# Entscheider/depthhead

Hardware: AMD Instinct MI355X
Metric: depth frames/sec (640x480, 10-tree forest) (higher is better)
Workload: dtype u32/f64

## Files before the change

depthhead_amd/_lib.py:

```python
from __future__ import annotations

import ctypes as C
import os

import numpy as np

_HERE = os.path.dirname(os.path.abspath(__file__))
LIB_PATH = os.path.join(_HERE, "libdepthhead_hip.so")

DH_OK = 0
ERRORS = {-1: "DH_EINVAL", -2: "DH_EFOREST", -3: "DH_EHIP", -4: "DH_ENOMEM", -5: "DH_ESIZE", -6: "DH_ESTATE"}

POSE_DTYPE = np.dtype([("mid_point", "<f4", (3,)), ("reserved", "<u4"), ("rotation", "<f8", (3,))], align=True)
assert POSE_DTYPE.itemsize == 40
SUPPORT_DTYPE = np.dtype([("x", "<u4"), ("y", "<u4"), ("width", "<u4"), ("height", "<u4"), ("windows", "<u4"), ("hits", "<u4"),
                          ("mass", "<u8"), ("total_mass", "<u8")], align=True)
assert SUPPORT_DTYPE.itemsize == 40
SUPPORT_RADIUS = 30
HEAD_DTYPE = np.dtype([("pose", POSE_DTYPE), ("support", SUPPORT_DTYPE)], align=True)
assert HEAD_DTYPE.itemsize == 80 and HEAD_DTYPE.fields["support"][1] == 40
MAX_HEADS = 4
HEADS_SUPPRESS = 2
TRACK_DTYPE = np.dtype([("id", "<u4"), ("age", "<u4"), ("hits", "<u4"), ("misses", "<u4"), ("head", HEAD_DTYPE)], align=True)
assert TRACK_DTYPE.itemsize == 96 and TRACK_DTYPE.fields["head"][1] == 16
# ... 92 lines not shown


class IdentParams(C.Structure):
    _fields_ = [("iterations", C.c_uint32), ("min_points", C.c_uint32), ("gate", C.c_double), ("lam", C.c_double), ("max_rms", C.c_double),
                ("min_ratio", C.c_double), ("reserved", C.c_uint64 * 3)]


VIEW_INSTANCE_DTYPE = np.dtype([("first_cam", "<u4"), ("model", "<u4"), ("views", "<u8"), ("R", "<f4", (9,)), ("t", "<f4", (3,)),
                                ("scale", "<f4"), ("flags", "<u4")], align=True)
assert VIEW_INSTANCE_DTYPE.itemsize == 72
VIEW_FIT_RECORD_DTYPE = np.dtype([("points", "<u4"), ("steps", "<u4"), ("status", "<u4"), ("reserved", "<u4"), ("sum_r2_fixed", "<i8"),
                                  ("views_used", "<u8")], align=True)
assert VIEW_FIT_RECORD_DTYPE.itemsize == 32
FIT_VIEW_TOLERANCE = 0.001


RIG_FIT_STATE_DTYPE = np.dtype([("id", "<u4"), ("R", "<f4", (9,)), ("t", "<f4", (3,)), ("t_prev", "<f4", (3,)), ("views_used", "<u8"),
                                ("tracked", "<u4"), ("have_prev", "<u4"), ("age", "<u4"), ("lost", "<u4")], align=True)
assert RIG_FIT_STATE_DTYPE.itemsize == 88 and RIG_FIT_STATE_DTYPE.fields["views_used"][1] == 64
RIG_FIT_RECORD_DTYPE = np.dtype([("instance", VIEW_INSTANCE_DTYPE), ("fit", VIEW_FIT_RECORD_DTYPE), ("id", "<u4"), ("status", "<u4"),
                                 ("age", "<u4"), ("lost", "<u4"), ("person", "<u4"), ("reserved", "<u4")], align=True)
assert RIG_FIT_RECORD_DTYPE.itemsize == 128 and RIG_FIT_RECORD_DTYPE.fields["fit"][1] == 72
RIG_FIT_NO_PERSON = 0xFFFFFFFF


class RigFitTrackParams(C.Structure):
    _fields_ = [("iterations_tracked", C.c_uint32), ("keep_points", C.c_uint32), ("rms_max", C.c_double), ("max_jump", C.c_double),
                ("max_coast", C.c_uint32), ("max_misses", C.c_uint32), ("reserved", C.c_uint64 * 2)]


class ShapeParams(C.Structure):
    _fields_ = [("gate", C.c_double), ("lam", C.c_double), ("min_points", C.c_uint32), ("reserved0", C.c_uint32),
                ("reserved", C.c_uint64 * 2)]


CALIB_RECORD_DTYPE = np.dtype([("V", "<f4", (9,)), ("u", "<f4", (3,)), ("points", "<u4"), ("pairs", "<u4"), ("status", "<u4"),
                               ("reserved", "<u4"), ("sum_r2_fixed", "<i8"), ("delta", "<f8", (6,))], align=True)
assert CALIB_RECORD_DTYPE.itemsize == 120
CALIB_SKIP = 0xFFFFFFFF
CALIB_ARM_UNIT = 64
CALIB_MAX_ARM = 2048


class CalibParams(C.Structure):
    _fields_ = [("gate", C.c_double), ("lam", C.c_double), ("pivot", C.c_double * 3), ("min_points", C.c_uint32),
                ("reserved0", C.c_uint32), ("reserved", C.c_uint64 * 2)]


class RigTrackParams(C.Structure):
    _fields_ = [("max_heads", C.c_int32), ("radius", C.c_uint32), ("fuse_gate", C.c_uint32), ("gate", C.c_uint32),
                ("max_misses", C.c_uint32)]


class MultiTrackParams(C.Structure):
    _fields_ = [("max_heads", C.c_int32), ("radius", C.c_uint32), ("gate", C.c_uint32), ("max_misses", C.c_uint32)]


class ForestDesc(C.Structure):
    _fields_ = [("n_trees", C.c_uint32), ("roots", C.c_void_p), ("n_nodes", C.c_uint32), ("nodes", C.c_void_p),
                ("n_leaves", C.c_uint32), ("leaf_prob", C.c_void_p), ("off_begin", C.c_void_p),
                ("rot_begin", C.c_void_p), ("offsets", C.c_void_p), ("rotations", C.c_void_p)]


class Params(C.Structure):
    _fields_ = [("stepwidth", C.c_uint32), ("subimage_width", C.c_uint32), ("subimage_height", C.c_uint32),
                ("gaussian_sigma", C.c_float), ("meanshift_iterations", C.c_uint32)]


class Timing(C.Structure):
    _fields_ = [("traverse_ms", C.c_float), ("vote_ms", C.c_float), ("cluster_ms", C.c_float),
                ("total_ms", C.c_float), ("n_frames", C.c_uint32), ("boxsum_ms", C.c_float),
                ("emit_ms", C.c_float), ("reserved", C.c_uint32)]


EXPORTS = [
    "dh_last_error", "dh_version", "dh_forest_create", "dh_forest_destroy", "dh_forest_info",
    "dh_predictor_create", "dh_predictor_destroy", "dh_predictor_update_sigma", "dh_predictor_sigma",
    "dh_predict_batch", "dh_predict_batch_device", "dh_predict_batch_rle", "dh_biwi_decode_depth_device", "dh_host_alloc", "dh_host_free", "dh_predictor_reserve", "dh_predictor_set_forking", "dh_patch_grid",
    "dh_predict_mask", "dh_predict_mask_device", "dh_hough_image", "dh_hough_image_device", "dh_build_hough_image", "dh_build_hough_image_device",
    "dh_predict_from2dhough", "dh_predict_from2dhough_device",
    "dh_biwi_decode_depth", "dh_biwi_parse_cal", "dh_biwi_parse_pose",
    "dh_graph_capture", "dh_graph_launch", "dh_graph_destroy",
    "dh_set_profiling", "dh_get_timing", "dh_debug_enable", "dh_debug_leaf_indices", "dh_debug_patch_flags",
    "dh_debug_grids", "dh_debug_guesses", "dh_debug_votes", "dh_debug_meanshift", "dh_debug_hit_counts", "dh_debug_geometry", "dh_debug_tile_shifts",
    "dh_trainer_create", "dh_trainer_destroy", "dh_trainer_add_frames", "dh_trainer_fit", "dh_trainer_stats", "dh_forest_export",
    "dh_cameras_create", "dh_cameras_destroy", "dh_predict_batch_cameras", "dh_predict_batch_cameras_device",
    "dh_tracker_create", "dh_tracker_destroy", "dh_tracker_reset", "dh_tracker_step", "dh_tracker_step_device",
    "dh_tracker_state", "dh_tracker_capture",
    "dh_predict_batch_support", "dh_predict_batch_support_device", "dh_predict_batch_cameras_support",
    "dh_predict_batch_cameras_support_device", "dh_tracker_step_support", "dh_tracker_step_support_device",
    "dh_predict_heads", "dh_predict_heads_device", "dh_predict_heads_cameras", "dh_predict_heads_cameras_device",
    "dh_multi_tracker_create", "dh_multi_tracker_destroy", "dh_multi_tracker_reset", "dh_multi_tracker_step",
    "dh_multi_tracker_step_device", "dh_multi_tracker_state", "dh_multi_tracker_capture",
    "dh_rig_create", "dh_rig_destroy", "dh_rig_tracker_create", "dh_rig_tracker_destroy", "dh_rig_tracker_reset",
    "dh_rig_tracker_step", "dh_rig_tracker_step_device", "dh_rig_tracker_state", "dh_rig_tracker_capture",
    "dh_mesh_create", "dh_mesh_destroy", "dh_mesh_info", "dh_renderer_create", "dh_renderer_destroy",
    "dh_renderer_set_profiling", "dh_renderer_timing",
    "dh_render_depth", "dh_render_depth_cameras", "dh_render_depth_device", "dh_render_depth_cameras_device",
    "dh_fit_model_create", "dh_fit_model_destroy", "dh_fit_model_info", "dh_fit_params_default", "dh_fitter_create",
    "dh_fitter_destroy", "dh_fit_depth", "dh_fit_depth_cameras", "dh_fit_depth_device", "dh_fit_depth_cameras_device",
    "dh_fit_track_params_default", "dh_fit_tracker_angles", "dh_fit_tracker_create", "dh_fit_tracker_destroy", "dh_fit_tracker_reset",
    "dh_fit_tracker_state", "dh_fit_tracker_step_poses", "dh_fit_tracker_step_poses_device", "dh_fit_tracker_step",
    "dh_fit_tracker_step_device",
    "dh_fit_basis_create", "dh_fit_basis_destroy", "dh_fit_basis_info", "dh_shape_params_default", "dh_fit_shape", "dh_fit_shape_cameras",
    "dh_fit_shape_device", "dh_fit_shape_cameras_device", "dh_fit_shape_views", "dh_fit_shape_views_device",
    "dh_calib_params_default", "dh_fit_calibrate_views", "dh_fit_calibrate_views_device",
    "dh_fit_views_create", "dh_fit_views_destroy", "dh_fit_views_info", "dh_fit_depth_views", "dh_fit_depth_views_device",
    "dh_rig_fit_track_params_default", "dh_rig_fit_tracker_create", "dh_rig_fit_tracker_destroy", "dh_rig_fit_tracker_reset",
    "dh_rig_fit_tracker_state", "dh_rig_fit_tracker_step_persons", "dh_rig_fit_tracker_step_persons_device", "dh_rig_fit_tracker_step",
    "dh_rig_fit_tracker_step_device",
    "dh_fit_subjects_create", "dh_fit_subjects_destroy", "dh_fit_subjects_info", "dh_fit_subjects_model", "dh_fit_subjects_set_coeffs",
    "dh_fit_subjects_state", "dh_fit_subjects_read", "dh_fit_subjects_update", "dh_fit_subjects_update_device", "dh_fit_shape_subjects", "dh_fit_shape_subjects_cameras",
    "dh_fit_shape_subjects_device", "dh_fit_shape_subjects_cameras_device", "dh_fit_depth_carried_device",
    "dh_fit_depth_cameras_carried_device",
    "dh_fit_subjects_create_surface", "dh_fit_subjects_set_offsets", "dh_fit_subjects_read_offsets", "dh_fit_surface_params_default",
    "dh_fit_surface_subjects", "dh_fit_surface_subjects_cameras", "dh_fit_surface_subjects_device", "dh_fit_surface_subjects_cameras_device",
    "dh_fit_ident_params_default", "dh_fit_identify_subjects", "dh_fit_identify_subjects_cameras", "dh_fit_identify_subjects_device",
    "dh_fit_identify_subjects_cameras_device",
    "dh_fit_ident_views_params_default", "dh_fit_identify_subjects_views", "dh_fit_identify_subjects_views_device",
]


class TrainParams(C.Structure):
    _fields_ = [("stepwidth", C.c_uint32), ("subimage_width", C.c_uint32), ("subimage_height", C.c_uint32),
                ("max_depth", C.c_uint32), ("n_trees", C.c_uint32), ("subset_per_tree", C.c_uint32),
                ("subrect_feature_scale", C.c_double), ("features_per_node", C.c_uint32), ("min_subset_size", C.c_uint32),
                ("steepness", C.c_double), ("seed", C.c_uint64)]


class TrainStats(C.Structure):
    _fields_ = [("frames", C.c_uint64), ("pool_size", C.c_uint64), ("pool_positives", C.c_uint64), ("neg_det", C.c_uint64),
                ("levels", C.c_uint32), ("reserved", C.c_uint32)]


class DepthheadError(RuntimeError):
    def __init__(self, code: int, msg: str):
        super().__init__(f"{ERRORS.get(code, code)}: {msg}")
        self.code = code


_lib = None


def load():
    global _lib
    if _lib is not None:
        return _lib
    if os.environ.get("DH_NO_TORCH_PRELOAD") != "1":
        try:
            import torch
        except ImportError:
            pass
    path = os.environ.get("DH_LIB_PATH") or LIB_PATH
    if not os.path.exists(path):
        raise ImportError(f"{path} not built: run `python -c 'import __graft_entry__ as g; g.build()'` "
                          "(the depthhead_amd product path has no CPU fallback)")
    lib = C.CDLL(path)
    for name in EXPORTS:
        fn = getattr(lib, name)
        fn.restype = C.c_int
    lib.dh_last_error.restype = C.c_char_p
    _lib = lib
    return lib


def check(rc: int):
    if rc != DH_OK:
# ... 69 lines not shown
```

depthhead_amd/csrc/dh_api.hip:

```cpp
#include "dh_runtime.h"
#include "dh_render.h"
#include "dh_fit.h"
#include "dh_runtime_fit.h"

extern "C" const char *dh_last_error(void) { return dh_err_get_(); }
extern "C" int dh_version(void) { return DH_VERSION; }

static int forest_create_(const dh_forest_desc *d, dh_forest **out) { return dh_forest_build_(d, out); }

static int forest_destroy_(dh_forest *f) {
    delete f;
    return DH_OK;
}

static int forest_info_(const dh_forest *f, uint32_t *n_trees, uint32_t *n_nodes, uint32_t *n_leaves, uint32_t *max_depth) {
    if (!f) return fail(DH_EINVAL, "dh_forest_info: NULL forest");
    if (n_trees) *n_trees = (uint32_t)f->roots.size();
    if (n_nodes) *n_nodes = (uint32_t)f->nodes.size();
    if (n_leaves) *n_leaves = (uint32_t)f->leaf_prob.size();
    if (max_depth) *max_depth = f->max_depth;
    return DH_OK;
}

static int patch_grid_(const dh_params *p, int w, int h, int *nx, int *ny) {
    if (!p || !nx || !ny) return fail(DH_EINVAL, "dh_patch_grid: NULL argument");
    return dh_patch_grid_(*p, w, h, nx, ny);
}

#define DH_MAX_CHUNKS 8
#define DH_MIN_CHUNK_FRAMES 16

struct Workspace {
    Geom geom;
    int cap_frames = 0;
    Buf<HitRec> hits;
    Buf<HitBox> hit_box;
    Buf<HitRot> hit_rot;
    uint32_t hits_cap = 0;
    Buf<uint32_t> box;
    Buf<unsigned long long> box_mask;
    int blk_shift = 5;
    Buf<uint32_t> tile_list;
    size_t tile_list_stride = 0;
    TileShifts shifts;
    Buf<uint32_t> tile_shift;
    int list_chunks = 0;
    uint32_t *list_ptr(int chunk) const { return tile_list.get() + (size_t)chunk * 8 * (2 * tile_list_stride + 1); }
    Buf<uint32_t> win_patch;
    Buf<uint8_t> win_leaf;
    int leaf_ls = 2;
    Buf<uint32_t> pre_region;
    int pre_cap = 0;
    uint32_t pre_min_hits = 0;
    Buf<uint32_t> counters;
    CounterLayout lay;
    Buf<dh_pose> poses;
    Buf<float> midp;
    Buf<double> rot;
    Buf<uint8_t> mask;
    Buf<uint16_t> frames;
    Buf<int32_t> aux_leaf;
    Buf<uint8_t> aux_flags;
    Buf<uint32_t> aux_u32;
    int aux_cap = 0;
    Buf<uint8_t> aux_out;
    Buf<int32_t> dbg_leaf;
    Buf<uint8_t> dbg_flags;
    Buf<int32_t> dbg_guess, dbg_trace;
    Buf<uint32_t> dbg_steps;
    Buf<int32_t> dbg_votes;
    Buf<uint32_t> dbg_vcount;
    bool dbg_valid = false;
    Buf<uint32_t> hit_win;
    Buf<SupAcc> sup_acc;
    Buf<uint32_t> sup_bits;
    uint32_t sup_words = 0;
    Buf<dh_support> sup;
    Buf<int32_t> hd_pick;
    Buf<uint32_t> hd_nseed;
    Buf<HdMom> hd_mom;
    Buf<dh_pose> hd_pose;
    Buf<SupAcc> hd_acc;
    Buf<uint32_t> hd_bits;
    Buf<dh_support> hd_sup;
    Buf<uint8_t> hd_mask;
    Buf<uint32_t> hd_rgrid;
    Buf<dh_head> hd_out;
    Buf<uint32_t> hd_n;

    uint32_t *hit_count(int f0) const { return counters.get() + lay.hit_count + f0; }
    uint32_t *pos_grid(int f0) const { return counters.get() + lay.pos_grid + (size_t)f0 * DH_POSGRID; }
    uint32_t *rot_grid(int f0) const { return counters.get() + lay.rot_grid + (size_t)f0 * DH_GRID3; }
    uint8_t *tile_flags(int f0) const { return (uint8_t *)(counters.get() + lay.tile_flags) + (size_t)f0 * lay.tiles; }
    uint32_t *win_count(int f0) const { return counters.get() + lay.win_count + (size_t)f0 * lay.tiles; }
    uint32_t *leaf_hits(int f0) const { return lay.leaves ? counters.get() + lay.leaf_hits + (size_t)f0 * lay.leaves : nullptr; }
};

struct dh_predictor {
    int device = 0;
    Knobs knobs;
    dh_params params{};
    uint32_t n_trees = 0, n_nodes = 0, n_leaves = 0, n_off = 0, n_rot = 0, max_depth = 0;
    DevForest dev{};
    std::vector<Buf<uint8_t>> forest;
    Buf<float> kern_r2;
    Buf<uint16_t> zeros;
    bool f_uniform = false;
    int f_rw = 0, f_rh = 0;
    Buf<NodeG> nodes_g;
    Buf<uint4> nodes_u;
    Buf<uint4> nodes_a;
    Buf<uint32_t> amb_flag;
    Buf<uint32_t> amb_list;
    uint32_t n_amb = 0;
    bool absorb_ok = false;
    Buf<uint32_t> top_tab;
    int top_levels = -1;
    long long nodes_u_key = 0;
    Buf<uint32_t> gen;
    hipStream_t own_stream = nullptr;
    hipStream_t copy_stream = nullptr;
    hipEvent_t ev_stage[DH_STAGE_EVENTS] = {};
    hipEvent_t ev_slice = nullptr;
    Buf<uint8_t, PINNED> pin_small;
    Buf<uint8_t, PINNED> pin_out;
    Buf<uint8_t, PINNED> pin_blob;
    Buf<uint2, PINNED> pin_runs;
    Buf<uint32_t, PINNED> pin_begin;
    Buf<uint8_t> dev_blob;
    Buf<uint2> dev_runs;
    Buf<uint32_t> dev_begin;
    int chunks = 1;
    hipStream_t aux_stream[DH_MAX_CHUNKS - 1] = {};
    hipEvent_t ev_fork = nullptr, ev_join[DH_MAX_CHUNKS - 1] = {};
    Workspace ws;
    Buf<float> blur_kern;
    int blur_klen = 0;
    float blur_sigma = 0.0f;
    hipGraph_t graph = nullptr;
    hipGraphExec_t graph_exec = nullptr;
    bool capturing = false;
    bool graph_stale = false;
    bool debug = false;
    int last_n = 0;
    const uint16_t *last_frames = nullptr;
    bool profiling = false;
    hipEvent_t ev[6] = {nullptr, nullptr, nullptr, nullptr, nullptr, nullptr};
    bool ev_valid = false;
#ifdef DH_PROFILING_KNOBS
    Buf<unsigned long long> trav_stamps, cl_stamps;
#endif
};

template <typename T>
static int forest_alloc(dh_predictor *p, T **out, size_t count) {
    Buf<uint8_t> b;
    TRY(b.alloc(std::max<size_t>(count, 1) * sizeof(T)));
    *out = (T *)b.get();
    p->forest.push_back(std::move(b));
    return DH_OK;
}
template <typename T>
static int upload(dh_predictor *p, const T **out, const std::vector<T> &v) {
    T *d = nullptr;
    TRY(forest_alloc(p, &d, v.size()));
    if (!v.empty()) HIP_TRY(hipMemcpy(d, v.data(), v.size() * sizeof(T), hipMemcpyHostToDevice));
    *out = d;
    return DH_OK;
}

static int build_kernel_table(dh_predictor *p) {
    std::vector<float> r2;
    dh_build_kernel_r2_(p->params.gaussian_sigma, r2, DH_KERN_R2);
    HIP_TRY(hipMemcpy(p->kern_r2.get(), r2.data(), r2.size() * sizeof(float), hipMemcpyHostToDevice));
    return DH_OK;
}

// ... 339 lines not shown
    snprintf(batch_name, sizeof batch_name, "dh:batch n=%d %dx%d", n, w, h);
    Range batch_range(o.profile, batch_name);
    if (o.profile) HIP_TRY(hipEventRecord(p->ev[0], s));
    uint32_t *box = g.uniform ? ws.box.get() + (size_t)f0 * g.box_rows * ((size_t)g.box_plane << g.swz_log2) : nullptr;
    uint8_t *tile_flags = ws.tile_flags(f0);
    const bool use_list = ws.tile_list && g.npatch > 0 && !o.leaf_out && !o.flags_out && !p->debug && (long)n * g.tiles_x * g.tiles_y > 512;
    if (use_list) p->ws.list_chunks = std::max(p->ws.list_chunks, o.chunk + 1);
    uint2 *tl_list = use_list ? (uint2 *)ws.list_ptr(o.chunk) : nullptr;
    uint32_t *tl_count = use_list ? ws.list_ptr(o.chunk) + 16 * ws.tile_list_stride : nullptr;
    if (g.npatch > 0 && g.uniform) {
        BoxArgs ba{};
        ba.frames = fr; ba.zeros = p->zeros.get(); ba.n_frames = n; ba.w = w; ba.h = h; ba.rw = p->f_rw; ba.rh = p->f_rh;
        ba.tile_flags = tile_flags; ba.tiles_x = g.tiles_x; ba.tiles_y = g.tiles_y; ba.gen = gen;
        if (o.zero_fold) { ba.zero_ptr = ws.counters.get(); ba.zero_lo = (uint32_t)ws.lay.zero_lo; ba.zero_hi = (uint32_t)ws.lay.zero_hi; ba.zero_end = (uint32_t)ws.lay.zero_words; }
        ba.tpx = g.px * (int)p->params.stepwidth; ba.tpy = g.py * (int)p->params.stepwidth;
        ba.tbw = (g.px - 1) * (int)p->params.stepwidth + (int)p->params.subimage_width - p->f_rw + 1;
        ba.tbh = (g.py - 1) * (int)p->params.stepwidth + (int)p->params.subimage_height - p->f_rh + 1;
        ba.out = box; ba.plane = g.box_plane; ba.rows = g.box_rows; ba.lg = g.swz_log2;
        ba.ow = g.box_ow; ba.oh = g.box_oh; ba.parts = g.box_parts; ba.bands = g.box_bands;
        const bool ring_on = !p->knobs.box_no_ring;
        if (ring_on && p->f_rh >= 2 && p->f_rh - 1 <= 28) {
            const int blk = 1 << ws.blk_shift;
            int oh = 0;
            const size_t lds_wg = (size_t)4 * (p->f_rh - 1) * 64 * 8 + (size_t)4 * (256 + 96 + 8) * 4;
            const int wg_per_cu = (int)std::max<size_t>(1, std::min<size_t>(6, ((size_t)160 * 1024) / lds_wg));
            int bands = dh_box_bands_(n, g.box_parts, g.box_rows, blk, p->f_rh, wg_per_cu * 256, &oh);
            if (p->knobs.box_bands > 0) {
                bands = std::min(p->knobs.box_bands, std::max(1, (g.box_rows + blk - 1) / blk));
                oh = ((g.box_rows + bands - 1) / bands + blk - 1) & ~(blk - 1);
            }
            ba.oh = oh;
            ba.bands = (g.box_rows + ba.oh - 1) / ba.oh;
            ba.ring = 1;
        }
        ba.blk_shift = ws.blk_shift;
        ba.mask_blocks = (g.box_rows + (1 << ws.blk_shift) - 1) >> ws.blk_shift;
        ba.blk_mask = ws.box_mask ? ws.box_mask.get() + (size_t)f0 * ba.mask_blocks * g.box_parts : nullptr;
        if (use_list && ws.shifts.on) ba.list_count = tl_count;
        ba.blocks_per_frame = (ba.parts * ba.bands + 3) / 4;
        { Range r(o.profile, "dh:boxsum"); HIP_TRY(dh_launch_boxsum(ba, s)); }
    }
    if (g.npatch > 0 && !g.uniform) {
        PixFlagArgs fa{};
        fa.frames = fr; fa.n_frames = n; fa.w = w; fa.h = h; fa.tile_flags = tile_flags; fa.gen = gen;
        fa.tiles_x = g.tiles_x; fa.tiles_y = g.tiles_y;
        fa.tpx = g.px * (int)p->params.stepwidth; fa.tpy = g.py * (int)p->params.stepwidth;
        fa.tfw = (g.px - 1) * (int)p->params.stepwidth + (int)p->params.subimage_width;
        fa.tfh = (g.py - 1) * (int)p->params.stepwidth + (int)p->params.subimage_height;
        { Range r(o.profile, "dh:pixflags"); HIP_TRY(dh_launch_pixflags(fa, s)); }
    }
    if (use_list && ws.shifts.on) {
        TileShiftArgs sa{};
        sa.n_frames = n; sa.blk_shift = ws.blk_shift; sa.mask_blocks = (g.box_rows + (1 << ws.blk_shift) - 1) >> ws.blk_shift; sa.parts = g.box_parts;
        sa.blk_mask = ws.box_mask.get() + (size_t)f0 * sa.mask_blocks * g.box_parts;
        sa.ow4 = g.box_ow / 4; sa.nc = g.box_parts * sa.ow4;
        sa.tiles_x = g.tiles_x; sa.tiles_y = g.tiles_y; sa.step = (int)p->params.stepwidth;
        sa.tpx = g.px * sa.step; sa.tpy = g.py * sa.step;
        sa.tbw = (g.px - 1) * sa.step + (int)p->params.subimage_width - p->f_rw + 1;
        sa.tbh = (g.py - 1) * sa.step + (int)p->params.subimage_height - p->f_rh + 1;
        sa.sx0 = ws.shifts.sx0; sa.sy0 = ws.shifts.sy0; sa.gx = ws.shifts.gx; sa.nsx = ws.shifts.nsx; sa.nsy = ws.shifts.nsy;
        sa.list = tl_list; sa.count = tl_count; sa.stride = (uint32_t)ws.tile_list_stride; sa.shift_out = ws.tile_shift.get() + f0;
        Range r(o.profile, "dh:tile_list"); HIP_TRY(dh_launch_tile_shift(sa, s));
    } else
    if (use_list) { Range r(o.profile, "dh:tile_list"); HIP_TRY(dh_launch_tile_list(tile_flags, gen, n, g.tiles_x * g.tiles_y, tl_list, tl_count, (uint32_t)ws.tile_list_stride, s)); }
    if (o.profile) HIP_TRY(hipEventRecord(p->ev[4], s));
    if (g.npatch > 0) {
        TraverseArgs ta{};
        ta.frames = fr; ta.n_frames = n; ta.w = w; ta.h = h;
        ta.step = (int)p->params.stepwidth; ta.sw = (int)p->params.subimage_width; ta.sh = (int)p->params.subimage_height;
        ta.nx = g.nx; ta.ny = g.ny; ta.px = g.px; ta.py = g.py; ta.tiles_x = g.tiles_x; ta.tiles_y = g.tiles_y;
        ta.ss_max = g.ss_max; ta.ss_row = g.ss_row; ta.swz_log2 = g.swz_log2; ta.swz_q = g.swz_q;
        ta.uniform = g.uniform ? 1 : 0; ta.rw = p->f_rw; ta.rh = p->f_rh; ta.area = (uint32_t)(p->f_rw * p->f_rh);
        ta.nodes_u = p->nodes_u.get(); ta.nodes_a = p->absorb_ok ? p->nodes_a.get() : nullptr; ta.walk_lb = (p->n_nodes + p->n_amb) << 4; ta.amb_list = p->amb_list.get(); ta.top_tab = p->top_tab.get(); ta.top_levels = g.top_levels; ta.nodes_g = p->knobs.no_general_int ? nullptr : p->nodes_g.get();
        ta.box = box; ta.box_plane = g.box_plane; ta.box_rows = g.box_rows;
        ta.tile_flags = tile_flags; ta.gen = gen;
#ifdef DH_PROFILING_KNOBS
        ta.stop_phase = p->knobs.trav_stop;
        if (p->knobs.trav_stamps) {
            unsigned long long *stamps = p->trav_stamps.get();
            if (!stamps) { TRY(p->trav_stamps.alloc(8)); stamps = p->trav_stamps.get(); HIP_TRY(hipMemset(stamps, 0, 64)); }
            else {
                unsigned long long hst[8];
                HIP_TRY(hipMemcpy(hst, stamps, 64, hipMemcpyDeviceToHost));
                fprintf(stderr, "[k_traverse cycles/phase summed over the workgroups that reach it] region=%llu gate=%llu walks=%llu\n", hst[0], hst[1], hst[2]);
                HIP_TRY(hipMemset(stamps, 0, 64));
            }
            ta.dbg_stamps = stamps;
        }
#endif
        ta.f = p->dev;
        const int tiles = g.tiles_x * g.tiles_y;
        uint32_t *win_count = ws.win_count(f0);
        ta.win_count = win_count; ta.win_cap = g.win_cap;
        ta.win_patch = ws.win_patch.get() + (size_t)f0 * g.win_cap; ta.win_leaf = ws.win_leaf.get() + (((size_t)f0 * g.win_cap * p->n_trees) << ws.leaf_ls); ta.leaf_ls = ws.leaf_ls;
        ta.dbg_leaf = o.leaf_out ? o.leaf_out : p->debug ? ws.dbg_leaf.get() + (size_t)f0 * g.npatch * p->n_trees : nullptr;
        ta.dbg_flags = o.flags_out ? o.flags_out : p->debug ? ws.dbg_flags.get() + (size_t)f0 * g.npatch : nullptr;
        if (use_list) { ta.tile_list = tl_list; ta.tile_list_count = tl_count; ta.tile_list_stride = (uint32_t)ws.tile_list_stride; }
        { Range r(o.profile, "dh:traverse"); HIP_TRY(dh_launch_traverse(ta, g.lds, s)); }
        if (o.profile) HIP_TRY(hipEventRecord(p->ev[5], s));
        if (!o.traverse_only) {
            EmitArgs ea{};
            ea.frames = fr; ea.n_frames = n; ea.w = w; ea.h = h;
            ea.step = ta.step; ea.lw = ta.sw / 2; ea.lh = ta.sh / 2; ea.nx = g.nx; ea.npatch = g.npatch;
            ea.px = g.px; ea.py = g.py; ea.tiles = tiles;
            memcpy(ea.kinv, kinv, 9 * sizeof(float));
            ea.cams = cs.dev();
            ea.f = p->dev;
            ea.win_count = win_count; ea.win_patch = ta.win_patch; ea.win_leaf = ta.win_leaf; ea.leaf_ls = ws.leaf_ls; ea.win_cap = g.win_cap;
            ea.hits = ws.hits.get() + hoff; ea.hit_box = ws.hit_box.get() + hoff; ea.hit_rot = ws.hit_rot.get() + hoff;
            ea.hit_count = hit_count; ea.hits_cap = ws.hits_cap;
            ea.leaf_hits = q.heads ? nullptr : leaf_hits;
            ea.gen = gen;
            ea.dbg_flags = ta.dbg_flags;
            if (q.support || q.heads) ea.hit_win = ws.hit_win.get() + hoff;
#ifdef DH_PROFILING_KNOBS
            ea.stop = p->knobs.emit_stop;
#endif
            { Range r(o.profile, "dh:emit"); HIP_TRY(dh_launch_emit(ea, s)); }
        }
    } else if (o.profile) HIP_TRY(hipEventRecord(p->ev[5], s));
    if (o.profile) HIP_TRY(hipEventRecord(p->ev[1], s));
    if (o.traverse_only) return DH_OK;
    {
        VoteArgs va{};
        va.n_frames = n; va.w = w; va.h = h;
        va.cell_fast = !p->knobs.vote_exact && (!cs.c || cs.all_cell_fast(n, w, h)) ? 1 : 0;
        memcpy(va.k, K, sizeof va.k);
        va.cams = cs.dev(); va.cams_pin = cs.c && cs.all_pin(n) ? 1 : 0;
        va.f = p->dev; va.hits = ws.hits.get() + hoff; va.hit_box = ws.hit_box.get() + hoff; va.hit_rot = ws.hit_rot.get() + hoff;
        va.hit_count = hit_count; va.hits_cap = ws.hits_cap;
        va.pos_grid = pos_grid; va.rot_grid = rot_grid;
        va.leaf_hits = q.heads ? nullptr : leaf_hits;
#ifdef DH_PROFILING_KNOBS
        va.stop = p->knobs.vote_stop;
#endif
        { Range r(o.profile, "dh:vote"); HIP_TRY(dh_launch_vote(va, s)); }
    }
    if (o.profile) HIP_TRY(hipEventRecord(p->ev[2], s));
    if (q.heads) {
        HeadsArgs ha{};
        ha.n_frames = n; ha.w = w; ha.h = h; ha.max_heads = q.max_heads;
        memcpy(ha.k, K, sizeof ha.k);
        ha.cams = cs.dev();
        ha.off4 = p->dev.off4; ha.rough_cell = p->dev.rough_cell;
        ha.hits = ws.hits.get() + hoff; ha.hit_box = ws.hit_box.get() + hoff; ha.hit_rot = ws.hit_rot.get() + hoff; ha.hit_win = ws.hit_win.get() + hoff;
        ha.hit_count = hit_count; ha.hits_cap = ws.hits_cap;
        ha.pos_grid = pos_grid;
        const size_t hk = (size_t)f0 * DH_MAX_HEADS;
        ha.pick = ws.hd_pick.get() + hk; ha.nseed = ws.hd_nseed.get() + f0; ha.mom = ws.hd_mom.get() + hk;
        ha.nx = g.nx; ha.step = (int)p->params.stepwidth;
        ha.lw = (int)p->params.subimage_width / 2; ha.lh = (int)p->params.subimage_height / 2;
        ha.radius = q.radius;
        ha.hpose = ws.hd_pose.get() + hk; ha.acc = ws.hd_acc.get() + hk; ha.bits = ws.hd_bits.get() + hk * ws.sup_words; ha.bit_words = ws.sup_words;
        ha.hsup = ws.hd_sup.get() + hk; ha.hmask = ws.hd_mask.get() + hoff; ha.rgrid = ws.hd_rgrid.get() + hk * DH_GRID3;
        ha.n_heads = q.n_heads; ha.heads = q.heads;
        ClusterArgs ca{};
        ca.frames = fr; ca.n_frames = n; ca.w = w; ca.h = h;
        memcpy(ca.kinv, kinv, 9 * sizeof(float));
        ca.cams = cs.dev();
        ca.f = p->dev; ca.hits = ha.hits; ca.hit_box = ha.hit_box; ca.hit_rot = ha.hit_rot;
        ca.hit_count = hit_count; ca.hits_cap = ws.hits_cap;
        ca.pos_grid = pos_grid; ca.rot_grid = ha.rgrid; ca.kern_r2 = p->kern_r2.get();
        ca.iterations = p->params.meanshift_iterations;
        ca.out = ws.hd_pose.get() + hk;
        ca.hd_nseed = ha.nseed; ca.hd_mom = ha.mom; ca.hd_rgrid = ha.rgrid; ca.hd_mask = ha.hmask;
        Range r(o.profile, "dh:heads");
        HIP_TRY(dh_launch_heads_seeds(ha, s));
        HIP_TRY(dh_launch_heads_moments(ha, s));
        ca.hd_which = 0;
        HIP_TRY(dh_launch_cluster_heads(ca, q.max_heads, s));
        HIP_TRY(dh_launch_heads_support(ha, s));
        ca.hd_which = 1;
        HIP_TRY(dh_launch_cluster_heads(ca, q.max_heads, s));
        HIP_TRY(dh_launch_heads_finish(ha, s));
        if (o.profile) { HIP_TRY(hipEventRecord(p->ev[3], s)); p->ev_valid = true; }
        return DH_OK;
    }
    {
        ClusterArgs ca{};
        ca.frames = fr; ca.n_frames = n; ca.w = w; ca.h = h;
        memcpy(ca.kinv, kinv, 9 * sizeof(float));
        ca.cams = cs.dev();
        ca.f = p->dev; ca.hits = ws.hits.get() + hoff; ca.hit_box = ws.hit_box.get() + hoff; ca.hit_rot = ws.hit_rot.get() + hoff;
        ca.hit_count = hit_count; ca.hits_cap = ws.hits_cap;
        ca.leaf_hits = leaf_hits;
        ca.pos_grid = pos_grid; ca.rot_grid = rot_grid; ca.kern_r2 = p->kern_r2.get();
        ca.iterations = p->params.meanshift_iterations;
#ifdef DH_PROFILING_KNOBS
        ca.stop = p->knobs.cl_stop;
        if (p->knobs.cl_stamps) {
// ... 1049 lines not shown
    return aux_call(p, "dh_predict_mask", AUX_MASK, frames, n, w, h, nullptr, mask, true);
}
static int hough_image_(dh_predictor *p, const uint16_t *frames, int n, int w, int h, const float K[9], uint16_t *out) {
    return aux_call(p, "dh_hough_image", AUX_VOTES, frames, n, w, h, K, out, true);
}
static int build_hough_image_(dh_predictor *p, const uint16_t *frames, int n, int w, int h, const float K[9], uint16_t *out) {
    return aux_call(p, "dh_build_hough_image", AUX_VOTES | AUX_BLUR, frames, n, w, h, K, out, true);
}
static int predict_from2dhough_(dh_predictor *p, const uint16_t *frames, int n, int w, int h, const float K[9], dh_pose *out) {
    return aux_call(p, "dh_predict_from2dhough", AUX_VOTES | AUX_BLUR | AUX_POSES, frames, n, w, h, K, out, true);
}

static int set_profiling_(dh_predictor *p, int on) {
    if (!p) return fail(DH_EINVAL, "NULL predictor");
    p->profiling = on != 0;
    p->ev_valid = false;
    return DH_OK;
}
static int get_timing_(dh_predictor *p, dh_timing *out) {
    if (!p || !out) return fail(DH_EINVAL, "NULL argument");
    if (!p->ev_valid) return fail(DH_ESTATE, "no profiled batch yet (dh_set_profiling + a batch)");
    DeviceGuard guard(p->device);
    if (!guard.ok) return DH_EHIP;
    HIP_TRY(hipEventSynchronize(p->ev[3]));
    HIP_TRY(hipEventElapsedTime(&out->boxsum_ms, p->ev[0], p->ev[4]));
    HIP_TRY(hipEventElapsedTime(&out->traverse_ms, p->ev[4], p->ev[5]));
    HIP_TRY(hipEventElapsedTime(&out->emit_ms, p->ev[5], p->ev[1]));
    HIP_TRY(hipEventElapsedTime(&out->vote_ms, p->ev[1], p->ev[2]));
    HIP_TRY(hipEventElapsedTime(&out->cluster_ms, p->ev[2], p->ev[3]));
    HIP_TRY(hipEventElapsedTime(&out->total_ms, p->ev[0], p->ev[3]));
    out->n_frames = (uint32_t)p->last_n;

    return DH_OK;
}

static int debug_enable_(dh_predictor *p, int on) {
    if (!p) return fail(DH_EINVAL, "NULL predictor");
    p->debug = on != 0;
    if (!p->debug) p->ws.dbg_valid = false;
    return DH_OK;
}
template <typename F>
static int with_taps(dh_predictor *p, bool dbg, F body) {
    if (!p) return fail(DH_EINVAL, "NULL predictor");
    if (p->last_n == 0) return fail(DH_ESTATE, "no batch has run on this predictor");
    DeviceGuard guard(p->device);
    if (!guard.ok) return DH_EHIP;
    hipError_t e = hipDeviceSynchronize();
    if (e != hipSuccess) return fail(DH_EHIP, "sync: %s", hipGetErrorString(e));
    if (dbg && !p->ws.dbg_valid) return fail(DH_ESTATE, "debug taps were not enabled for the last batch");
    return body();
}
static int debug_leaf_indices_(dh_predictor *p, int32_t *out, size_t cap) {
    return with_taps(p, true, [&]() -> int {
        size_t n = (size_t)p->last_n * p->ws.geom.npatch * p->n_trees;
        if (!out || cap < n) return fail(DH_EINVAL, "buffer too small: need %zu elements", n);
        if (n) HIP_TRY(hipMemcpy(out, p->ws.dbg_leaf.get(), n * sizeof(int32_t), hipMemcpyDeviceToHost));
        return DH_OK;
    });
}
static int debug_patch_flags_(dh_predictor *p, uint8_t *out, size_t cap) {
    return with_taps(p, true, [&]() -> int {
        size_t n = (size_t)p->last_n * p->ws.geom.npatch;
        if (!out || cap < n) return fail(DH_EINVAL, "buffer too small: need %zu elements", n);
        if (n) HIP_TRY(hipMemcpy(out, p->ws.dbg_flags.get(), n, hipMemcpyDeviceToHost));
        return DH_OK;
    });
}
static int debug_grids_(dh_predictor *p, uint32_t *pos_grid, uint32_t *rot_grid) {
    return with_taps(p, false, [&]() -> int {
        const Workspace &ws = p->ws;
        if (pos_grid) HIP_TRY(hipMemcpy(pos_grid, ws.pos_grid(0), (ws.pos_grid(p->last_n) - ws.pos_grid(0)) * 4, hipMemcpyDeviceToHost));
        if (rot_grid) HIP_TRY(hipMemcpy(rot_grid, ws.rot_grid(0), (ws.rot_grid(p->last_n) - ws.rot_grid(0)) * 4, hipMemcpyDeviceToHost));
        return DH_OK;
    });
}
static int debug_hit_counts_(dh_predictor *p, uint32_t *out) {
    return with_taps(p, false, [&]() -> int {
        if (!out) return fail(DH_EINVAL, "NULL output");
        HIP_TRY(hipMemcpy(out, p->ws.hit_count(0), (size_t)p->last_n * 4, hipMemcpyDeviceToHost));
        return DH_OK;
    });
}
static int debug_geometry_(dh_predictor *p, int32_t out[10]) {
    if (!p || !out) return fail(DH_EINVAL, "NULL argument");
    if (p->ws.cap_frames == 0) return fail(DH_ESTATE, "no workspace yet (dh_predictor_reserve or a batch)");
    const Geom &g = p->ws.geom;
    const bool walk_tab = g.uniform && p->absorb_ok;
    const int32_t v[10] = {(g.uniform ? 1 : 0) | (walk_tab ? 1 << 8 : 0) | (walk_tab ? g.top_levels << 16 : 0), g.px, g.py, g.tiles_x, g.tiles_y, g.swz_log2, g.swz_q, g.ss_row, p->f_rw, p->f_rh};
    memcpy(out, v, sizeof v);
    return DH_OK;
}
static int debug_tile_shifts_(dh_predictor *p, int32_t *shifts, uint32_t counts[8]) {
    return with_taps(p, false, [&]() -> int {
        const Workspace &ws = p->ws;
        if (!shifts || !counts) return fail(DH_EINVAL, "NULL output");
        if (ws.list_chunks == 0) return fail(DH_ESTATE, "the last batch ran without tile lists");
        std::vector<uint32_t> sh((size_t)p->last_n, 0u);
        if (ws.tile_shift) HIP_TRY(hipMemcpy(sh.data(), ws.tile_shift.get(), sh.size() * 4, hipMemcpyDeviceToHost));
        for (int f = 0; f < p->last_n; ++f) { shifts[2 * f] = (int32_t)(sh[f] & 0xffffu); shifts[2 * f + 1] = (int32_t)(sh[f] >> 16); }
        for (int x = 0; x < 8; ++x) counts[x] = 0;
        for (int c = 0; c < ws.list_chunks; ++c) {
            uint32_t cc[8];
            HIP_TRY(hipMemcpy(cc, ws.list_ptr(c) + 16 * ws.tile_list_stride, sizeof cc, hipMemcpyDeviceToHost));
            for (int x = 0; x < 8; ++x) counts[x] += cc[x];
        }
        return DH_OK;
    });
}
static int debug_guesses_(dh_predictor *p, int32_t *out) {
    return with_taps(p, true, [&]() -> int {
        if (!out) return fail(DH_EINVAL, "NULL output");
        HIP_TRY(hipMemcpy(out, p->ws.dbg_guess.get(), (size_t)p->last_n * 6 * 4, hipMemcpyDeviceToHost));
        return DH_OK;
    });
}
static int debug_meanshift_(dh_predictor *p, int which, int32_t *trace, uint32_t *steps) {
    return with_taps(p, true, [&]() -> int {
        if (which < 0 || which > 1) return fail(DH_EINVAL, "which must be 0 or 1");
        size_t per = (size_t)(p->params.meanshift_iterations + 1) * 3;
        if (trace) HIP_TRY(hipMemcpy(trace, p->ws.dbg_trace.get() + (size_t)which * p->last_n * per, (size_t)p->last_n * per * 4, hipMemcpyDeviceToHost));
        if (steps) HIP_TRY(hipMemcpy(steps, p->ws.dbg_steps.get() + (size_t)which * p->last_n, (size_t)p->last_n * 4, hipMemcpyDeviceToHost));
        return DH_OK;
    });
}
static int debug_votes_(dh_predictor *p, int frame, int which, int32_t *out, size_t cap, size_t *count) {
    return with_taps(p, false, [&]() -> int {
        if (frame < 0 || frame >= p->last_n || which < 0 || which > 1 || !count) return fail(DH_EINVAL, "bad frame / which / count");
        Workspace &ws = p->ws;
        if (which == 1 && ws.lay.leaves && !ws.dbg_valid) return fail(DH_ESTATE, "rotation votes need dh_debug_enable(1) before the batch");
        if (cap > 0xffffffffull) cap = 0xffffffffull;
        if (!ws.dbg_vcount) TRY(ws.dbg_vcount.alloc(1));
        if (cap * 4 > ws.dbg_votes.cap()) TRY(ws.dbg_votes.alloc(cap * 4));
        HIP_TRY(hipMemset(ws.dbg_vcount.get(), 0, 4));
        VotesDumpArgs a{};
        a.frame = frame; a.which = which; a.f = p->dev; a.hits = ws.hits.get(); a.hit_box = ws.hit_box.get(); a.hit_rot = ws.hit_rot.get(); a.hit_count = ws.hit_count(0); a.hits_cap = ws.hits_cap;
        a.out = ws.dbg_votes.get(); a.cap = (uint32_t)cap; a.count = ws.dbg_vcount.get();
        HIP_TRY(dh_launch_votes_dump(a, nullptr));
        HIP_TRY(hipDeviceSynchronize());
        uint32_t c = 0;
        HIP_TRY(hipMemcpy(&c, ws.dbg_vcount.get(), 4, hipMemcpyDeviceToHost));
        *count = c;
        size_t ncopy = std::min<size_t>(c, cap);
        if (ncopy && out) HIP_TRY(hipMemcpy(out, ws.dbg_votes.get(), ncopy * 16, hipMemcpyDeviceToHost));
        return DH_OK;
    });
}

struct FitTrackAngles {
    double v[DH_FIT_TRACK_ANGLES][2];
    FitTrackAngles() {
        for (int i = 0; i < DH_FIT_TRACK_ANGLES; ++i) {
            const double a = (double)(i - 60) / 60.0 * 3.14159;
            v[i][0] = cos(a); v[i][1] = sin(a);
        }
    }
};
static const FitTrackAngles &fit_track_angles() {
    static const FitTrackAngles tab;
    return tab;
}
static int fit_tracker_angles_(double out[DH_FIT_TRACK_ANGLES][2]) {
    if (!out) return fail(DH_EINVAL, "dh_fit_tracker_angles: NULL argument");
    memcpy(out, fit_track_angles().v, sizeof fit_track_angles().v);
    return DH_OK;
}
static int fit_track_params_default_(dh_fit_track_params *p) {
    if (!p) return fail(DH_EINVAL, "dh_fit_track_params_default: NULL argument");
    memset(p, 0, sizeof *p);
    p->iterations_tracked = 6; p->keep_points = 30;
    p->rms_max = 5.0; p->max_jump = 150.0;
    p->conf_num = 1; p->conf_den = 50;
// ... 349 lines not shown
    if (!guard.ok) return DH_EHIP;
    return rig_fit_enqueue(t, frames, w, h, present, rt->prm.max_heads, n_heads, heads, n_persons, persons, prm, records, (hipStream_t)stream);
}
static int rig_fit_host(dh_predictor *p, dh_rig_fit_tracker *t, dh_rig_tracker *rt, const uint16_t *frames, int w, int h, const uint8_t *present,
                        int max_heads, const dh_fit_params &prm, uint32_t *n_heads, dh_head *heads, uint32_t *ids, uint32_t *n_persons,
                        dh_rig_person *persons, dh_rig_track *tracks, dh_rig_fit_record *records) {
    const size_t n = (size_t)t->n, ng = (size_t)t->rig->n_rigs, mh = (size_t)max_heads;
    return fit_tracker_host(t, frames, w, h, present, [&](hipStream_t s) -> int {
        if (p) return DH_OK;
        HIP_TRY(hipMemcpyAsync(t->n_heads.get(), n_heads, n * sizeof(uint32_t), hipMemcpyHostToDevice, s));
        HIP_TRY(hipMemcpyAsync(t->heads.get(), heads, n * mh * sizeof(dh_head), hipMemcpyHostToDevice, s));
        HIP_TRY(hipMemcpyAsync(t->n_persons.get(), n_persons, ng * sizeof(uint32_t), hipMemcpyHostToDevice, s));
        HIP_TRY(hipMemcpyAsync(t->persons.get(), persons, ng * DH_RIG_MAX_PERSONS * sizeof(dh_rig_person), hipMemcpyHostToDevice, s));
        return DH_OK;
    }, [&](const uint16_t *fr, const uint8_t *pr, hipStream_t s) -> int {
        if (p) TRY(rig_tracker_step_device_(p, rt, fr, w, h, pr, t->n_heads.get(), t->heads.get(), t->ids.get(), t->n_persons.get(),
                                            t->persons.get(), tracks ? t->tracks.get() : nullptr, s));
        return rig_fit_enqueue(t, fr, w, h, pr, max_heads, t->n_heads.get(), t->heads.get(), t->n_persons.get(), t->persons.get(), prm,
                               t->records.get(), s);
    }, [&](hipStream_t s) -> int {
        if (!p) return DH_OK;
        HIP_TRY(hipMemcpyAsync(n_heads, t->n_heads.get(), n * sizeof(uint32_t), hipMemcpyDeviceToHost, s));
        HIP_TRY(hipMemcpyAsync(heads, t->heads.get(), n * mh * sizeof(dh_head), hipMemcpyDeviceToHost, s));
        HIP_TRY(hipMemcpyAsync(ids, t->ids.get(), n * mh * sizeof(uint32_t), hipMemcpyDeviceToHost, s));
        HIP_TRY(hipMemcpyAsync(n_persons, t->n_persons.get(), ng * sizeof(uint32_t), hipMemcpyDeviceToHost, s));
        HIP_TRY(hipMemcpyAsync(persons, t->persons.get(), ng * DH_RIG_MAX_PERSONS * sizeof(dh_rig_person), hipMemcpyDeviceToHost, s));
        if (tracks) HIP_TRY(hipMemcpyAsync(tracks, t->tracks.get(), ng * DH_RIG_MAX_TRACKS * sizeof(dh_rig_track), hipMemcpyDeviceToHost, s));
        return DH_OK;
    }, records, ng * DH_RIG_MAX_TRACKS);
}
static int rig_fit_tracker_step_persons_(dh_rig_fit_tracker *t, const uint16_t *frames, int w, int h, const uint8_t *present, int max_heads,
                                         const uint32_t *n_heads, const dh_head *heads, const uint32_t *n_persons, const dh_rig_person *persons,
                                         const dh_fit_params *fit_params, dh_rig_fit_record *records) {
    dh_fit_params prm;
    TRY(rig_fit_check(t, frames, w, h, max_heads, n_heads, heads, n_persons, persons, fit_params, records, &prm, "dh_rig_fit_tracker_step_persons"));
    return rig_fit_host(nullptr, t, nullptr, frames, w, h, present, max_heads, prm, const_cast<uint32_t *>(n_heads), const_cast<dh_head *>(heads),
                        nullptr, const_cast<uint32_t *>(n_persons), const_cast<dh_rig_person *>(persons), nullptr, records);
}
static int rig_fit_tracker_step_(dh_predictor *p, dh_rig_fit_tracker *t, dh_rig_tracker *rt, const uint16_t *frames, int w, int h,
                                 const uint8_t *present, const dh_fit_params *fit_params, uint32_t *n_heads, dh_head *heads, uint32_t *ids,
                                 uint32_t *n_persons, dh_rig_person *persons, dh_rig_track *tracks, dh_rig_fit_record *records) {
    const char *who = "dh_rig_fit_tracker_step";
    dh_fit_params prm;
    TRY(rig_fit_step_check(p, t, rt, frames, w, h, n_heads, heads, ids, n_persons, persons, fit_params, records, &prm, who));
    if (t->cams->device != p->device) return fail(DH_EINVAL, "%s: rig table on device %d, predictor on device %d", who, t->cams->device, p->device);
    return rig_fit_host(p, t, rt, frames, w, h, present, rt->prm.max_heads, prm, n_heads, heads, ids, n_persons, persons, tracks, records);
}

DH_API(forest_create, (const dh_forest_desc *d, dh_forest **out), (d, out))
DH_API(forest_destroy, (dh_forest *f), (f))
DH_API(forest_info, (const dh_forest *f, uint32_t *n_trees, uint32_t *n_nodes, uint32_t *n_leaves, uint32_t *max_depth), (f, n_trees, n_nodes, n_leaves, max_depth))
DH_API(patch_grid, (const dh_params *p, int w, int h, int *nx, int *ny), (p, w, h, nx, ny))
DH_API(predictor_destroy, (dh_predictor *p), (p))
DH_API(predictor_create, (const dh_forest *f, const dh_params *prm, int device, dh_predictor **out), (f, prm, device, out))
DH_API(predictor_update_sigma, (dh_predictor *p, float val), (p, val))
DH_API(predictor_sigma, (const dh_predictor *p, float *out), (p, out))
DH_API(predictor_reserve, (dh_predictor *p, int n, int w, int h), (p, n, w, h))
DH_API(predictor_set_forking, (dh_predictor *p, int chunks), (p, chunks))
DH_API(predict_batch_device, (dh_predictor *p, const uint16_t *frames, int n, int w, int h, const float K[9], const float *midp_guess, const double *rot_guess, const uint8_t *guess_mask, dh_pose *out, void *stream_), (p, frames, n, w, h, K, midp_guess, rot_guess, guess_mask, out, stream_))
DH_API(predict_batch, (dh_predictor *p, const uint16_t *frames, int n, int w, int h, const float K[9], const float *midp_guess, const double *rot_guess, const uint8_t *guess_mask, dh_pose *out), (p, frames, n, w, h, K, midp_guess, rot_guess, guess_mask, out))
DH_API(host_alloc, (size_t bytes, void **out), (bytes, out))
DH_API(host_free, (void *ptr), (ptr))
DH_API(biwi_decode_depth_device, (dh_predictor *p, const uint8_t *const *bufs, const size_t *lens, int n, uint16_t *frames_dev, size_t cap_px, uint32_t *w, uint32_t *h), (p, bufs, lens, n, frames_dev, cap_px, w, h))
DH_API(predict_batch_rle, (dh_predictor *p, const uint8_t *const *bufs, const size_t *lens, int n, const float K[9], const float *midp_guess, const double *rot_guess, const uint8_t *guess_mask, dh_pose *out), (p, bufs, lens, n, K, midp_guess, rot_guess, guess_mask, out))
DH_API(graph_destroy, (dh_predictor *p), (p))
DH_API(graph_capture, (dh_predictor *p, const uint16_t *frames, int n, int w, int h, const float K[9], const float *midp_guess, const double *rot_guess, const uint8_t *guess_mask, dh_pose *out), (p, frames, n, w, h, K, midp_guess, rot_guess, guess_mask, out))
DH_API(graph_launch, (dh_predictor *p, void *stream), (p, stream))
DH_API(predict_mask_device, (dh_predictor *p, const uint16_t *frames, int n, int w, int h, uint8_t *mask, void *stream), (p, frames, n, w, h, mask, stream))
DH_API(hough_image_device, (dh_predictor *p, const uint16_t *frames, int n, int w, int h, const float K[9], uint16_t *out, void *stream), (p, frames, n, w, h, K, out, stream))
DH_API(predict_mask, (dh_predictor *p, const uint16_t *frames, int n, int w, int h, uint8_t *mask), (p, frames, n, w, h, mask))
DH_API(hough_image, (dh_predictor *p, const uint16_t *frames, int n, int w, int h, const float K[9], uint16_t *out), (p, frames, n, w, h, K, out))
DH_API(build_hough_image_device, (dh_predictor *p, const uint16_t *frames, int n, int w, int h, const float K[9], uint16_t *out, void *stream), (p, frames, n, w, h, K, out, stream))
DH_API(predict_from2dhough_device, (dh_predictor *p, const uint16_t *frames, int n, int w, int h, const float K[9], dh_pose *out, void *stream), (p, frames, n, w, h, K, out, stream))
DH_API(build_hough_image, (dh_predictor *p, const uint16_t *frames, int n, int w, int h, const float K[9], uint16_t *out), (p, frames, n, w, h, K, out))
DH_API(predict_from2dhough, (dh_predictor *p, const uint16_t *frames, int n, int w, int h, const float K[9], dh_pose *out), (p, frames, n, w, h, K, out))
DH_API(set_profiling, (dh_predictor *p, int on), (p, on))
DH_API(get_timing, (dh_predictor *p, dh_timing *out), (p, out))
DH_API(debug_enable, (dh_predictor *p, int on), (p, on))
DH_API(debug_leaf_indices, (dh_predictor *p, int32_t *out, size_t cap), (p, out, cap))
DH_API(debug_patch_flags, (dh_predictor *p, uint8_t *out, size_t cap), (p, out, cap))
DH_API(debug_grids, (dh_predictor *p, uint32_t *pos_grid, uint32_t *rot_grid), (p, pos_grid, rot_grid))
DH_API(debug_hit_counts, (dh_predictor *p, uint32_t *out), (p, out))
DH_API(debug_geometry, (dh_predictor *p, int32_t out[10]), (p, out))
DH_API(debug_tile_shifts, (dh_predictor *p, int32_t *shifts, uint32_t counts[8]), (p, shifts, counts))
DH_API(debug_guesses, (dh_predictor *p, int32_t *out), (p, out))
DH_API(debug_meanshift, (dh_predictor *p, int which, int32_t *trace, uint32_t *steps), (p, which, trace, steps))
DH_API(debug_votes, (dh_predictor *p, int frame, int which, int32_t *out, size_t cap, size_t *count), (p, frame, which, out, cap, count))
DH_API(cameras_create, (const float *K, int n, int device, dh_cameras **out), (K, n, device, out))
DH_API(cameras_destroy, (dh_cameras *c), (c))
DH_API(predict_batch_cameras, (dh_predictor *p, const uint16_t *frames, int n, int w, int h, const dh_cameras *c, const float *midp_guess, const double *rot_guess, const uint8_t *guess_mask, dh_pose *out), (p, frames, n, w, h, c, midp_guess, rot_guess, guess_mask, out))
DH_API(predict_batch_cameras_device, (dh_predictor *p, const uint16_t *frames, int n, int w, int h, const dh_cameras *c, const float *midp_guess, const double *rot_guess, const uint8_t *guess_mask, dh_pose *out, void *stream), (p, frames, n, w, h, c, midp_guess, rot_guess, guess_mask, out, stream))
DH_API(tracker_create, (const dh_cameras *c, uint32_t flags, dh_tracker **out), (c, flags, out))
DH_API(tracker_destroy, (dh_tracker *t), (t))
DH_API(tracker_reset, (dh_tracker *t, int camera, void *stream), (t, camera, stream))
DH_API(tracker_step, (dh_predictor *p, dh_tracker *t, const uint16_t *frames, int w, int h, const uint8_t *present, dh_pose *out), (p, t, frames, w, h, present, out))
DH_API(tracker_step_device, (dh_predictor *p, dh_tracker *t, const uint16_t *frames, int w, int h, const uint8_t *present, dh_pose *out, void *stream), (p, t, frames, w, h, present, out, stream))
DH_API(tracker_state, (dh_tracker *t, float *midp, double *rot, uint8_t *flags), (t, midp, rot, flags))
DH_API(tracker_capture, (dh_predictor *p, dh_tracker *t, const uint16_t *frames, int w, int h, const uint8_t *present, dh_pose *out), (p, t, frames, w, h, present, out))
DH_API(predict_batch_support, (dh_predictor *p, const uint16_t *frames, int n, int w, int h, const float K[9], const float *midp_guess, const double *rot_guess, const uint8_t *guess_mask, uint32_t radius, dh_pose *out, dh_support *support), (p, frames, n, w, h, K, midp_guess, rot_guess, guess_mask, radius, out, support))
DH_API(predict_batch_support_device, (dh_predictor *p, const uint16_t *frames, int n, int w, int h, const float K[9], const float *midp_guess, const double *rot_guess, const uint8_t *guess_mask, uint32_t radius, dh_pose *out, dh_support *support, void *stream), (p, frames, n, w, h, K, midp_guess, rot_guess, guess_mask, radius, out, support, stream))
DH_API(predict_batch_cameras_support, (dh_predictor *p, const uint16_t *frames, int n, int w, int h, const dh_cameras *c, const float *midp_guess, const double *rot_guess, const uint8_t *guess_mask, uint32_t radius, dh_pose *out, dh_support *support), (p, frames, n, w, h, c, midp_guess, rot_guess, guess_mask, radius, out, support))
DH_API(predict_batch_cameras_support_device, (dh_predictor *p, const uint16_t *frames, int n, int w, int h, const dh_cameras *c, const float *midp_guess, const double *rot_guess, const uint8_t *guess_mask, uint32_t radius, dh_pose *out, dh_support *support, void *stream), (p, frames, n, w, h, c, midp_guess, rot_guess, guess_mask, radius, out, support, stream))
DH_API(tracker_step_support, (dh_predictor *p, dh_tracker *t, const uint16_t *frames, int w, int h, const uint8_t *present, uint32_t radius, dh_pose *out, dh_support *support), (p, t, frames, w, h, present, radius, out, support))
DH_API(tracker_step_support_device, (dh_predictor *p, dh_tracker *t, const uint16_t *frames, int w, int h, const uint8_t *present, uint32_t radius, dh_pose *out, dh_support *support, void *stream), (p, t, frames, w, h, present, radius, out, support, stream))
DH_API(predict_heads, (dh_predictor *p, const uint16_t *frames, int n, int w, int h, const float K[9], int max_heads, uint32_t radius, uint32_t *n_heads, dh_head *heads), (p, frames, n, w, h, K, max_heads, radius, n_heads, heads))
DH_API(predict_heads_device, (dh_predictor *p, const uint16_t *frames, int n, int w, int h, const float K[9], int max_heads, uint32_t radius, uint32_t *n_heads, dh_head *heads, void *stream), (p, frames, n, w, h, K, max_heads, radius, n_heads, heads, stream))
DH_API(predict_heads_cameras, (dh_predictor *p, const uint16_t *frames, int n, int w, int h, const dh_cameras *c, int max_heads, uint32_t radius, uint32_t *n_heads, dh_head *heads), (p, frames, n, w, h, c, max_heads, radius, n_heads, heads))
DH_API(predict_heads_cameras_device, (dh_predictor *p, const uint16_t *frames, int n, int w, int h, const dh_cameras *c, int max_heads, uint32_t radius, uint32_t *n_heads, dh_head *heads, void *stream), (p, frames, n, w, h, c, max_heads, radius, n_heads, heads, stream))
DH_API(multi_tracker_create, (const dh_cameras *c, const dh_multi_track_params *prm, dh_multi_tracker **out), (c, prm, out))
DH_API(multi_tracker_destroy, (dh_multi_tracker *t), (t))
DH_API(multi_tracker_reset, (dh_multi_tracker *t, int camera, void *stream), (t, camera, stream))
DH_API(multi_tracker_step, (dh_predictor *p, dh_multi_tracker *t, const uint16_t *frames, int w, int h, const uint8_t *present, uint32_t *n_heads, dh_head *heads, uint32_t *ids, dh_head_track *tracks), (p, t, frames, w, h, present, n_heads, heads, ids, tracks))
DH_API(multi_tracker_step_device, (dh_predictor *p, dh_multi_tracker *t, const uint16_t *frames, int w, int h, const uint8_t *present, uint32_t *n_heads, dh_head *heads, uint32_t *ids, dh_head_track *tracks, void *stream), (p, t, frames, w, h, present, n_heads, heads, ids, tracks, stream))
DH_API(multi_tracker_state, (dh_multi_tracker *t, dh_head_track *tracks, uint32_t *next_id), (t, tracks, next_id))
DH_API(multi_tracker_capture, (dh_predictor *p, dh_multi_tracker *t, const uint16_t *frames, int w, int h, const uint8_t *present, uint32_t *n_heads, dh_head *heads, uint32_t *ids, dh_head_track *tracks), (p, t, frames, w, h, present, n_heads, heads, ids, tracks))
DH_API(rig_create, (const dh_cameras *c, const float *R, const float *t, const int32_t *rig_begin, int n_rigs, dh_rig **out), (c, R, t, rig_begin, n_rigs, out))
DH_API(rig_destroy, (dh_rig *r), (r))
DH_API(rig_tracker_create, (const dh_rig *r, const dh_rig_track_params *prm, dh_rig_tracker **out), (r, prm, out))
DH_API(rig_tracker_destroy, (dh_rig_tracker *t), (t))
DH_API(rig_tracker_reset, (dh_rig_tracker *t, int rig, void *stream), (t, rig, stream))
DH_API(rig_tracker_step, (dh_predictor *p, dh_rig_tracker *t, const uint16_t *frames, int w, int h, const uint8_t *present, uint32_t *n_heads, dh_head *heads, uint32_t *rig_ids, uint32_t *n_persons, dh_rig_person *persons, dh_rig_track *tracks), (p, t, frames, w, h, present, n_heads, heads, rig_ids, n_persons, persons, tracks))
DH_API(rig_tracker_step_device, (dh_predictor *p, dh_rig_tracker *t, const uint16_t *frames, int w, int h, const uint8_t *present, uint32_t *n_heads, dh_head *heads, uint32_t *rig_ids, uint32_t *n_persons, dh_rig_person *persons, dh_rig_track *tracks, void *stream), (p, t, frames, w, h, present, n_heads, heads, rig_ids, n_persons, persons, tracks, stream))
DH_API(rig_tracker_state, (dh_rig_tracker *t, dh_rig_track *tracks, uint32_t *next_id), (t, tracks, next_id))
DH_API(rig_tracker_capture, (dh_predictor *p, dh_rig_tracker *t, const uint16_t *frames, int w, int h, const uint8_t *present, uint32_t *n_heads, dh_head *heads, uint32_t *rig_ids, uint32_t *n_persons, dh_rig_person *persons, dh_rig_track *tracks), (p, t, frames, w, h, present, n_heads, heads, rig_ids, n_persons, persons, tracks))
DH_API(fit_track_params_default, (dh_fit_track_params *p), (p))
DH_API(fit_tracker_angles, (double out[DH_FIT_TRACK_ANGLES][2]), (out))
DH_API(fit_tracker_create, (const dh_cameras *c, const dh_fit_model *m, float scale, uint32_t flags, const dh_fit_track_params *params, dh_fit_tracker **out), (c, m, scale, flags, params, out))
DH_API(fit_tracker_destroy, (dh_fit_tracker *t), (t))
DH_API(fit_tracker_reset, (dh_fit_tracker *t, int camera, void *stream), (t, camera, stream))
DH_API(fit_tracker_state, (dh_fit_tracker *t, dh_fit_track_state *states), (t, states))
DH_API(fit_tracker_step_poses, (dh_fit_tracker *t, const uint16_t *frames, int w, int h, const uint8_t *present, const dh_pose *poses, const dh_support *support, const dh_fit_params *fit_params, dh_fit_track_record *records), (t, frames, w, h, present, poses, support, fit_params, records))
DH_API(fit_tracker_step_poses_device, (dh_fit_tracker *t, const uint16_t *frames, int w, int h, const uint8_t *present, const dh_pose *poses, const dh_support *support, const dh_fit_params *fit_params, dh_fit_track_record *records, void *stream), (t, frames, w, h, present, poses, support, fit_params, records, stream))
DH_API(fit_tracker_step, (dh_predictor *p, dh_fit_tracker *t, const uint16_t *frames, int w, int h, const uint8_t *present, uint32_t radius, const dh_fit_params *fit_params, dh_pose *poses_out, dh_support *support_out, dh_fit_track_record *records), (p, t, frames, w, h, present, radius, fit_params, poses_out, support_out, records))
DH_API(fit_tracker_step_device, (dh_predictor *p, dh_fit_tracker *t, const uint16_t *frames, int w, int h, const uint8_t *present, uint32_t radius, const dh_fit_params *fit_params, dh_pose *poses_out, dh_support *support_out, dh_fit_track_record *records, void *stream), (p, t, frames, w, h, present, radius, fit_params, poses_out, support_out, records, stream))
DH_API(rig_fit_track_params_default, (dh_rig_fit_track_params *p), (p))
DH_API(rig_fit_tracker_create, (const dh_rig *rig, const dh_fit_views *views, const dh_fit_model *model, float scale, uint32_t flags, const dh_rig_fit_track_params *params, dh_rig_fit_tracker **out), (rig, views, model, scale, flags, params, out))
DH_API(rig_fit_tracker_destroy, (dh_rig_fit_tracker *t), (t))
DH_API(rig_fit_tracker_reset, (dh_rig_fit_tracker *t, int rig, void *stream), (t, rig, stream))
DH_API(rig_fit_tracker_state, (dh_rig_fit_tracker *t, dh_rig_fit_state *states), (t, states))
DH_API(rig_fit_tracker_step_persons, (dh_rig_fit_tracker *t, const uint16_t *frames, int w, int h, const uint8_t *present, int max_heads, const uint32_t *n_heads, const dh_head *heads, const uint32_t *n_persons, const dh_rig_person *persons, const dh_fit_params *fit_params, dh_rig_fit_record *records), (t, frames, w, h, present, max_heads, n_heads, heads, n_persons, persons, fit_params, records))
DH_API(rig_fit_tracker_step_persons_device, (dh_rig_fit_tracker *t, const uint16_t *frames, int w, int h, const uint8_t *present, int max_heads, const uint32_t *n_heads, const dh_head *heads, const uint32_t *n_persons, const dh_rig_person *persons, const dh_fit_params *fit_params, dh_rig_fit_record *records, void *stream), (t, frames, w, h, present, max_heads, n_heads, heads, n_persons, persons, fit_params, records, stream))
DH_API(rig_fit_tracker_step, (dh_predictor *p, dh_rig_fit_tracker *t, dh_rig_tracker *rt, const uint16_t *frames, int w, int h, const uint8_t *present, const dh_fit_params *fit_params, uint32_t *n_heads, dh_head *heads, uint32_t *rig_ids, uint32_t *n_persons, dh_rig_person *persons, dh_rig_track *tracks, dh_rig_fit_record *records), (p, t, rt, frames, w, h, present, fit_params, n_heads, heads, rig_ids, n_persons, persons, tracks, records))
DH_API(rig_fit_tracker_step_device, (dh_predictor *p, dh_rig_fit_tracker *t, dh_rig_tracker *rt, const uint16_t *frames, int w, int h, const uint8_t *present, const dh_fit_params *fit_params, uint32_t *n_heads, dh_head *heads, uint32_t *rig_ids, uint32_t *n_persons, dh_rig_person *persons, dh_rig_track *tracks, dh_rig_fit_record *records, void *stream), (p, t, rt, frames, w, h, present, fit_params, n_heads, heads, rig_ids, n_persons, persons, tracks, records, stream))
```

depthhead_amd/csrc/dh_host.cpp:

```cpp
#include "dh_host.h"

#include <limits.h>
#include <math.h>
#include <stdarg.h>
#include <stdio.h>
#include <stdlib.h>
#include <string.h>

#include <algorithm>
#include <cmath>
#include <atomic>
#include <string>
#include <thread>
#include <utility>

static thread_local char g_err[512] = "";

int dh_fail_(int code, const char *fmt, ...) {
    va_list ap;
    va_start(ap, fmt);
    vsnprintf(g_err, sizeof g_err, fmt, ap);
    va_end(ap);
    return code;
}
// ... 78 lines not shown
        }
    }
    for (uint32_t L = 0; L < NL; ++L)
        if (f->off_begin[L + 1] - f->off_begin[L] >= (1u << 24) || f->rot_begin[L + 1] - f->rot_begin[L] >= (1u << 16))
            return dh_fail_(DH_EFOREST, "leaf %u: more than 2^24 offset or 2^16 rotation votes", L);
    if (NN > 0) {
        const dh_node &n0 = f->nodes[0];
        f->rw = (uint16_t)(n0.r1[2] - n0.r1[0]); f->rh = (uint16_t)(n0.r1[3] - n0.r1[1]);
        f->uniform = f->rw > 0 && f->rh > 0;
        for (uint32_t i = 0; i < NN && f->uniform; ++i)
            for (const uint16_t *rc : {f->nodes[i].r1, f->nodes[i].r2})
                if (rc[2] - rc[0] != f->rw || rc[3] - rc[1] != f->rh) f->uniform = false;
    }
    for (uint32_t L = 0; L < NL; ++L) {
        if (!(f->leaf_prob[L] > 0.0)) continue;
        if (f->off_begin[L + 1] == f->off_begin[L]) return dh_fail_(DH_EFOREST, "leaf %u: prob > 0 but no offsets (reference divides by zero)", L);
        if (f->rot_begin[L + 1] == f->rot_begin[L]) return dh_fail_(DH_EFOREST, "leaf %u: prob > 0 but no rotations (reference unwraps None)", L);
        for (uint32_t i = f->rot_begin[L]; i < f->rot_begin[L + 1]; ++i)
            for (int k = 0; k < 3; ++k)
                if (!dh_rot_vote_ok_(f->rotations[(size_t)i * 3 + k]))
                    return dh_fail_(DH_EFOREST, "leaf %u: rotation bin outside [0,120) after one wrap (reference indexes out of bounds)", L);
    }
    own.f = nullptr;
    *out = f;
    return DH_OK;
}

void dh_pack_off4_(const dh_forest &f, std::vector<uint32_t> &b4, std::vector<float> &o4) {
    const uint32_t NL = (uint32_t)f.leaf_prob.size();
    b4.assign((size_t)NL + 1, 0);
    for (uint32_t L = 0; L < NL; ++L) b4[L + 1] = b4[L] + ((f.off_begin[L + 1] - f.off_begin[L] + 3u) & ~3u);
    o4.assign(((size_t)b4[NL] + 4) * 4, 0.0f);
    for (uint32_t L = 0; L < NL; ++L)
        for (uint32_t k = f.off_begin[L]; k < f.off_begin[L + 1]; ++k) {
            float *o = &o4[((size_t)b4[L] + (k - f.off_begin[L])) * 4];
            o[0] = f.offsets[(size_t)k * 3]; o[1] = f.offsets[(size_t)k * 3 + 1]; o[2] = f.offsets[(size_t)k * 3 + 2]; o[3] = 0.0f;
        }
}

void dh_build_nodes_g_(const dh_forest &f, std::vector<NodeG> &ng) {
    ng.resize(f.nodes.size());
    for (size_t i = 0; i < f.nodes.size(); ++i) {
        const dh_node &nd = f.nodes[i];
        NodeG o{};
        for (int k = 0; k < 4; ++k) { o.r1[k] = (uint8_t)nd.r1[k]; o.r2[k] = (uint8_t)nd.r2[k]; }
        const uint32_t c1 = (uint32_t)(nd.r1[2] - nd.r1[0]) * (uint32_t)(nd.r1[3] - nd.r1[1]);
        const uint32_t c2 = (uint32_t)(nd.r2[2] - nd.r2[0]) * (uint32_t)(nd.r2[3] - nd.r2[1]);
        const uint32_t C1 = std::max(c1, 1u), C2 = std::max(c2, 1u);
        o.cc = C1 | (C2 << 16);
        o.child_zero = nd.child_zero; o.child_one = nd.child_one;
        const double thr = nd.threshold, cc = (double)C1 * (double)C2;
        if (thr >= 65535.0) { o.ilo = INT64_MAX - 16; o.amb = 0; }
        else if (thr < -65535.0) { o.ilo = INT64_MIN; o.amb = 0; }
        else {
            const double m = 5.820766091346741e-11;
            const double lo = floor((thr - m) * cc - 1.0), hi = ceil((thr + m) * cc + 1.0);
            o.ilo = (int64_t)lo;
            o.amb = (uint32_t)std::min<int64_t>((int64_t)hi - (int64_t)lo - 1, 0xffffffffll);
        }
        ng[i] = o;
    }
}

Knobs dh_read_knobs_() {
    Knobs k;
    auto geti = [](const char *name, int dflt) { const char *e = getenv(name); return e ? atoi(e) : dflt; };
    k.force_general = getenv("DH_FORCE_GENERAL") != nullptr;
    k.no_leaf_hist = getenv("DH_NO_LEAF_HIST") != nullptr;
    k.box_no_ring = getenv("DH_BOX_NO_RING") != nullptr;
    k.leaf_hist_max = (uint32_t)std::max(0, geti("DH_LEAF_HIST_MAX", 16384));
    k.lds_budget_kb = std::max(0, geti("DH_LDS_BUDGET_KB", 0));
    if (const char *e = getenv("DH_TILE")) {
        if (sscanf(e, "%d,%d", &k.tile_x, &k.tile_y) != 2 || k.tile_x < 1 || k.tile_y < 1) k.tile_x = k.tile_y = 0;
    }
    k.box_band = std::max(1, geti("DH_BOX_BAND", 64));
    k.box_bands = std::max(0, geti("DH_BOX_BANDS", 0));
    k.max_resident = std::max(1, geti("DH_MAX_RESIDENT_FRAMES", 512));
    k.chunks = std::max(0, std::min(8, geti("DH_CHUNKS", 0)));
    k.box_dense = getenv("DH_BOX_DENSE") != nullptr;
    k.no_region = getenv("DH_NO_REGION") != nullptr;
    k.region_min_hits = std::max(0, geti("DH_REGION_MIN_HITS", 0));
    k.no_general_int = getenv("DH_NO_GENERAL_INT") != nullptr;
    k.no_absorb = getenv("DH_NO_ABSORB") != nullptr;
    k.vote_exact = getenv("DH_VOTE_EXACT") != nullptr;
    k.no_tile_list = getenv("DH_NO_TILE_LIST") != nullptr;
    k.no_zero_fold = getenv("DH_NO_ZERO_FOLD") != nullptr;
    if (const char *e = getenv("DH_TILE_SHIFT")) {
        char tail = 0;
        if (strcmp(e, "off") == 0) k.tile_shift_mode = 1;
        else if (sscanf(e, "%d,%d%c", &k.tile_shift_x, &k.tile_shift_y, &tail) == 2 && k.tile_shift_x >= 0 && k.tile_shift_y >= 0) k.tile_shift_mode = 2;
        else k.tile_shift_mode = 3;
    }
    if (const char *e = getenv("DH_TOP_LEVELS")) k.top_levels = std::max(0, std::min(8, atoi(e)));
    k.stage_chunk = std::max(1, geti("DH_STAGE_CHUNK", 64));
    k.host_threads = std::max(1, std::min(64, geti("DH_HOST_THREADS", (int)std::max(1u, std::min(8u, std::thread::hardware_concurrency())))));
#ifdef DH_PROFILING_KNOBS
    k.trav_stop = geti("DH_TRAV_STOP", 0); k.emit_stop = geti("DH_EMIT_STOP", 0);
    k.vote_stop = geti("DH_VOTE_STOP", 0); k.cl_stop = geti("DH_CL_STOP", 0);
    k.trav_stamps = getenv("DH_TRAV_STAMPS") != nullptr;
    k.cl_stamps = getenv("DH_CL_STAMPS") != nullptr;
#endif
    return k;
}

int dh_patch_grid_(const dh_params &p, int w, int h, int *nx, int *ny) {
    if (p.stepwidth == 0 || p.subimage_width == 0 || p.subimage_height == 0) return dh_fail_(DH_EINVAL, "zero stepwidth / patch size");
    if (w <= 0 || h <= 0) return dh_fail_(DH_EINVAL, "non-positive frame size");
    if ((uint32_t)w < p.subimage_width || (uint32_t)h < p.subimage_height) return dh_fail_(DH_ESIZE, "frame %dx%d smaller than the %ux%u patch", w, h, p.subimage_width, p.subimage_height);
    uint32_t lw = p.subimage_width / 2, rw = p.subimage_width - lw, lh = p.subimage_height / 2, rh = p.subimage_height - lh;
    uint32_t xe = (uint32_t)w - rw, ye = (uint32_t)h - rh;
    *nx = xe > lw ? (int)((xe - lw + p.stepwidth - 1) / p.stepwidth) : 0;
    *ny = ye > lh ? (int)((ye - lh + p.stepwidth - 1) / p.stepwidth) : 0;
    return DH_OK;
}

void dh_traverse_swizzle(int px, int step, int sw, int rw, int *swz_log2, int *swz_q, int *ss_row) {
    const int bw = (px - 1) * step + sw - rw + 1;
    int lg = 0;
    while (lg < 3 && (step & (1 << lg)) == 0) ++lg;
    const int m = 1 << lg, q = ((bw + m - 1) / m + 3) & ~3;
    int best_pad = 0;
    long best_cost = -1;
    for (int pad = 0; pad < 32; pad += 4) {
        const int ss = m * q + pad;
        int cnt[64] = {0};
        for (int i = 0; i < 64; ++i) cnt[(unsigned)((i / px) * step * ss + (i % px) * (step / m)) & 63u]++;
        long cost = 0;
        for (int b = 0; b < 64; ++b) cost += (long)cnt[b] * cnt[b];
        if (best_cost < 0 || cost < best_cost) { best_cost = cost; best_pad = pad; }
    }
    *swz_log2 = lg; *swz_q = q; *ss_row = m * q + best_pad;
}
int dh_traverse_row_stride(int px, int step, int sw, int rw) {
    if (rw > 0) { int lg, q, ss; dh_traverse_swizzle(px, step, sw, rw, &lg, &q, &ss); return ss; }
    return ((px - 1) * step + sw + 1) | 1;
}
size_t dh_traverse_lds_bytes(int px, int py, int step, int sw, int sh, int top_words, int rw, int rh) {
    size_t fh = (size_t)(py - 1) * step + sh;
    size_t ss = (size_t)dh_traverse_row_stride(px, step, sw, rw);
    size_t rows = rw > 0 ? fh - rh + 1 : fh + 1;
    size_t npt = (size_t)px * py;
    return (ss * rows + npt * 2 + 16 + (size_t)top_words) * 4;
}

int dh_choose_tile_(const TileQuery &p, Geom &g) {
    const int step = (int)p.params.stepwidth, sw = (int)p.params.subimage_width, sh = (int)p.params.subimage_height;
    const int rw = g.uniform ? p.f_rw : 0, rh = g.uniform ? p.f_rh : 0;
    size_t budget = 79 * 1024;
    if (p.lds_budget_kb > 0) budget = (size_t)p.lds_budget_kb * 1024;
    budget = std::min<size_t>(budget, 158 * 1024);
    const int fx = p.tile_x, fy = p.tile_y;
    g.top_levels = 0;
    if (g.uniform && p.absorb_ok) {
        if (p.top_levels >= 0) g.top_levels = p.top_levels;
        else {
            const double want = 200.0 * p.n_trees * 16.0 / ((double)step * step);
            const size_t top_budget = (size_t)std::min(40.0 * 1024, std::max(4.0 * 1024, want));
            while (g.top_levels < 8 && (size_t)p.n_trees * (2u << g.top_levels) * 12 <= top_budget) ++g.top_levels;
        }
        while (g.top_levels > 0 && (size_t)p.n_trees * (1u << g.top_levels) * 12 > 48 * 1024) --g.top_levels;
    }
    const int top_words = g.uniform && p.absorb_ok ? (int)p.n_trees * (1 << g.top_levels) * 3 : 0;
#ifdef TRAV_THREADS
    long max_win = TRAV_THREADS;
#else
    long max_win = 1024;
#endif
    if (p.one_pass && g.uniform && p.absorb_ok) max_win = std::max<long>(16, std::min<long>(max_win, 3200 / std::max<uint32_t>(p.n_trees, 1)));
    long best = -1;
    for (int py = 1; py <= std::min(g.ny, 64); ++py)
        for (int px = 1; px <= std::min(g.nx, 64); ++px) {
            if (px * py > max_win) continue;
            if (fx > 0 && fy > 0 && (px != std::min(fx, g.nx) || py != std::min(fy, g.ny))) continue;
            if (rw > 0 && (px & 3) != 0 && px < g.nx && !(fx > 0)) continue;
            if (rw > 0 && (long)(sh - rh + 1) * dh_traverse_row_stride(px, step, sw, rw) >= 16384) continue;
            size_t lds = dh_traverse_lds_bytes(px, py, step, sw, sh, top_words, rw, rh);
            if (lds > budget && !(fx > 0 && lds <= 158 * 1024)) continue;
            long score = (long)px * py * 1000 - labs((long)px - py);
            if (p.one_pass && g.uniform && p.absorb_ok) score = (long)px * py * 1000 + (px - py);
            if (score > best) { best = score; g.px = px; g.py = py; g.lds = lds; }
        }
    if (best < 0) {
        if (rw > 0 && (long)(sh - rh + 1) * dh_traverse_row_stride(1, step, sw, rw) >= 16384) return 1;
        g.px = g.py = 1;
        g.lds = dh_traverse_lds_bytes(1, 1, step, sw, sh, top_words, rw, rh);
        if (g.lds > 158 * 1024) return rw > 0 ? 1 : dh_fail_(DH_ESIZE, "patch %dx%d with %u trees does not fit LDS", sw, sh, p.n_trees);
    }
    if (g.uniform && p.absorb_ok && p.top_levels < 0)
        while (g.top_levels < 8 && g.lds + (size_t)p.n_trees * (1u << g.top_levels) * 12 <= budget) {
            g.lds += (size_t)p.n_trees * (1u << g.top_levels) * 12;
            ++g.top_levels;
        }
    g.tiles_x = (g.nx + g.px - 1) / g.px;
    g.tiles_y = (g.ny + g.py - 1) / g.py;
    if ((long)g.tiles_x * g.tiles_y > 65535) return dh_fail_(DH_ESIZE, "frame %dx%d needs %ld tiles per frame (limit 65535)", g.w, g.h, (long)g.tiles_x * g.tiles_y);
    g.win_cap = g.tiles_x * g.tiles_y * g.px * g.py;
    g.flag_words = (g.tiles_x * g.tiles_y + 3) / 4;
    g.ss_row = dh_traverse_row_stride(g.px, step, sw, rw);
    if (rw > 0) dh_traverse_swizzle(g.px, step, sw, rw, &g.swz_log2, &g.swz_q, &g.ss_row);
    g.ss_max = g.ss_row * ((g.py - 1) * step + sh + (rw > 0 ? 1 - rh : 1));
    if (rw > 0) {
        g.box_rows = g.h - rh + 1;
        const int m = 1 << g.swz_log2;
        g.box_plane = ((g.w - rw + 1 + m - 1) / m + 4 + 3) & ~3;
        const int bw = g.w - rw + 1, ow_max = (kBoxSpan - rw) & ~3;
        g.box_parts = (bw + ow_max - 1) / ow_max;
        g.box_ow = std::min(ow_max, ((bw + g.box_parts - 1) / g.box_parts + 3) & ~3);
        const int band = std::max(1, p.box_band);
        g.box_bands = (g.box_rows + band - 1) / band;
        g.box_oh = ((g.box_rows + g.box_bands - 1) / g.box_bands + 31) & ~31;
        g.box_bands = (g.box_rows + g.box_oh - 1) / g.box_oh;
    }
    return DH_OK;
}

int dh_tile_shifts_(const Geom &g, int step, int blk_shift, const Knobs &k, TileShifts *out) {
    TileShifts t;
    if (k.tile_shift_mode == 3) return dh_fail_(DH_EINVAL, "DH_TILE_SHIFT: expected \"off\" or \"sx,sy\" (windows, >= 0)");
    *out = t;
    if (k.tile_shift_mode == 1 || !g.uniform || g.npatch <= 0 || k.box_dense || k.no_tile_list || step <= 0) return DH_OK;
    const int slack_x = g.tiles_x * g.px - g.nx, slack_y = g.tiles_y * g.py - g.ny;
    const int m4 = 4 << g.swz_log2;
    int a = step, b = m4;
    while (b) { const int r = a % b; a = b; b = r; }
    t.gx = m4 / a;
    if (k.tile_shift_mode == 2) {
        t.sx0 = std::min(k.tile_shift_x, slack_x) / t.gx * t.gx; t.sy0 = std::min(k.tile_shift_y, slack_y);
    } else {
        t.nsx = slack_x / t.gx + 1; t.nsy = slack_y + 1;
        if (t.nsx * t.nsy == 1) return DH_OK;
    }
    const int mask_blocks = (g.box_rows + (1 << blk_shift) - 1) >> blk_shift;
    const bool fits = dh_tile_shift_lds_words(mask_blocks, g.box_parts, g.box_parts * (g.box_ow / 4), t.nsx * t.nsy) <= DH_TILE_SHIFT_LDS_WORDS;
    if (!fits && k.tile_shift_mode == 2)
        return dh_fail_(DH_EINVAL, "DH_TILE_SHIFT=%d,%d: frames of %dx%d are too large for the shifted tile lists", k.tile_shift_x, k.tile_shift_y, g.w, g.h);
    t.on = fits;
    *out = t;
    return DH_OK;
}

CounterLayout dh_counter_layout_(size_t cap, size_t flag_words, size_t tiles, size_t leaf_hist_leaves) {
    CounterLayout l;
    l.tiles = tiles; l.leaves = leaf_hist_leaves;
    l.hit_count = 0;
    l.pos_grid = l.hit_count + cap;
    l.rot_grid = l.pos_grid + cap * DH_POSGRID;
    l.tile_flags = l.rot_grid + cap * DH_GRID3;
    l.win_count = l.tile_flags + cap * flag_words;
    l.leaf_hits = l.win_count + cap * tiles;
    l.zero_words = l.leaf_hits + cap * leaf_hist_leaves;
    l.zero_lo = l.tile_flags; l.zero_hi = l.win_count;
    l.alloc_words = l.zero_words + 4;
    return l;
}

int dh_box_bands_(int n, int parts, int rows, int blk, int rh, int wg_slots, int *oh_out) {
    n = std::max(n, 1); parts = std::max(parts, 1); rows = std::max(rows, 1); blk = std::max(blk, 1); wg_slots = std::max(wg_slots, 1);
    const int max_bands = std::max(1, (rows + blk - 1) / blk);
    int best_bands = 1, best_oh = ((rows + blk - 1) / blk) * blk;
    double best = -1.0;
    for (int want = 1; want <= max_bands; ++want) {
        const int oh = (((rows + want - 1) / want + blk - 1) / blk) * blk;
        const int bands = (rows + oh - 1) / oh;
        if (bands != want && want > 1) continue;
        const double wgs = (double)n * ((parts * bands + 3) / 4);
        const double r = wgs / wg_slots;
        const double rounds = r <= 1.0 ? 1.0 : r + 0.5 * (std::ceil(r) - r);
        const double cost = (oh + 0.5 * std::max(rh - 1, 0)) * rounds;
        if (best < 0.0 || cost < best - 1e-9) { best = cost; best_bands = bands; best_oh = oh; }
    }
    if (oh_out) *oh_out = best_oh;
    return best_bands;
}

void dh_mat3_inv_f32_(const float m[9], float o[9]) {
    const float a = m[0], b = m[1], c = m[2], d = m[3], e = m[4], f = m[5], g = m[6], h = m[7], i = m[8];
    const float det = a * (e * i - f * h) - d * (b * i - c * h) + g * (b * f - c * e);
    o[0] = (e * i - f * h) / det; o[1] = (c * h - b * i) / det; o[2] = (b * f - c * e) / det;
    o[3] = (f * g - d * i) / det; o[4] = (a * i - c * g) / det; o[5] = (c * d - a * f) / det;
    o[6] = (d * h - e * g) / det; o[7] = (b * g - a * h) / det; o[8] = (a * e - b * d) / det;
}

void dh_build_kernel_table_(float sigma, std::vector<float> &k) {
    const int G = DH_MEANSHIFT_KERNEL_SIZE;
    k.resize((size_t)G * G * G);
    for (int x = 0; x < G; ++x)
        for (int y = 0; y < G; ++y)
            for (int z = 0; z < G; ++z) {
                int dx = x - 10, dy = y - 10, dz = z - 10;
                int norm = dx * dx + dy * dy + dz * dz;
                k[((size_t)x * G + y) * G + z] = expf(-1.0f * (float)norm / (2.0f * sigma));
            }
}
void dh_build_kernel_r2_(float sigma, std::vector<float> &k, size_t padded) {
    k.assign(padded, 0.0f);
    for (int norm = 0; norm <= 300 && (size_t)norm < padded; ++norm) k[(size_t)norm] = expf(-1.0f * (float)norm / (2.0f * sigma));
}

int dh_blur_taps_(float sigma, std::vector<float> &k) {
    if (!(sigma > 0.0f)) return dh_fail_(DH_EINVAL, "gaussian_blur_f32 needs sigma > 0 (the reference asserts)");
    const float r2 = ceilf(2.0f * sigma);
    if (!(r2 <= 2048.0f)) return dh_fail_(DH_ESIZE, "blur radius %g too large", (double)r2);
    const int radius = (int)r2;
    k.assign((size_t)2 * radius + 1, 0.0f);
    const float norm = 1.0f / (sqrtf(2.0f * 3.14159274101257324f) * sigma);
    for (int i = 0; i <= radius; ++i) {
        const float x = (float)i;
        const float v = norm * expf(-(x * x) / (2.0f * (sigma * sigma)));
        k[radius + i] = v; k[radius - i] = v;
    }
    return DH_OK;
}

bool dh_vote_cell_fast_(const float K[9], int w, int h) {
    if (w <= 0 || h <= 0 || w % 20 != 0 || h % 20 != 0) return false;
    return std::fabs((double)K[2]) * 20.0 <= 100.0 * w && std::fabs((double)K[5]) * 20.0 <= 100.0 * h;
}

int dh_chunk_plan_(int m, int stage_chunk, bool single, int cstart[DH_STAGE_EVENTS + 1]) {
    if (m <= 0) { cstart[0] = 0; return 0; }
    if (single) { cstart[0] = 0; cstart[1] = m; return 1; }
// ... 95 lines not shown
```

depthhead_amd/csrc/dh_host.h:

```cpp
#pragma once
#include <stddef.h>
#include <stdint.h>

#include <functional>
#include <new>
#include <vector>

#include "../../include/depthhead_hip.h"

int dh_fail_(int code, const char *fmt, ...) __attribute__((format(printf, 2, 3)));
const char *dh_err_get_(void);
void dh_err_set_(const char *msg);

template <typename F>
static inline int dh_guard_(const char *what, F &&body) noexcept {
    try {
        return body();
    } catch (const std::bad_alloc &) {
        return dh_fail_(DH_ENOMEM, "%s: out of host memory", what);
    } catch (const std::exception &e) {
        return dh_fail_(DH_EINVAL, "%s: %s", what, e.what());
    } catch (...) {
        return dh_fail_(DH_EINVAL, "%s: unexpected exception", what);
    }
}

struct dh_forest {
    std::vector<int32_t> roots;
    std::vector<dh_node> nodes;
    std::vector<double> leaf_prob;
    std::vector<uint32_t> off_begin, rot_begin;
    std::vector<float> offsets;
    std::vector<double> rotations;
    uint32_t max_depth = 0;
    uint16_t max_x = 0, max_y = 0;
    bool uniform = false;
    uint16_t rw = 0, rh = 0;
};
int dh_forest_build_(const dh_forest_desc *d, dh_forest **out);
bool dh_rot_vote_ok_(double deg);

void dh_pack_off4_(const dh_forest &f, std::vector<uint32_t> &b4, std::vector<float> &o4);

struct __attribute__((aligned(16))) NodeG {
    uint8_t  r1[4], r2[4];
    int64_t  ilo;
    int32_t  child_zero, child_one;
    uint32_t amb;
    uint32_t cc;
};
void dh_build_nodes_g_(const dh_forest &f, std::vector<NodeG> &out);

struct Knobs {
    bool force_general = false;
    bool no_leaf_hist = false;
    bool box_no_ring = false;
    uint32_t leaf_hist_max = 16384;
    int lds_budget_kb = 0;
    int tile_x = 0, tile_y = 0;
    int box_band = 64;
    int box_bands = 0;
    int max_resident = 512;
    int chunks = 0;
    bool box_dense = false;
    bool no_region = false;
    int region_min_hits = 0;
    int top_levels = -1;
    bool no_zero_fold = false;
    bool no_tile_list = false;
    int tile_shift_mode = 0;
    int tile_shift_x = 0, tile_shift_y = 0;
    bool vote_exact = false;
    bool no_absorb = false;
    bool no_general_int = false;
    int stage_chunk = 64;
    int host_threads = 8;
    bool cl_stamps = false;
    int trav_stop = 0, emit_stop = 0, vote_stop = 0, cl_stop = 0;
    bool trav_stamps = false;
};
Knobs dh_read_knobs_();

struct Geom {
    int w = 0, h = 0, nx = 0, ny = 0, npatch = 0;
    int px = 0, py = 0, tiles_x = 0, tiles_y = 0, ss_max = 0, ss_row = 0, swz_log2 = 0, swz_q = 0;
    bool uniform = false;
    int top_levels = 0;
    int flag_words = 0;
    int win_cap = 0;
    int box_plane = 0, box_rows = 0, box_ow = 0, box_oh = 0, box_parts = 0, box_bands = 0;
    size_t lds = 0;
};
int dh_patch_grid_(const dh_params &p, int w, int h, int *nx, int *ny);

void dh_traverse_swizzle(int px, int step, int sw, int rw, int *swz_log2, int *swz_q, int *ss_row);
int dh_traverse_row_stride(int px, int step, int sw, int rw);
size_t dh_traverse_lds_bytes(int px, int py, int step, int sw, int sh, int top_words, int rw, int rh);

struct TileQuery {
    dh_params params{};
    int f_rw = 0, f_rh = 0;
    uint32_t n_trees = 0;
    bool absorb_ok = false;
    int top_levels = -1;
    bool one_pass = false;
    int lds_budget_kb = 0, tile_x = 0, tile_y = 0, box_band = 64;
};
int dh_choose_tile_(const TileQuery &q, Geom &g);
struct TileShifts {
    bool on = false;
    int gx = 1, nsx = 1, nsy = 1, sx0 = 0, sy0 = 0;
};
#define DH_TILE_SHIFT_LDS_WORDS 12288
static inline size_t dh_tile_shift_lds_words(int mask_blocks, int parts, int nc, int n_shifts) {
    return (size_t)2 * mask_blocks * parts + (size_t)(mask_blocks + 1) * (nc + 1) + (size_t)n_shifts + 8;
}
int dh_tile_shifts_(const Geom &g, int step, int blk_shift, const Knobs &k, TileShifts *out);
static const int kBoxSpan = 256, kBoxMaxRect = 96;
int dh_box_bands_(int n, int parts, int rows, int blk, int rh, int wg_slots, int *oh);

#define DH_GRID3 8000
#define DH_POSGRID 400
struct CounterLayout {
    size_t tiles = 0, leaves = 0;
    size_t hit_count = 0, pos_grid = 0, rot_grid = 0, tile_flags = 0, win_count = 0, leaf_hits = 0;
    size_t zero_lo = 0, zero_hi = 0;
    size_t zero_words = 0;
    size_t alloc_words = 0;
};
CounterLayout dh_counter_layout_(size_t cap, size_t flag_words, size_t tiles, size_t leaf_hist_leaves);

void dh_mat3_inv_f32_(const float m[9], float o[9]);
void dh_build_kernel_r2_(float sigma, std::vector<float> &k, size_t padded);
void dh_build_kernel_table_(float sigma, std::vector<float> &k);
int dh_blur_taps_(float sigma, std::vector<float> &k);

bool dh_vote_cell_fast_(const float K[9], int w, int h);

#define DH_STAGE_EVENTS 16
int dh_chunk_plan_(int m, int stage_chunk, bool single, int cstart[DH_STAGE_EVENTS + 1]);

struct DhRun { uint32_t dst, src; };
void dh_parallel_for_(int n, int threads, const std::function<void(int)> &fn);
long dh_rle_scan_(const uint8_t *buf, size_t len, uint32_t W, uint32_t H, DhRun *runs, uint32_t dst0, uint32_t src0, char *err, size_t errn);
struct RlePlan {
    uint32_t W = 0, H = 0;
    std::vector<size_t> blob_off;
    std::vector<uint32_t> run_begin;
    size_t nruns = 0;
};
int dh_rle_plan_(const uint8_t *const *bufs, const size_t *lens, int n, int threads, RlePlan &plan);
void dh_rle_pack_(const uint8_t *const *bufs, const size_t *lens, int n, int threads, const RlePlan &plan, uint8_t *blob, DhRun *runs);
```

depthhead_amd/csrc/dh_internal.h:

```cpp
#pragma once
#include <hip/hip_runtime.h>
#include <stddef.h>
#include <stdint.h>

#include "dh_host.h"
#include "dh_train.h"

#define DH_GRID 20
#define DH_ROTPARTS 120
#define DH_REGION_CELLS (26 * 26 * 26)
#define DH_KERN_R2 304
#define DH_SUPER_CELLS (64 * 64 * 64)

#define LF_PROB 1u
#define LF_ROT 2u
#define LF_OFF 4u
#define LF_FIN 8u

struct __attribute__((aligned(16))) DhCam {
    float k[9];
    float kinv[9];
    uint32_t pin;
    uint32_t pad;
};
// ... 9 lines not shown
    uint32_t flags;
    double   prob;
};

struct DevForest {
    const int32_t  *roots;
    const dh_node  *nodes;
    const double   *leaf_prob;
    const uint32_t *off_begin;
    const uint32_t *rot_begin;
    const float    *offsets;
    const float4   *off4;
    const uint32_t *off4_begin;
    const double   *rotations;
    uint32_t n_trees, n_nodes, n_leaves, n_off, n_rot;
    uint32_t *leaf_v;
    uint8_t  *leaf_flags;
    uint32_t *rot_bin;
    uint16_t *rot_mult;
    uint16_t *rot_rough;
    uint16_t *rough_mult;
    uint32_t *rough_cell;
    float    *off_min;
    float    *off_max;
    uint32_t *rbin_box;
    uint32_t *rbin_box_hi;
    struct LeafTpl *tpl;
    uint4 *rot_dir;
};

struct __attribute__((aligned(16))) HitRec {
    float    p3[3];
    uint32_t ob;
};
struct __attribute__((aligned(16))) HitBox {
    int32_t  lo[3];
    int32_t  hi0;
    int32_t  hi1, hi2;
    uint32_t v;
    uint32_t fc;
};
struct __attribute__((aligned(16))) HitRot {
    uint32_t lo;
    uint32_t hi;
    uint32_t rb;
    uint32_t n_rot;
};

struct TraverseArgs {
    const uint16_t *frames;
    int n_frames, w, h;
    int step, sw, sh;
    int nx, ny;
    int px, py;
    int tiles_x, tiles_y;
    int ss_max;
    int ss_row;
    int uniform;
    int rw, rh;
    uint32_t area;
    int swz_log2, swz_q;
    const uint32_t *box;
    int box_plane, box_rows;
    const uint2 *tile_list;
    const uint32_t *tile_list_count;
    uint32_t tile_list_stride;
    const uint32_t *gen;
    const uint8_t *tile_flags;
    const void *nodes_u;
    const void *nodes_a;
    uint32_t walk_lb;
    const uint32_t *amb_list;
    const uint32_t *top_tab;
    int top_levels;
    const void *nodes_g;
    unsigned long long *dbg_stamps;
    int stop_phase;
    DevForest f;
    uint32_t *win_count;
    uint32_t *win_patch;
    void     *win_leaf;
    int       leaf_ls;
    int       win_cap;
    int32_t  *dbg_leaf;
    uint8_t  *dbg_flags;
};

struct EmitArgs {
    const uint16_t *frames;
    int n_frames, w, h;
    int step, lw, lh;
    int nx, npatch;
    int px, py, tiles;
    float kinv[9];
    DevForest f;
    const uint32_t *win_count;
    const uint32_t *win_patch;
    const void     *win_leaf;
    int       leaf_ls;
    int       win_cap;
    HitRec   *hits;
    HitBox   *hit_box;
    HitRot   *hit_rot;
    uint32_t *hit_count;
    uint32_t  hits_cap;
    uint32_t *leaf_hits;
    uint32_t *gen;
    uint8_t  *dbg_flags;
    int stop;
    const DhCam *cams;
    uint32_t *hit_win;
};

struct BoxArgs {
    const uint16_t *frames;
    const uint16_t *zeros;
    int n_frames, w, h;
    int rw, rh;
    uint32_t *out;
    int plane, rows, lg;
    int ow, oh;
    uint8_t *tile_flags;
    const uint32_t *gen;
    uint32_t *list_count;
    uint32_t *zero_ptr;
    uint32_t zero_lo, zero_hi, zero_end;
    int tiles_x, tiles_y;
    int tpx, tpy, tbw, tbh;
    int parts, bands;
    int blocks_per_frame;
    int ring;
    unsigned long long *blk_mask;
    int mask_blocks;
    int blk_shift;
};

struct TileShiftArgs {
    const unsigned long long *blk_mask;
    int n_frames, mask_blocks, blk_shift, parts;
    int ow4, nc;
    int tiles_x, tiles_y;
    int tpx, tpy, tbw, tbh;
    int step;
    int sx0, sy0, gx, nsx, nsy;
    uint2 *list;
    uint32_t *count;
    uint32_t stride;
    uint32_t *shift_out;
};

struct PixFlagArgs {
    const uint16_t *frames;
    int n_frames, w, h;
    uint8_t *tile_flags;
    const uint32_t *gen;
    int tiles_x, tiles_y;
    int tpx, tpy, tfw, tfh;
};

struct VoteArgs {
    int n_frames, w, h;
    float k[9];
    DevForest f;
    const HitRec   *hits;
    const HitBox   *hit_box;
    const HitRot   *hit_rot;
    const uint32_t *hit_count;
    uint32_t  hits_cap;
    uint32_t *pos_grid;
    uint32_t *rot_grid;
    const uint32_t *leaf_hits;
    int stop;
    int cell_fast;
    float sx, sy;
    float kxs, cxs, kys, cys;
    const DhCam *cams;
    int cams_pin;
};

struct ClusterArgs {
    const uint16_t *frames;
    int n_frames, w, h;
    float kinv[9];
// ... 150 lines not shown
    DevForest f;
    const int32_t *leaf;
    const uint8_t *flags;
    uint8_t  *mask;
    uint32_t *hough32;
};

struct RleArgs {
    const uint16_t *blob;
    const uint2    *runs;
    const uint32_t *run_begin;
    uint16_t       *frames;
    int n_frames, blocks_per_frame;
};

struct TrainWinArgs {
    const uint16_t *frames;
    const uint8_t  *masks;
    uint32_t       *sat;
    int n, w, h;
    uint32_t W, H, step, lw, lh, nx, ny;
    uint64_t seed, frame0;
    uint32_t *sel;
    uint32_t *cnt;
};
struct TrainExtractArgs {
    const uint16_t *frames;
    const uint8_t  *masks;
    const uint32_t *sat;
    int w, h;
    uint32_t W, H, step, lw, lh, nx;
    uint32_t rw, rh, bw, bh;
    const uint4    *list;
    uint32_t        n_list;
    const float    *kinv;
    const float    *pos3d;
    const float    *rot_deg;
    uint32_t *box;
    uint8_t  *lab;
    float    *off;
    double   *rot;
};
struct TrainLevelArgs {
    const uint32_t *box;
    size_t stride;
    uint32_t bw;
    double area;
    const uint8_t  *lab;
    const float    *off;
    const double   *rot;
    const uint32_t *idx;
    const TrainNode *nodes;
    uint32_t n_nodes, F, cblocks;
    uint64_t seed;
    uint32_t W, H, rw, rh;
    double scale, wdepth;
    double   *score;
    TrainBest *best;
    uint8_t  *side;
    unsigned long long *neg_det;
};
hipError_t dh_launch_train_windows(const TrainWinArgs &a, hipStream_t s);
hipError_t dh_launch_train_extract(const TrainExtractArgs &a, hipStream_t s);
hipError_t dh_launch_train_level(const TrainLevelArgs &a, hipStream_t s);

struct Mat3Arg { float m[9]; };

hipError_t dh_launch_blur_u16(const uint16_t *in, uint16_t *tmp, uint16_t *out, int n, int w, int h, const float *kern, int klen, hipStream_t s);
hipError_t dh_launch_argmax2d(const uint16_t *hough, const uint16_t *frames, int n, int w, int h, const float kinv[9], dh_pose *out, hipStream_t s);
hipError_t dh_launch_rle_decode(const RleArgs &a, hipStream_t s);
hipError_t dh_region_init();
hipError_t dh_launch_zero(void *ptr, size_t bytes, hipStream_t s);
hipError_t dh_launch_mask(const AuxArgs &a, hipStream_t s);
hipError_t dh_launch_hough2d(const AuxArgs &a, uint16_t *out, hipStream_t s);
hipError_t dh_kernels_init(int device);
hipError_t dh_launch_leaf_prepare(const DevForest &f, hipStream_t s);
hipError_t dh_launch_nodes_compact(const DevForest &f, int ss, int swz_log2, int swz_q, uint32_t area, void *out, void *out_a, uint32_t *any_amb,
                                   uint32_t *amb_list, uint32_t n_amb, hipStream_t s);
#define DH_AMB_CAP 4096
hipError_t dh_launch_traverse(const TraverseArgs &a, size_t lds_bytes, hipStream_t s);
hipError_t dh_launch_tile_list(const uint8_t *flags, const uint32_t *gen, int n_frames, int tiles, uint2 *list, uint32_t *count, uint32_t stride, hipStream_t s);
hipError_t dh_launch_tile_shift(const TileShiftArgs &a, hipStream_t s);
hipError_t dh_launch_emit(const EmitArgs &a, hipStream_t s);
hipError_t dh_launch_vote(const VoteArgs &a, hipStream_t s);
hipError_t dh_launch_cluster(const ClusterArgs &a, hipStream_t s);
hipError_t dh_launch_region(const ClusterArgs &a, hipStream_t s);
hipError_t dh_launch_support(const SupportArgs &a, hipStream_t s);
hipError_t dh_launch_cluster_heads(const ClusterArgs &a, int max_heads, hipStream_t s);
hipError_t dh_launch_heads_seeds(const HeadsArgs &a, hipStream_t s);
hipError_t dh_launch_heads_moments(const HeadsArgs &a, hipStream_t s);
hipError_t dh_launch_heads_support(const HeadsArgs &a, hipStream_t s);
hipError_t dh_launch_heads_finish(const HeadsArgs &a, hipStream_t s);
hipError_t dh_launch_votes_dump(const VotesDumpArgs &a, hipStream_t s);
hipError_t dh_launch_track(const TrackArgs &a, hipStream_t s);
hipError_t dh_launch_track_heads(const TrackHeadsArgs &a, hipStream_t s);
hipError_t dh_launch_rig_fuse(const RigFuseArgs &a, hipStream_t s);
hipError_t dh_launch_boxsum(const BoxArgs &a, hipStream_t s);
hipError_t dh_launch_pixflags(const PixFlagArgs &a, hipStream_t s);
hipError_t dh_launch_top_build(const DevForest &f, const void *nodes_a, uint32_t n_amb, int top_levels, uint32_t *out, hipStream_t s);
```

depthhead_amd/csrc/k_emit.hip:

```cpp
#include "dh_device.h"

#define EMIT_THREADS 256
template <int EB, int LS, bool CAM, bool SUP>
__global__ void __launch_bounds__(EMIT_THREADS) k_emit(EmitArgs a) {
    const int frame = blockIdx.y, lane = threadIdx.x & (WAVE - 1);
    if (CAM) cam_kinv(a.kinv, a.cams + frame);
    if (a.gen && blockIdx.x == 0 && blockIdx.y == 0 && threadIdx.x == 0) *a.gen = *a.gen % 255u + 1u;
    const int pp = a.px * a.py;
    const uint32_t *counts = a.win_count + (size_t)frame * a.tiles;
    const uint32_t idx = (uint32_t)blockIdx.x * EMIT_THREADS + threadIdx.x;
    uint32_t before = 0;
    int tile = -1, slot = 0;
    for (int t0 = 0; t0 < a.tiles; t0 += WAVE) {
        const uint32_t c = t0 + lane < a.tiles ? counts[t0 + lane] : 0u;
        const uint32_t inc = wave_incl_scan(c);
        const uint32_t step_total = (uint32_t)__shfl((int)inc, WAVE - 1);
        const uint32_t r = idx - before;
        int s = 0;
#pragma unroll
        for (int b = WAVE / 2; b; b >>= 1)
            if ((uint32_t)__shfl((int)inc, s + b - 1) <= r) s += b;
        s = min(s, WAVE - 1);
        const uint32_t first = (uint32_t)__shfl((int)inc, s) - (uint32_t)__shfl((int)c, s);
        if (tile < 0 && idx >= before && r < step_total) { tile = t0 + s; slot = (int)(r - first); }
        before += step_total;
        if (__ballot(tile < 0) == 0ull) break;
    }
    const bool live = tile >= 0;
    if (__ballot(live) == 0ull || KNOB_STOP(a.stop == 1)) return;
    if (!live) { tile = 0; slot = 0; }
    const int T = (int)a.f.n_trees;
    const size_t w = (size_t)tile * pp + slot;
    uint32_t cnt = 0, gp = 0;
    bool gated = false;
    constexpr int ls = LS;
    const char *wl = (const char *)a.win_leaf + (((size_t)frame * a.win_cap * T + w) << ls);
    unsigned long long voting = 0;
    uint32_t rotv = 0, l[EB];
#pragma unroll
    for (int k = 0; k < EB; ++k) l[k] = 0;
    uint16_t zc = 0;
    if (live) {
        gp = a.win_patch[(size_t)frame * a.win_cap + w];
        double prob = 0.0;
        for (int t0 = 0; t0 < T; t0 += EB) {
            uint32_t lf[EB];
            double pr[EB];
            uint4 g[EB];
#pragma unroll
            for (int k = 0; k < EB; ++k) l[k] = load_leaf(wl, ls, (size_t)min(t0 + k, T - 1) * a.win_cap);
            if (t0 == 0) {
                const int gyi = (int)(gp / (uint32_t)a.nx), gxi = (int)gp - gyi * a.nx;
                zc = a.frames[(size_t)frame * a.w * a.h + (size_t)(gyi * a.step + a.lh) * a.w + gxi * a.step + a.lw];
            }
#pragma unroll
            for (int k = 0; k < EB; ++k) g[k] = ((const uint4 *)(a.f.tpl + l[k]))[3];
#pragma unroll
            for (int k = 0; k < EB; ++k) { lf[k] = g[k].y; pr[k] = __hiloint2double((int)g[k].w, (int)g[k].z); }
#pragma unroll
            for (int k = 0; k < EB; ++k)
                if (t0 + k < T) {
                    prob = __dadd_rn(prob, pr[k]);
                    if ((lf[k] & LF_PROB) && (lf[k] & (LF_ROT | LF_OFF))) {
                        cnt++; voting |= 1ull << ((t0 + k) & 63);
                        if (lf[k] & LF_ROT) rotv |= 1u << k;
                    }
                }
        }
        prob = __ddiv_rn(prob, (double)T);
        gated = prob > DH_PROB_GATE;
        if (!gated) { cnt = 0; voting = 0; rotv = 0; }
        if (gated && a.dbg_flags) a.dbg_flags[(size_t)frame * a.npatch + gp] = 3;
    }
    const bool hist_here = a.leaf_hits && T <= EB;
    if (hist_here) {
        uint32_t *lhist = a.leaf_hits + (size_t)frame * a.f.n_leaves;
#pragma unroll
        for (int k = 0; k < EB; ++k) {
            if (k >= T) continue;
            const bool v = (rotv >> k) & 1u;
            const uint32_t key = v ? l[k] : 0xFFFFFFFFu;
            const uint32_t prev = (uint32_t)__shfl_up((int)key, 1);
            const bool cont = v && lane > 0 && prev == key;
            const unsigned long long c = __ballot(cont);
            if (v && !cont) {
                const unsigned long long rest = lane == WAVE - 1 ? 0ull : (c >> (lane + 1));
                atomicAdd(&lhist[key], 1u + (uint32_t)__builtin_ctzll(~rest));
            }
        }
    }
    if (KNOB_STOP(a.stop == 2)) return;
    const uint32_t incl = wave_incl_scan(cnt);
    const uint32_t wave_total = __shfl(incl, WAVE - 1);
    if (wave_total == 0) return;
    uint32_t base = 0;
    if (lane == 0) base = atomicAdd(&a.hit_count[frame], wave_total);
    base = __shfl(base, 0);
    const uint32_t excl = incl - cnt;
    float q0 = 0.0f, q1 = 0.0f, q2 = 0.0f;
    if (cnt) {
        const int gyi = (int)(gp / (uint32_t)a.nx), gxi = (int)gp - gyi * a.nx;
        float q[3];
        to3d(a.kinv, (float)(gxi * a.step + a.lw), (float)(gyi * a.step + a.lh), (float)zc, q);
        q0 = q[0]; q1 = q[1]; q2 = q[2];
    }
    HitRec *dst = a.hits + (size_t)frame * a.hits_cap;
    HitBox *dbox = a.hit_box + (size_t)frame * a.hits_cap;
    HitRot *drot = a.hit_rot + (size_t)frame * a.hits_cap;
    const char *wlf = (const char *)a.win_leaf + (((size_t)frame * a.win_cap * T) << ls);
    const int wi = (int)w;
    for (uint32_t chunk = 0; chunk < wave_total; chunk += WAVE) {
        int src = 0, tree = 0;
        if (T <= 64) {
            const uint32_t h = chunk + (uint32_t)lane;
#pragma unroll
            for (int b = WAVE / 2; b; b >>= 1)
                if ((uint32_t)__shfl((int)incl, src + b - 1) <= h) src += b;
            src = min(src, WAVE - 1);
            uint32_t n = h - (uint32_t)__shfl((int)excl, src);
            const uint32_t vlo = (uint32_t)__shfl((int)(uint32_t)voting, src), vhi = (uint32_t)__shfl((int)(uint32_t)(voting >> 32), src);
            uint32_t word = vlo;
            const uint32_t clo = (uint32_t)__popc(vlo);
            if (n >= clo) { n -= clo; word = vhi; tree = 32; }
#pragma unroll
            for (int b = 16; b; b >>= 1) {
                const uint32_t c = (uint32_t)__popc(word & ((1u << b) - 1u));
                if (n >= c) { n -= c; word >>= b; tree += b; }
            }
        } else {
            const uint32_t h = chunk + (uint32_t)lane;
            for (int sl = 0; sl < WAVE; ++sl) {
                const uint32_t ex = (uint32_t)__shfl((int)excl, sl), cn = (uint32_t)__shfl((int)cnt, sl);
                const int sw = __shfl(wi, sl);
                if (h < ex || h >= ex + cn) continue;
                uint32_t r = ex;
                for (int t = 0; t < T; ++t) {
                    const uint32_t lf = a.f.leaf_flags[load_leaf(wlf, ls, (size_t)t * a.win_cap + sw)];
                    if ((lf & LF_PROB) && (lf & (LF_ROT | LF_OFF))) { if (r == h) { src = sl; tree = t; } ++r; }
                }
            }
        }
        const uint32_t h = chunk + (uint32_t)lane;
        const int sw = __shfl(wi, src);
        const float p0 = __shfl(q0, src), p1 = __shfl(q1, src), p2 = __shfl(q2, src);
        const uint32_t hw = SUP ? (uint32_t)__shfl((int)gp, src) : 0u;
        const uint32_t o = base + h;
        if (h < wave_total && o < a.hits_cap) {
            const uint32_t lid = load_leaf(wlf, ls, (size_t)tree * a.win_cap + sw);
            const uint4 *tp = (const uint4 *)(a.f.tpl + lid);
            const uint4 t0 = tp[0], t1 = tp[1], t2v = tp[2], t3 = tp[3];
            const float mn0 = __uint_as_float(t0.x), mn1 = __uint_as_float(t0.y), mn2 = __uint_as_float(t0.z),
                        mx0 = __uint_as_float(t0.w), mx1 = __uint_as_float(t1.x), mx2 = __uint_as_float(t1.y);
            *(float4 *)(dst + o) = make_float4(p0, p1, p2, __uint_as_float(t2v.x));
            ((int4 *)(dbox + o))[0] = make_int4(f32_as_i32(__fsub_rn(p0, mx0)), f32_as_i32(__fsub_rn(p1, mx1)),
                                                 f32_as_i32(__fsub_rn(p2, mx2)), f32_as_i32(__fsub_rn(p0, mn0)));
            ((int4 *)(dbox + o))[1] = make_int4(f32_as_i32(__fsub_rn(p1, mn1)), f32_as_i32(__fsub_rn(p2, mn2)), (int)t1.z, (int)t1.w);
            if (!a.leaf_hits || a.dbg_flags) *(uint4 *)(drot + o) = make_uint4(t2v.y, t2v.z, t2v.w, t3.x);
            if (a.leaf_hits && !hist_here && (t1.w & LF_ROT)) atomicAdd(&a.leaf_hits[(size_t)frame * a.f.n_leaves + lid], 1u);
            if (SUP) a.hit_win[(size_t)frame * a.hits_cap + o] = hw;
        }
    }
}

hipError_t dh_launch_emit(const EmitArgs &a, hipStream_t s) {
    if (a.n_frames == 0 || a.tiles == 0 || a.npatch == 0) return hipSuccess;
    if (a.n_frames > 65535) return hipErrorInvalidConfiguration;
    const dim3 grid((a.npatch + EMIT_THREADS - 1) / EMIT_THREADS, a.n_frames), block(EMIT_THREADS);
    const uint32_t T = a.f.n_trees;
#define EMIT_LAUNCH_S(EB_, SUP_)                                                                      \
    do {                                                                                              \
        if (a.cams) {                                                                                 \
            if (a.leaf_ls == 1) hipLaunchKernelGGL((k_emit<EB_, 1, true, SUP_>), grid, block, 0, s, a);   \
            else hipLaunchKernelGGL((k_emit<EB_, 2, true, SUP_>), grid, block, 0, s, a);                  \
        } else {                                                                                      \
            if (a.leaf_ls == 1) hipLaunchKernelGGL((k_emit<EB_, 1, false, SUP_>), grid, block, 0, s, a);  \
            else hipLaunchKernelGGL((k_emit<EB_, 2, false, SUP_>), grid, block, 0, s, a);                 \
        }                                                                                             \
    } while (0)
#define EMIT_LAUNCH(EB_)                                \
    do {                                                \
        if (a.hit_win) EMIT_LAUNCH_S(EB_, true);        \
        else EMIT_LAUNCH_S(EB_, false);                 \
    } while (0)
    if (T <= 4) EMIT_LAUNCH(4);
    else if (T <= 8) EMIT_LAUNCH(8);
    else if (T <= 10) EMIT_LAUNCH(10);
    else if (T <= 12) EMIT_LAUNCH(12);
    else EMIT_LAUNCH(16);
#undef EMIT_LAUNCH
#undef EMIT_LAUNCH_S
    return hipGetLastError();
}
```

depthhead_amd/csrc/k_traverse.hip:

```cpp
#include "dh_device.h"

#ifndef TRAV_THREADS
#define TRAV_THREADS 1024
#endif
#define TRAV_WMAX (4096 / TRAV_THREADS)
#define TRAV_WAVES (TRAV_THREADS / WAVE)
#define ROWS_IN_FLIGHT 8

template <int PPL>
__device__ __forceinline__ bool sat_rows_dpp(uint32_t *sat, uint32_t *flag, const uint16_t *img, int w, int fx0, int fy0,
                                             int fw, int fh, int ss) {
    constexpr int RMAX = 16 / PPL;
    const int tid = threadIdx.x, lane = tid & (WAVE - 1), wave = tid >> 6;
    const int R = (fh + TRAV_WAVES - 1) / TRAV_WAVES;
    const int y0 = wave * R, x0 = lane * PPL;
    const bool al = ((w % PPL) == 0) && ((fx0 % PPL) == 0) && ((((size_t)img) & (PPL * 2 - 1)) == 0);
    uint32_t p[RMAX][PPL];
    uint32_t any_px = 0;
    const uint16_t *org = img + (size_t)fy0 * w + fx0;
    if (al) {
        const bool fullx = x0 + PPL <= fw;
        uint32_t raw[RMAX][PPL / 2];
#pragma unroll
        for (int r = 0; r < RMAX; ++r) {
// ... 171 lines not shown
        }
        __syncthreads();
        if (SH > 1) {
            for (int y = tid; y < fh; y += TRAV_THREADS) {
                uint32_t *row = sat + (1 + y) * ss;
                uint32_t tot[8];
#pragma unroll
                for (int s2 = 0; s2 < 8; ++s2) tot[s2] = s2 < SH ? row[min(fw, (s2 + 1) * CW)] : 0u;
                uint32_t run = tot[0];
#pragma unroll
                for (int s2 = 1; s2 < 8; ++s2)
                    if (s2 < SH && s2 * CW < fw) { run += tot[s2]; row[min(fw, (s2 + 1) * CW)] = run; }
            }
            __syncthreads();
            int sg = tid / fh, y = tid - sg * fh;
            for (; sg < SH; sg += q, y += r) {
                if (y >= fh) { y -= fh; ++sg; if (sg >= SH) break; }
                const int xa = sg * CW, xb = min(fw, xa + CW);
                if (sg == 0 || xa >= fw) continue;
                uint32_t *row = sat + (1 + y) * ss;
                const uint32_t o = row[xa];
                for (int x = xa + 1; x < xb; ++x) row[x] += o;
            }
            __syncthreads();
        }
    }
    return true;
}

template <int W>
__device__ __forceinline__ void walk_uniform(const TraverseArgs &a, const uint32_t *sat, char *wleaf, int32_t *dleaf, const uint32_t *active,
                                             const uint32_t *agp, int n_active, int total, int cx, int ss, int T) {
    const int tid = threadIdx.x;
    const NodeU *nodes_u = (const NodeU *)a.nodes_u;
    const float r_active = 1.0f / (float)n_active, r_cx = 1.0f / (float)cx;
    for (int k0 = tid; k0 < total; k0 += W * TRAV_THREADS) {
        int cur[W], dst[W], ddst[W];
        const uint32_t *sp[W];
#pragma unroll
        for (int i = 0; i < W; ++i) {
            const int k = k0 + i * TRAV_THREADS;
            const bool has = k < total;
            const int kk = has ? k : k0;
            const int t = div_small(kk, n_active, r_active), slot = kk - t * n_active;
            const int p = (int)active[slot];
            const int py = div_small(p, cx, r_cx), px = p - py * cx;
            sp[i] = sat + py * a.step * ss + ((px * a.step) >> a.swz_log2);
            dst[i] = t * a.win_cap + slot;
            ddst[i] = dleaf ? (int)agp[slot] * T + t : 0;
            cur[i] = has ? a.f.roots[t] : -1;
        }
        for (;;) {
            bool go = false;
#pragma unroll
            for (int i = 0; i < W; ++i) go |= cur[i] >= 0;
            if (!go) break;
            uint4 n[W];
#pragma unroll
            for (int i = 0; i < W; ++i) n[i] = *(const uint4 *)(nodes_u + (cur[i] >= 0 ? cur[i] : 0));
            uint32_t s1[W], s2[W];
#pragma unroll
            for (int i = 0; i < W; ++i) { s1[i] = sp[i][n[i].x & 0x3fffu]; s2[i] = sp[i][(n[i].x >> 14) & 0x3fffu]; }
#pragma unroll
            for (int i = 0; i < W; ++i) {
                const int32_t d = (int32_t)s1[i] - (int32_t)s2[i];
                bool one = d > (int32_t)n[i].y;
                const uint32_t amb = n[i].x >> 28;
                if (cur[i] >= 0 && amb && one && d <= (int32_t)n[i].y + (int32_t)amb) {
                    const double thr = a.f.nodes[cur[i]].threshold, c = (double)a.area;
                    one = __dsub_rn(__ddiv_rn((double)s1[i], c), __ddiv_rn((double)s2[i], c)) > thr;
                }
                if (cur[i] >= 0) cur[i] = one ? (int)n[i].w : (int)n[i].z;
            }
        }
#pragma unroll
        for (int i = 0; i < W; ++i)
            if (k0 + i * TRAV_THREADS < total) {
                store_leaf(wleaf, a.leaf_ls, dst[i], ~cur[i]);
                if (dleaf) dleaf[ddst[i]] = ~cur[i];
            }
    }
}

template <int W>
__device__ __forceinline__ void walk_absorb(const TraverseArgs &a, const uint32_t *sat, const uint32_t *top, char *wleaf, int32_t *dleaf,
                                            const uint32_t *active, const uint32_t *agp, int n_active, int total, int cx, int ss, int T) {
    const int tid = threadIdx.x;
    const char *tab = (const char *)a.nodes_a;
    const uint32_t lb = a.walk_lb;
    const uint32_t amb_base = lb + (a.f.n_leaves << 4);
    const int DT = a.top_levels;
    const uint32_t hs = 1u << DT;
    const char *entries = (const char *)(top + (size_t)T * hs * 2);
    const float r_active = 1.0f / (float)n_active, r_cx = 1.0f / (float)cx;
    for (int k0 = tid; k0 < total; k0 += W * TRAV_THREADS) {
        uint32_t cur[W];
        int dst[W], ddst[W];
        const char *sp[W];
        uint32_t hb[W], h[W];
#pragma unroll
        for (int i = 0; i < W; ++i) {
            const int k = k0 + i * TRAV_THREADS;
            const int kk = k < total ? k : k0;
            const int t = div_small(kk, n_active, r_active), slot = kk - t * n_active;
            const int p = (int)active[slot];
            const int py = div_small(p, cx, r_cx), px = p - py * cx;
            sp[i] = (const char *)(sat + py * a.step * ss + ((px * a.step) >> a.swz_log2));
            dst[i] = t * a.win_cap + slot;
            ddst[i] = dleaf ? (int)agp[slot] * T + t : 0;
            hb[i] = ((uint32_t)t * hs) << 3;
            h[i] = 0;
        }
        for (int l = 0; l < DT; ++l) {
            uint2 nd[W];
#pragma unroll
            for (int i = 0; i < W; ++i) nd[i] = *(const uint2 *)((const char *)top + hb[i] + (h[i] << 3));
            uint32_t s1[W], s2[W];
#pragma unroll
            for (int i = 0; i < W; ++i) {
                s1[i] = *(const uint32_t *)(sp[i] + (nd[i].x & 0xffffu));
                s2[i] = *(const uint32_t *)(sp[i] + (nd[i].x >> 16));
            }
#pragma unroll
            for (int i = 0; i < W; ++i) h[i] = 2 * h[i] + (((int32_t)s1[i] - (int32_t)s2[i] > (int32_t)nd[i].y) ? 2u : 1u);
        }
#pragma unroll
        for (int i = 0; i < W; ++i) {
            const uint32_t e = *(const uint32_t *)(entries + (hb[i] >> 1) + ((h[i] - (hs - 1)) << 2));
            cur[i] = k0 + i * TRAV_THREADS < total ? e : lb;
        }
        for (;;) {
            for (;;) {
                uint32_t mn = cur[0];
#pragma unroll
                for (int i = 1; i < W; ++i) mn = min(mn, cur[i]);
                if (__ballot(mn < lb) == 0ull) break;
                uint4 n[W];
#pragma unroll
                for (int i = 0; i < W; ++i) n[i] = *(const uint4 *)(tab + min(cur[i], lb));
                uint32_t s1[W], s2[W];
#pragma unroll
                for (int i = 0; i < W; ++i) {
                    s1[i] = *(const uint32_t *)(sp[i] + (n[i].x & 0xffffu));
                    s2[i] = *(const uint32_t *)(sp[i] + (n[i].x >> 16));
                }
#pragma unroll
                for (int i = 0; i < W; ++i) {
                    const uint32_t nx = ((int32_t)s1[i] - (int32_t)s2[i] > (int32_t)n[i].y) ? n[i].w : n[i].z;
                    cur[i] = cur[i] >= lb ? cur[i] : nx;
                }
            }
            bool again = false;
#pragma unroll
            for (int i = 0; i < W; ++i)
                if (cur[i] >= amb_base) {
                    const uint32_t j = (cur[i] - amb_base) >> 4, X = a.amb_list[j];
                    const uint4 nu = *(const uint4 *)(tab + ((size_t)X << 4)), n2 = *(const uint4 *)(tab + ((size_t)(a.f.n_nodes + j) << 4));
                    const uint32_t s1 = *(const uint32_t *)(sp[i] + (nu.x & 0xffffu)), s2 = *(const uint32_t *)(sp[i] + (nu.x >> 16));
                    const double thr = a.f.nodes[X].threshold, c = (double)a.area;
                    const bool one = __dsub_rn(__ddiv_rn((double)s1, c), __ddiv_rn((double)s2, c)) > thr;
                    cur[i] = one ? n2.w : nu.z;
                    again = true;
                }
            if (__ballot(again) == 0ull) break;
        }
#pragma unroll
        for (int i = 0; i < W; ++i)
            if (k0 + i * TRAV_THREADS < total) {
                const int32_t leaf = (int32_t)((cur[i] - lb) >> 4);
                store_leaf(wleaf, a.leaf_ls, dst[i], leaf);
                if (dleaf) dleaf[ddst[i]] = leaf;
            }
    }
}


template <int W>
__device__ __forceinline__ void walk_general_int(const TraverseArgs &a, const uint32_t *sat, char *wleaf, int32_t *dleaf, const uint32_t *active,
                                                 const uint32_t *agp, int n_active, int total, int cx, int ss, int T) {
    const int tid = threadIdx.x;
    const NodeG *nodes_g = (const NodeG *)a.nodes_g;
    const float r_active = 1.0f / (float)n_active, r_cx = 1.0f / (float)cx;
    for (int k0 = tid; k0 < total; k0 += W * TRAV_THREADS) {
        int cur[W], dst[W], ddst[W];
        const uint32_t *sp[W];
#pragma unroll
        for (int i = 0; i < W; ++i) {
            const int k = k0 + i * TRAV_THREADS;
            const bool has = k < total;
            const int kk = has ? k : k0;
            const int t = div_small(kk, n_active, r_active), slot = kk - t * n_active;
            const int p = (int)active[slot];
            const int py = div_small(p, cx, r_cx), px = p - py * cx;
            sp[i] = sat + py * a.step * ss + px * a.step;
            dst[i] = t * a.win_cap + slot;
            ddst[i] = dleaf ? (int)agp[slot] * T + t : 0;
            cur[i] = has ? a.f.roots[t] : -1;
        }
        for (;;) {
            bool go = false;
#pragma unroll
            for (int i = 0; i < W; ++i) go |= cur[i] >= 0;
            if (!go) break;
            uint4 n0[W], n1[W];
#pragma unroll
            for (int i = 0; i < W; ++i) {
                const uint4 *np = (const uint4 *)(nodes_g + (cur[i] >= 0 ? cur[i] : 0));
                n0[i] = np[0]; n1[i] = np[1];
            }
            uint32_t c[W][8];
#pragma unroll
            for (int i = 0; i < W; ++i) {
                const int ax0 = n0[i].x & 0xff, ay0 = (n0[i].x >> 8) & 0xff, ax1 = (n0[i].x >> 16) & 0xff, ay1 = n0[i].x >> 24;
                const int bx0 = n0[i].y & 0xff, by0 = (n0[i].y >> 8) & 0xff, bx1 = (n0[i].y >> 16) & 0xff, by1 = n0[i].y >> 24;
                const uint32_t *q = sp[i];
                c[i][0] = q[ay1 * ss + ax1]; c[i][1] = q[ay0 * ss + ax1]; c[i][2] = q[ay1 * ss + ax0]; c[i][3] = q[ay0 * ss + ax0];
                c[i][4] = q[by1 * ss + bx1]; c[i][5] = q[by0 * ss + bx1]; c[i][6] = q[by1 * ss + bx0]; c[i][7] = q[by0 * ss + bx0];
            }
#pragma unroll
            for (int i = 0; i < W; ++i) {
                const uint32_t s1 = c[i][0] - c[i][1] - c[i][2] + c[i][3], s2 = c[i][4] - c[i][5] - c[i][6] + c[i][7];
                const uint32_t C1 = n1[i].w & 0xffffu, C2 = n1[i].w >> 16;
                const long long D = (long long)((unsigned long long)s1 * C2) - (long long)((unsigned long long)s2 * C1);
                const long long ilo = (long long)(((unsigned long long)n0[i].w << 32) | n0[i].z);
                bool one = D > ilo;
                if (cur[i] >= 0 && one && (unsigned long long)(D - ilo - 1) < (unsigned long long)n1[i].z) {
                    const dh_node nd = a.f.nodes[cur[i]];
                    const uint32_t c1 = (uint32_t)((nd.r1[2] - nd.r1[0]) * (nd.r1[3] - nd.r1[1])), c2 = (uint32_t)((nd.r2[2] - nd.r2[0]) * (nd.r2[3] - nd.r2[1]));
                    const double a1 = c1 ? __ddiv_rn((double)s1, (double)c1) : 0.0;
                    const double a2 = c2 ? __ddiv_rn((double)s2, (double)c2) : 0.0;
                    one = __dsub_rn(a1, a2) > nd.threshold;
                }
                if (cur[i] >= 0) cur[i] = one ? (int)n1[i].y : (int)n1[i].x;
            }
        }
#pragma unroll
        for (int i = 0; i < W; ++i)
            if (k0 + i * TRAV_THREADS < total) {
                store_leaf(wleaf, a.leaf_ls, dst[i], ~cur[i]);
                if (dleaf) dleaf[ddst[i]] = ~cur[i];
            }
    }
}

#ifdef DH_PROFILING_KNOBS
#define STAMP(k)                                                                        \
    if (a.dbg_stamps && tid == 0) {                                                     \
        unsigned long long t_ = clock64();                                              \
        atomicAdd(&a.dbg_stamps[k], t_ - t_prev);                                        \
        t_prev = t_;                                                                    \
    }
#else
#define STAMP(k)
#endif

template <bool UNI, bool GI>
__global__ void __launch_bounds__(TRAV_THREADS, TRAV_THREADS / 128) k_traverse(TraverseArgs a) {
    extern __shared__ __attribute__((aligned(16))) uint32_t lds[];
    const int tid = threadIdx.x, lane = tid & (WAVE - 1);
    const int T = (int)a.f.n_trees;

    int frame = (int)blockIdx.z * 8 + (int)blockIdx.x;
    int tile = (int)blockIdx.y;
    int sx = 0, sy = 0;
    if (a.tile_list) {
        const uint32_t k = blockIdx.y + gridDim.y * blockIdx.z;
        const uint2 e = a.tile_list[(size_t)blockIdx.x * a.tile_list_stride + k];
        const uint32_t cnt = a.tile_list_count[blockIdx.x];
        if (k >= cnt) return;
        frame = (int)(e.x >> 16) * 8 + (int)blockIdx.x; tile = (int)(e.x & 0xffffu);
        sx = (int)(e.y & 0xffffu); sy = (int)(e.y >> 16);
    }
    if (frame >= a.n_frames || KNOB_STOP(a.stop_phase == 9)) return;
    const int ty = div_small(tile, a.tiles_x, 1.0f / (float)a.tiles_x), tx = tile - ty * a.tiles_x;
    const int wx0 = max(0, tx * a.px - sx), wy0 = max(0, ty * a.py - sy);
    const int cx = min(a.nx, (tx + 1) * a.px - sx) - wx0, cy = min(a.ny, (ty + 1) * a.py - sy) - wy0;
    const float r_cx = 1.0f / (float)cx;
    const int npt = cx * cy;
    const int fx0 = wx0 * a.step, fy0 = wy0 * a.step;
    const int fw = (cx - 1) * a.step + a.sw, fh = (cy - 1) * a.step + a.sh;
    const int ss = a.ss_row;

    uint32_t *sat = lds;
    uint32_t *active = sat + a.ss_max;
    uint32_t *agp = active + a.px * a.py;
    uint32_t *misc = agp + a.px * a.py;
    uint32_t *top = misc + 16;

    const uint16_t *img = a.frames + (size_t)frame * a.w * a.h;
#ifdef DH_PROFILING_KNOBS
    unsigned long long t_prev = a.dbg_stamps ? clock64() : 0ull;
#endif

    const int wy = div_small(tid, cx, r_cx), wx = tid - wy * cx;
    bool nonzero = a.tile_list != nullptr || a.tile_flags[(size_t)frame * (a.tiles_x * a.tiles_y) + tile] == (uint8_t)*a.gen;
    if (tid < 8) misc[tid] = 0;
    if (!UNI) __syncthreads();
    if (UNI && nonzero) {
        const int bh = fh - a.rh + 1, bw = fw - a.rw + 1;
        const int m = 1 << a.swz_log2, q = a.swz_q, X0 = fx0 >> a.swz_log2;
        const uint32_t *bx = a.box + ((size_t)frame * a.box_rows + fy0) * ((size_t)a.box_plane << a.swz_log2) + X0;
        const int pieces = (m * q) >> 2;
        if ((X0 & 3) == 0 && pieces <= WAVE) {
            const int q4 = q >> 2;
            const int c = (lane * (65536 / q4 + 1)) >> 16, g = lane - c * q4;
            const uint32_t *src = bx + (size_t)c * a.box_plane + 4 * g;
            const size_t row_pitch = (size_t)a.box_plane << a.swz_log2;
            const int q4_tile = (((bw + m - 1) >> a.swz_log2) + 3) >> 2;
            if (lane < pieces && g < q4_tile)
                for (int y = tid >> 6; y < bh; y += TRAV_WAVES)
                    __builtin_amdgcn_global_load_lds(src + (size_t)y * row_pitch, sat + y * ss, 16, 0, 0);
        } else {
            const int qd = TRAV_THREADS / bw, rd = TRAV_THREADS - qd * bw;
            int yy = tid / bw, xx = tid - yy * bw;
            const int mm = m - 1;
            while (yy < bh) {
                const int xg = fx0 + xx;
                sat[yy * ss + (xx & mm) * q + (xx >> a.swz_log2)] =
                    a.box[((size_t)frame * a.box_rows + fy0 + yy) * ((size_t)a.box_plane << a.swz_log2) + (size_t)(xg & mm) * a.box_plane + (xg >> a.swz_log2)];
                yy += qd; xx += rd;
                if (xx >= bw) { xx -= bw; ++yy; }
            }
        }
        if (GI) {
            const int tw = T * (1 << a.top_levels) * 3;
            for (int i = tid; i < tw; i += TRAV_THREADS) top[i] = a.top_tab[i];
        }
        __syncthreads();
    }
    if (!UNI && nonzero) {
        const int strip = (fh + TRAV_WAVES - 1) / TRAV_WAVES;
        if (fw <= 2 * WAVE && strip <= 8 && a.ss_max >= TRAV_WAVES * WAVE * 2) nonzero = sat_rows_dpp<2>(sat, &misc[4], img, a.w, fx0, fy0, fw, fh, ss);
        else if (fw <= 4 * WAVE && strip <= 4 && a.ss_max >= TRAV_WAVES * WAVE * 4) nonzero = sat_rows_dpp<4>(sat, &misc[4], img, a.w, fx0, fy0, fw, fh, ss);
        else nonzero = sat_passes(sat, &misc[4], img, a.w, fx0, fy0, fw, fh, ss);
    }
    if (!nonzero) {
        if (a.dbg_flags)
            for (int p = tid; p < npt; p += TRAV_THREADS) {
                int gp = (wy0 + p / cx) * a.nx + wx0 + p % cx;
                size_t o = (size_t)frame * a.nx * a.ny + gp;
                a.dbg_flags[o] = 0;
                if (a.dbg_leaf)
                    for (int t = 0; t < T; ++t) a.dbg_leaf[o * T + t] = -1;
            }
        return;
    }
    if (KNOB_STOP(a.stop_phase == 1)) return;
    STAMP(0)

    const size_t wbase = (size_t)tile * (a.px * a.py);
    uint32_t *wpatch = a.win_patch + (size_t)frame * a.win_cap + wbase;
    if (tid < npt) {
        const int pxi = wx, pyi = wy;
        int ox = pxi * a.step, oy = pyi * a.step;
        uint32_t sum;
        if (UNI) {
            sum = 0;
            const uint32_t *wp = sat + oy * ss + (ox >> a.swz_log2);
            const int ncx = (a.sw + a.rw - 1) / a.rw, ncy = (a.sh + a.rh - 1) / a.rh;
            for (int iy = 0; iy < ncy; ++iy) {
                const int ro = min(iy * a.rh, a.sh - a.rh) * ss;
                for (int ix = 0; ix < ncx; ix += 4) {
                    uint32_t v[4];
#pragma unroll
                    for (int k = 0; k < 4; ++k) {
                        const int xc = min(min(ix + k, ncx - 1) * a.rw, a.sw - a.rw);
                        v[k] = wp[ro + (xc & ((1 << a.swz_log2) - 1)) * a.swz_q + (xc >> a.swz_log2)];
                    }
                    sum |= v[0] | v[1] | v[2] | v[3];
                }
            }
        } else {
            sum = sat[(oy + a.sh) * ss + ox + a.sw] - sat[oy * ss + ox + a.sw] - sat[(oy + a.sh) * ss + ox] + sat[oy * ss + ox];
        }
        const bool nonbg = sum != 0;
        const int gp = (wy0 + pyi) * a.nx + wx0 + pxi;
        const unsigned long long bal = __ballot(nonbg);
        uint32_t wave_base = 0;
        if (lane == 0 && bal) wave_base = atomicAdd(&misc[0], (uint32_t)__popcll(bal));
        wave_base = __shfl(wave_base, 0);
        if (nonbg) {
            const uint32_t slot = wave_base + (uint32_t)__popcll(bal & ((1ull << lane) - 1ull));
            active[slot] = (uint32_t)tid;
            agp[slot] = (uint32_t)gp;
        }
        if (a.dbg_flags) {
            a.dbg_flags[(size_t)frame * a.nx * a.ny + gp] = nonbg ? 1 : 0;
            if (!nonbg && a.dbg_leaf)
                for (int t = 0; t < T; ++t) a.dbg_leaf[((size_t)frame * a.nx * a.ny + gp) * T + t] = -1;
        }
    }
    __syncthreads();
    if (KNOB_STOP(a.stop_phase == 3)) return;
    STAMP(1)
    const int n_active = (int)misc[0];
    if (tid == 0) a.win_count[(size_t)frame * (a.tiles_x * a.tiles_y) + tile] = (uint32_t)n_active;
    if (n_active == 0) return;
    if (tid < n_active) wpatch[tid] = agp[tid];

    const int total = n_active * T;
    char *wleaf = (char *)a.win_leaf + (((size_t)frame * a.win_cap * T + wbase) << a.leaf_ls);
    int32_t *dleaf = a.dbg_leaf ? a.dbg_leaf + (size_t)frame * a.nx * a.ny * T : nullptr;
    if (UNI) {
        const int wave_first = __builtin_amdgcn_readfirstlane(tid & ~(WAVE - 1));
        const int all_passes = (total - wave_first + TRAV_THREADS - 1) / TRAV_THREADS;
        const int per_lane = all_passes > TRAV_WMAX ? (total + TRAV_THREADS - 1) / TRAV_THREADS : all_passes;
        if (GI) {
            if (per_lane <= 1) walk_absorb<1>(a, sat, top, wleaf, dleaf, active, agp, n_active, total, cx, ss, T);
            else if (per_lane == 2) walk_absorb<2>(a, sat, top, wleaf, dleaf, active, agp, n_active, total, cx, ss, T);
            else if (per_lane == 3) walk_absorb<3>(a, sat, top, wleaf, dleaf, active, agp, n_active, total, cx, ss, T);
#if TRAV_WMAX >= 8
            else if (per_lane == 4) walk_absorb<4>(a, sat, top, wleaf, dleaf, active, agp, n_active, total, cx, ss, T);
            else if (per_lane == 5) walk_absorb<5>(a, sat, top, wleaf, dleaf, active, agp, n_active, total, cx, ss, T);
            else if (per_lane == 6) walk_absorb<6>(a, sat, top, wleaf, dleaf, active, agp, n_active, total, cx, ss, T);
            else if (per_lane == 7) walk_absorb<7>(a, sat, top, wleaf, dleaf, active, agp, n_active, total, cx, ss, T);
            else walk_absorb<8>(a, sat, top, wleaf, dleaf, active, agp, n_active, total, cx, ss, T);
#else
            else walk_absorb<4>(a, sat, top, wleaf, dleaf, active, agp, n_active, total, cx, ss, T);
#endif
        } else
        if (per_lane <= 1) walk_uniform<1>(a, sat, wleaf, dleaf, active, agp, n_active, total, cx, ss, T);
        else if (per_lane == 2) walk_uniform<2>(a, sat, wleaf, dleaf, active, agp, n_active, total, cx, ss, T);
        else if (per_lane == 3) walk_uniform<3>(a, sat, wleaf, dleaf, active, agp, n_active, total, cx, ss, T);
        else walk_uniform<4>(a, sat, wleaf, dleaf, active, agp, n_active, total, cx, ss, T);
    } else if (GI) {
        const int per_lane = (total + TRAV_THREADS - 1) / TRAV_THREADS;
        if (per_lane <= 1) walk_general_int<1>(a, sat, wleaf, dleaf, active, agp, n_active, total, cx, ss, T);
        else walk_general_int<2>(a, sat, wleaf, dleaf, active, agp, n_active, total, cx, ss, T);
    } else {
        for (int k = tid; k < total; k += TRAV_THREADS) {
            const int t = div_small(k, n_active, 1.0f / (float)n_active), slot = k - t * n_active;
            const int p = (int)active[slot];
            const int pyi = div_small(p, cx, r_cx), pxi = p - pyi * cx;
            const uint32_t *sp = sat + pyi * a.step * ss + pxi * a.step;
            int cur = a.f.roots[t];
            while (cur >= 0) {
                const uint4 *np = (const uint4 *)(a.f.nodes + cur);
                const uint4 n0 = np[0], n1 = np[1];
                const int ax0 = n0.x & 0xffff, ay0 = n0.x >> 16, ax1 = n0.y & 0xffff, ay1 = n0.y >> 16;
                const int bx0 = n0.z & 0xffff, by0 = n0.z >> 16, bx1 = n0.w & 0xffff, by1 = n0.w >> 16;
                const double thr = __hiloint2double((int)n1.y, (int)n1.x);
                const uint32_t s1 = sp[ay1 * ss + ax1] - sp[ay0 * ss + ax1] - sp[ay1 * ss + ax0] + sp[ay0 * ss + ax0];
                const uint32_t s2 = sp[by1 * ss + bx1] - sp[by0 * ss + bx1] - sp[by1 * ss + bx0] + sp[by0 * ss + bx0];
                const uint32_t c1 = (uint32_t)((ax1 - ax0) * (ay1 - ay0)), c2 = (uint32_t)((bx1 - bx0) * (by1 - by0));
                const double a1 = c1 ? __ddiv_rn((double)s1, (double)c1) : 0.0;
                const double a2 = c2 ? __ddiv_rn((double)s2, (double)c2) : 0.0;
                cur = (__dsub_rn(a1, a2) > thr) ? (int)n1.w : (int)n1.z;
            }
            store_leaf(wleaf, a.leaf_ls, t * a.win_cap + slot, ~cur);
            if (dleaf) dleaf[(size_t)agp[slot] * T + t] = ~cur;
        }
    }

    STAMP(2)
}

#include <algorithm>
#include <atomic>
hipError_t dh_kernels_init(int device) {
    static std::atomic<unsigned long long> done[4];
    const bool tracked = device >= 0 && device < 256;
    if (tracked && (done[device >> 6].load(std::memory_order_acquire) >> (device & 63)) & 1ull) return hipSuccess;
    hipError_t e = hipFuncSetAttribute((const void *)k_traverse<true, false>, hipFuncAttributeMaxDynamicSharedMemorySize, 160 * 1024);
    if (e == hipSuccess) e = hipFuncSetAttribute((const void *)k_traverse<true, true>, hipFuncAttributeMaxDynamicSharedMemorySize, 160 * 1024);
    if (e == hipSuccess) e = hipFuncSetAttribute((const void *)k_traverse<false, false>, hipFuncAttributeMaxDynamicSharedMemorySize, 160 * 1024);
    if (e == hipSuccess) e = hipFuncSetAttribute((const void *)k_traverse<false, true>, hipFuncAttributeMaxDynamicSharedMemorySize, 160 * 1024);
    if (e == hipSuccess) e = dh_region_init();
    if (e != hipSuccess) return e;
    if (tracked) done[device >> 6].fetch_or(1ull << (device & 63), std::memory_order_release);
    return hipSuccess;
}

hipError_t dh_launch_traverse(const TraverseArgs &a, size_t lds_bytes, hipStream_t s) {
    const int tiles = a.tiles_x * a.tiles_y, fb = (a.n_frames + 7) / 8;
    if (tiles == 0 || fb == 0) return hipSuccess;
    if (tiles > 65535 || fb > 65535) return hipErrorInvalidConfiguration;
    const dim3 grid((unsigned)std::min(8, a.n_frames), tiles, fb);
    if (a.uniform && a.nodes_a) hipLaunchKernelGGL((k_traverse<true, true>), grid, dim3(TRAV_THREADS), lds_bytes, s, a);
    else if (a.uniform) hipLaunchKernelGGL((k_traverse<true, false>), grid, dim3(TRAV_THREADS), lds_bytes, s, a);
    else if (a.nodes_g) hipLaunchKernelGGL((k_traverse<false, true>), grid, dim3(TRAV_THREADS), lds_bytes, s, a);
    else hipLaunchKernelGGL((k_traverse<false, false>), grid, dim3(TRAV_THREADS), lds_bytes, s, a);
    return hipGetLastError();
}
```

depthhead_amd/prediction.py:

```python
from __future__ import annotations

import ctypes as C
from dataclasses import dataclass

import numpy as np

from . import _lib
from ._lib import HEAD_DTYPE, MAX_HEADS, POSE_DTYPE, SUPPORT_DTYPE, SUPPORT_RADIUS, check, vp
from .forest import Forest
from .synth import ModelParams


def _host_frames(img):
    frames = np.ascontiguousarray(img, dtype=np.uint16)
    single = frames.ndim == 2
    if single:
        frames = frames[None]
    n, h, w = frames.shape
    return frames, single, n, h, w


def _batch_frames(frames):
    frames = np.ascontiguousarray(frames, dtype=np.uint16)
    if frames.ndim != 3:
# ... 248 lines not shown
        return PredictionResult(out["mid_point"][0].copy(), out["rotation"][0].copy()) if single else out

    def predict_mask_device(self, frames_ptr: int, n: int, w: int, h: int, mask_ptr: int, stream: int = 0) -> None:
        check(self._lib.dh_predict_mask_device(self._ph, vp(frames_ptr), C.c_int(n), C.c_int(w), C.c_int(h), vp(mask_ptr),
                                               _stream(stream)))

    def hough_image_device(self, frames_ptr: int, n: int, w: int, h: int, intrinsic: IntrinsicMatrix, out_ptr: int,
                           stream: int = 0) -> None:
        check(self._lib.dh_hough_image_device(self._ph, vp(frames_ptr), C.c_int(n), C.c_int(w), C.c_int(h), _kmat(intrinsic),
                                              vp(out_ptr), _stream(stream)))

    def build_hough_image_device(self, frames_ptr: int, n: int, w: int, h: int, intrinsic: IntrinsicMatrix, out_ptr: int,
                                 stream: int = 0) -> None:
        check(self._lib.dh_build_hough_image_device(self._ph, vp(frames_ptr), C.c_int(n), C.c_int(w), C.c_int(h),
                                                    _kmat(intrinsic), vp(out_ptr), _stream(stream)))

    def predict_from2dhough_device(self, frames_ptr: int, n: int, w: int, h: int, intrinsic: IntrinsicMatrix, out_ptr: int,
                                   stream: int = 0) -> None:
        check(self._lib.dh_predict_from2dhough_device(self._ph, vp(frames_ptr), C.c_int(n), C.c_int(w), C.c_int(h),
                                                      _kmat(intrinsic), vp(out_ptr), _stream(stream)))

    def graph_capture(self, frames_ptr: int, n: int, w: int, h: int, intrinsic: IntrinsicMatrix, out_ptr: int,
                      midp_guess_ptr: int | None = None, rot_guess_ptr: int | None = None,
                      guess_mask_ptr: int | None = None) -> None:
        check(self._lib.dh_graph_capture(self._ph, vp(frames_ptr), C.c_int(n), C.c_int(w), C.c_int(h), _kmat(intrinsic),
                                         vp(midp_guess_ptr), vp(rot_guess_ptr), vp(guess_mask_ptr), vp(out_ptr)))

    def graph_launch(self, stream: int = 0) -> None:
        check(self._lib.dh_graph_launch(self._ph, _stream(stream)))

    def reserve(self, n: int, w: int, h: int) -> None:
        check(self._lib.dh_predictor_reserve(self._ph, C.c_int(n), C.c_int(w), C.c_int(h)))

    def set_forking(self, chunks: int) -> None:
        check(self._lib.dh_predictor_set_forking(self._ph, C.c_int(chunks)))

    def patch_grid(self, w: int, h: int) -> tuple[int, int]:
        nx, ny = C.c_int(), C.c_int()
        prm = self._cparams()
        check(self._lib.dh_patch_grid(C.byref(prm), C.c_int(w), C.c_int(h), C.byref(nx), C.byref(ny)))
        return nx.value, ny.value

    def set_profiling(self, on: bool) -> None:
        check(self._lib.dh_set_profiling(self._ph, C.c_int(1 if on else 0)))

    def timing(self) -> dict:
        t = _lib.Timing()
        check(self._lib.dh_get_timing(self._ph, C.byref(t)))
        return {"boxsum_ms": t.boxsum_ms, "traverse_ms": t.traverse_ms, "emit_ms": t.emit_ms, "vote_ms": t.vote_ms,
                "cluster_ms": t.cluster_ms, "total_ms": t.total_ms, "n_frames": t.n_frames}

    def debug_enable(self, on: bool = True) -> None:
        check(self._lib.dh_debug_enable(self._ph, C.c_int(1 if on else 0)))

    def debug_leaf_indices(self, n: int, w: int, h: int) -> np.ndarray:
        nx, ny = self.patch_grid(w, h)
        out = np.zeros((n, nx * ny, self.forest.n_trees), dtype=np.int32)
        check(self._lib.dh_debug_leaf_indices(self._ph, vp(out), C.c_size_t(out.size)))
        return out

    def debug_patch_flags(self, n: int, w: int, h: int) -> np.ndarray:
        nx, ny = self.patch_grid(w, h)
        out = np.zeros((n, nx * ny), dtype=np.uint8)
        check(self._lib.dh_debug_patch_flags(self._ph, vp(out), C.c_size_t(out.size)))
        return out

    def debug_grids(self, n: int):
        pos = np.zeros((n, 400), dtype=np.uint32)
        rot = np.zeros((n, 8000), dtype=np.uint32)
        check(self._lib.dh_debug_grids(self._ph, vp(pos), vp(rot)))
        return pos, rot

    def debug_guesses(self, n: int) -> np.ndarray:
        out = np.zeros((n, 6), dtype=np.int32)
        check(self._lib.dh_debug_guesses(self._ph, vp(out)))
        return out

    def debug_geometry(self) -> dict:
        out = np.zeros(10, dtype=np.int32)
        check(self._lib.dh_debug_geometry(self._ph, vp(out)))
        keys = ("uniform", "px", "py", "tiles_x", "tiles_y", "swz_log2", "swz_q", "ss_row", "rw", "rh")
        geo = dict(zip(keys, (int(x) for x in out)))
        path = geo["uniform"]
        geo.update(uniform=path & 1, walk_table=(path >> 8) & 1, top_levels=path >> 16)
        return geo

    def debug_tile_shifts(self, n: int) -> tuple[np.ndarray, np.ndarray]:
        shifts, counts = np.zeros((n, 2), dtype=np.int32), np.zeros(8, dtype=np.uint32)
        check(self._lib.dh_debug_tile_shifts(self._ph, vp(shifts), vp(counts)))
        return shifts, counts

    def debug_hit_counts(self, n: int) -> np.ndarray:
        out = np.zeros(n, dtype=np.uint32)
        check(self._lib.dh_debug_hit_counts(self._ph, vp(out)))
        return out

    def debug_votes(self, frame: int, which: int, cap: int = 1 << 22) -> np.ndarray:
        out = np.zeros((cap, 4), dtype=np.int32)
        cnt = C.c_size_t()
        check(self._lib.dh_debug_votes(self._ph, C.c_int(frame), C.c_int(which), vp(out), C.c_size_t(cap), C.byref(cnt)))
        if cnt.value > cap:
            return self.debug_votes(frame, which, int(cnt.value))
        return out[: cnt.value].copy()

    def debug_meanshift(self, n: int, which: int):
        it = self.params.meanshift_iterations
        trace = np.zeros((n, it + 1, 3), dtype=np.int32)
        steps = np.zeros(n, dtype=np.uint32)
        check(self._lib.dh_debug_meanshift(self._ph, C.c_int(which), vp(trace), vp(steps)))
        return trace, steps


def aggregate_votes(votes: np.ndarray) -> np.ndarray:
    if votes.shape[0] == 0:
        return np.zeros((0, 4), dtype=np.int32)
    order = np.lexsort((votes[:, 2], votes[:, 1], votes[:, 0]))
    v = votes[order]
    new = np.ones(v.shape[0], dtype=bool)
    new[1:] = np.any(v[1:, :3] != v[:-1, :3], axis=1)
    idx = np.flatnonzero(new)
    sums = np.add.reduceat(v[:, 3].astype(np.uint32).astype(np.uint64), idx) & np.uint64(0xFFFFFFFF)
    out = np.empty((idx.size, 4), dtype=np.int32)
    out[:, :3] = v[idx, :3]
    out[:, 3] = sums.astype(np.uint32).view(np.int32)
    return out
```

include/depthhead_hip.h:

```cpp
#ifndef DEPTHHEAD_HIP_H
#define DEPTHHEAD_HIP_H

#include <stddef.h>
#include <stdint.h>

#ifdef __cplusplus
extern "C" {
#endif

#define DH_VERSION 100

#define DH_OK 0
#define DH_EINVAL (-1)
#define DH_EFOREST (-2)
#define DH_EHIP (-3)
#define DH_ENOMEM (-4)
#define DH_ESIZE (-5)
#define DH_ESTATE (-6)

#define DH_ZSCALEFACTOR 1
#define DH_GUESS_GRID_PARTS 20
#define DH_ROT_GRID_PARTS 120
#define DH_MAX_VARIANCE_ROT 400.0
#define DH_MAX_VARIANCE_OFFSET 5200.0f
// ... 667 lines not shown
int dh_fit_identify_subjects_cameras(dh_fitter *f, const uint16_t *frames, int n, int w, int h, const dh_cameras *c,
                                     const dh_fit_subjects *set, const dh_render_instance *instances, uint32_t n_instances,
                                     const uint8_t *enrolled, uint32_t n_subjects, const dh_fit_record *fit_records,
                                     const dh_ident_params *params, uint32_t *subjects_out, dh_ident_record *records,
                                     dh_render_instance *poses_out, dh_fit_record *scores);
int dh_fit_identify_subjects_device(dh_fitter *f, const uint16_t *frames, int n, int w, int h, const float K[9], const dh_fit_subjects *set,
                                    const dh_render_instance *instances, uint32_t n_instances, const uint8_t *enrolled,
                                    uint32_t n_subjects, const dh_fit_record *fit_records, const dh_ident_params *params,
                                    uint32_t *subjects_out, dh_ident_record *records, dh_render_instance *poses_out,
                                    dh_fit_record *scores, void *stream);
int dh_fit_identify_subjects_cameras_device(dh_fitter *f, const uint16_t *frames, int n, int w, int h, const dh_cameras *c,
                                            const dh_fit_subjects *set, const dh_render_instance *instances, uint32_t n_instances,
                                            const uint8_t *enrolled, uint32_t n_subjects, const dh_fit_record *fit_records,
                                            const dh_ident_params *params, uint32_t *subjects_out, dh_ident_record *records,
                                            dh_render_instance *poses_out, dh_fit_record *scores, void *stream);

#define DH_IDENT_VIEWS_DEFAULT_MAX_RMS 2.58
int dh_fit_ident_views_params_default(dh_ident_params *p);
int dh_fit_identify_subjects_views(dh_fitter *f, const uint16_t *frames, uint32_t n_sets, int w, int h, const dh_fit_views *views,
                                   const dh_fit_subjects *set, const dh_view_instance *instances, uint32_t n_instances,
                                   const uint32_t *sets, const uint8_t *enrolled, uint32_t n_subjects,
                                   const dh_view_fit_record *fit_records, const dh_ident_params *params, uint32_t *subjects_out,
                                   dh_ident_record *records, dh_view_instance *poses_out, dh_view_fit_record *scores);
int dh_fit_identify_subjects_views_device(dh_fitter *f, const uint16_t *frames, uint32_t n_sets, int w, int h, const dh_fit_views *views,
                                          const dh_fit_subjects *set, const dh_view_instance *instances, uint32_t n_instances,
                                          const uint32_t *sets, const uint8_t *enrolled, uint32_t n_subjects,
                                          const dh_view_fit_record *fit_records, const dh_ident_params *params, uint32_t *subjects_out,
                                          dh_ident_record *records, dh_view_instance *poses_out, dh_view_fit_record *scores,
                                          void *stream);

int dh_biwi_decode_depth(const uint8_t *buf, size_t len, uint16_t *out, size_t cap_px, uint32_t *w, uint32_t *h);
int dh_biwi_parse_cal(const char *text, size_t len, float K[9]);
int dh_biwi_parse_pose(const uint8_t *buf, size_t len, const float K[9], float pos3d[3], float pos2d[2], float rot[3]);

typedef struct dh_train_params {
    uint32_t stepwidth;
    uint32_t subimage_width;
    uint32_t subimage_height;
    uint32_t max_depth;
    uint32_t n_trees;
    uint32_t subset_per_tree;
    double   subrect_feature_scale;
    uint32_t features_per_node;
    uint32_t min_subset_size;
    double   steepness;
    uint64_t seed;
} dh_train_params;

typedef struct dh_train_stats {
    uint64_t frames;
    uint64_t pool_size;
    uint64_t pool_positives;
    uint64_t neg_det;
    uint32_t levels;
    uint32_t reserved;
} dh_train_stats;

typedef struct dh_trainer dh_trainer;

int dh_trainer_create(const dh_train_params *p, int device, dh_trainer **out);
int dh_trainer_destroy(dh_trainer *t);
int dh_trainer_add_frames(dh_trainer *t, const uint16_t *frames, const uint8_t *masks, int n, int w, int h, const float *K,
                          const float *pos3d, const float *rot_deg);
int dh_trainer_fit(dh_trainer *t, dh_forest **out);
int dh_trainer_stats(const dh_trainer *t, dh_train_stats *out, uint32_t *nodes_per_level, uint32_t *leaves_per_level,
                     float *level_ms, uint32_t cap_levels);

int dh_forest_export(const dh_forest *f, int32_t *roots, dh_node *nodes, double *leaf_prob, uint32_t *off_begin,
                     uint32_t *rot_begin, float *offsets, double *rotations, uint32_t *n_off, uint32_t *n_rot);

int dh_set_profiling(dh_predictor *p, int on);
int dh_get_timing(dh_predictor *p, dh_timing *out);

int dh_debug_enable(dh_predictor *p, int on);
int dh_debug_leaf_indices(dh_predictor *p, int32_t *out, size_t cap_elems);
int dh_debug_patch_flags(dh_predictor *p, uint8_t *out, size_t cap_elems);
int dh_debug_grids(dh_predictor *p, uint32_t *pos_grid, uint32_t *rot_grid);
int dh_debug_guesses(dh_predictor *p, int32_t *out);
int dh_debug_votes(dh_predictor *p, int frame, int which, int32_t *out, size_t cap_records, size_t *count);
int dh_debug_meanshift(dh_predictor *p, int which, int32_t *trace, uint32_t *steps);
int dh_debug_hit_counts(dh_predictor *p, uint32_t *out);
int dh_debug_geometry(dh_predictor *p, int32_t out[10]);
int dh_debug_tile_shifts(dh_predictor *p, int32_t *shifts, uint32_t counts[8]);

#ifdef __cplusplus
}
#endif
#endif
```

Before: 715,100.

## Gate patches by leaf probability inside traverse and compact windows per frame

Moves the per-patch probability gate from the emit kernel into the tail of the uniform absorb traverse kernel. Leaf probabilities are averaged in LDS, and gated patches are compacted into a single per-frame window list using wave-level atomics. Emit then skips the per-tile prefix scan and the probability recompute. This cuts the window and leaf-index writes and the emit work for ungated patches, at the cost of extra LDS traffic, barriers and registers in traverse, plus a global atomic per wave.

```diff
diff --git a/depthhead_amd/_lib.py b/depthhead_amd/_lib.py
--- a/depthhead_amd/_lib.py
+++ b/depthhead_amd/_lib.py
@@ -198,7 +198,7 @@
     "dh_biwi_decode_depth", "dh_biwi_parse_cal", "dh_biwi_parse_pose",
     "dh_graph_capture", "dh_graph_launch", "dh_graph_destroy",
     "dh_set_profiling", "dh_get_timing", "dh_debug_enable", "dh_debug_leaf_indices", "dh_debug_patch_flags",
-    "dh_debug_grids", "dh_debug_guesses", "dh_debug_votes", "dh_debug_meanshift", "dh_debug_hit_counts", "dh_debug_geometry", "dh_debug_tile_shifts",
+    "dh_debug_grids", "dh_debug_guesses", "dh_debug_votes", "dh_debug_meanshift", "dh_debug_hit_counts", "dh_debug_geometry", "dh_debug_tile_shifts", "dh_debug_window_totals",
     "dh_trainer_create", "dh_trainer_destroy", "dh_trainer_add_frames", "dh_trainer_fit", "dh_trainer_stats", "dh_forest_export",
     "dh_cameras_create", "dh_cameras_destroy", "dh_predict_batch_cameras", "dh_predict_batch_cameras_device",
     "dh_tracker_create", "dh_tracker_destroy", "dh_tracker_reset", "dh_tracker_step", "dh_tracker_step_device",
diff --git a/depthhead_amd/csrc/dh_api.hip b/depthhead_amd/csrc/dh_api.hip
--- a/depthhead_amd/csrc/dh_api.hip
+++ b/depthhead_amd/csrc/dh_api.hip
@@ -44,6 +44,7 @@
     size_t tile_list_stride = 0;
     TileShifts shifts;
     Buf<uint32_t> tile_shift;
+    bool last_gated = false;
     int list_chunks = 0;
     uint32_t *list_ptr(int chunk) const { return tile_list.get() + (size_t)chunk * 8 * (2 * tile_list_stride + 1); }
     Buf<uint32_t> win_patch;
@@ -93,6 +94,7 @@
     uint32_t *rot_grid(int f0) const { return counters.get() + lay.rot_grid + (size_t)f0 * DH_GRID3; }
     uint8_t *tile_flags(int f0) const { return (uint8_t *)(counters.get() + lay.tile_flags) + (size_t)f0 * lay.tiles; }
     uint32_t *win_count(int f0) const { return counters.get() + lay.win_count + (size_t)f0 * lay.tiles; }
+    uint32_t *win_total(int f0) const { return counters.get() + lay.win_count + f0; }
     uint32_t *leaf_hits(int f0) const { return lay.leaves ? counters.get() + lay.leaf_hits + (size_t)f0 * lay.leaves : nullptr; }
 };
 
@@ -598,7 +600,7 @@
             else {
                 unsigned long long hst[8];
                 HIP_TRY(hipMemcpy(hst, stamps, 64, hipMemcpyDeviceToHost));
-                fprintf(stderr, "[k_traverse cycles/phase summed over the workgroups that reach it] region=%llu gate=%llu walks=%llu\n", hst[0], hst[1], hst[2]);
+                fprintf(stderr, "[k_traverse cycles/phase summed over the workgroups that reach it] region=%llu gate=%llu walks=%llu gated tail=%llu\n", hst[0], hst[1], hst[2], hst[3]);
                 HIP_TRY(hipMemset(stamps, 0, 64));
             }
             ta.dbg_stamps = stamps;
@@ -608,6 +610,9 @@
         const int tiles = g.tiles_x * g.tiles_y;
         uint32_t *win_count = ws.win_count(f0);
         ta.win_count = win_count; ta.win_cap = g.win_cap;
+        const bool gate = !o.traverse_only && !o.leaf_out && !o.flags_out && dh_tile_gate_(g, p->ws.cap_frames, p->absorb_ok, p->n_trees, p->debug, p->knobs);
+        if (gate) { ta.tile_gate = 1; ta.win_total = ws.win_total(f0); }
+        if (!o.traverse_only) p->ws.last_gated = gate;
         ta.win_patch = ws.win_patch.get() + (size_t)f0 * g.win_cap; ta.win_leaf = ws.win_leaf.get() + (((size_t)f0 * g.win_cap * p->n_trees) << ws.leaf_ls); ta.leaf_ls = ws.leaf_ls;
         ta.dbg_leaf = o.leaf_out ? o.leaf_out : p->debug ? ws.dbg_leaf.get() + (size_t)f0 * g.npatch * p->n_trees : nullptr;
         ta.dbg_flags = o.flags_out ? o.flags_out : p->debug ? ws.dbg_flags.get() + (size_t)f0 * g.npatch : nullptr;
@@ -622,6 +627,7 @@
             memcpy(ea.kinv, kinv, 9 * sizeof(float));
             ea.cams = cs.dev();
             ea.f = p->dev;
+            ea.win_total = ta.win_total; ea.pre_gated = ta.tile_gate;
             ea.win_count = win_count; ea.win_patch = ta.win_patch; ea.win_leaf = ta.win_leaf; ea.leaf_ls = ws.leaf_ls; ea.win_cap = g.win_cap;
             ea.hits = ws.hits.get() + hoff; ea.hit_box = ws.hit_box.get() + hoff; ea.hit_rot = ws.hit_rot.get() + hoff;
             ea.hit_count = hit_count; ea.hits_cap = ws.hits_cap;
@@ -1837,12 +1843,33 @@
         return DH_OK;
     });
 }
+static int debug_window_totals_(dh_predictor *p, uint32_t *out) {
+    return with_taps(p, false, [&]() -> int {
+        if (!out) return fail(DH_EINVAL, "NULL output");
+        const Workspace &ws = p->ws;
+        const Geom &g = ws.geom;
+        const size_t bytes = (size_t)p->last_n * 4;
+        if (g.npatch <= 0) { memset(out, 0, bytes); return DH_OK; }
+        if (ws.last_gated) { HIP_TRY(hipMemcpy(out, ws.win_total(0), bytes, hipMemcpyDeviceToHost)); return DH_OK; }
+        Buf<uint32_t> tot;
+        TRY(tot.alloc(p->last_n));
+        HIP_TRY(hipMemset(tot.get(), 0, bytes));
+        EmitArgs ea{};
+        ea.n_frames = p->last_n; ea.px = g.px; ea.py = g.py; ea.tiles = g.tiles_x * g.tiles_y; ea.f = p->dev;
+        ea.win_count = ws.win_count(0); ea.win_leaf = ws.win_leaf.get(); ea.leaf_ls = ws.leaf_ls; ea.win_cap = g.win_cap;
+        HIP_TRY(dh_launch_window_totals(ea, tot.get(), nullptr));
+        HIP_TRY(hipDeviceSynchronize());
+        HIP_TRY(hipMemcpy(out, tot.get(), bytes, hipMemcpyDeviceToHost));
+        return DH_OK;
+    });
+}
 static int debug_geometry_(dh_predictor *p, int32_t out[10]) {
     if (!p || !out) return fail(DH_EINVAL, "NULL argument");
     if (p->ws.cap_frames == 0) return fail(DH_ESTATE, "no workspace yet (dh_predictor_reserve or a batch)");
     const Geom &g = p->ws.geom;
     const bool walk_tab = g.uniform && p->absorb_ok;
-    const int32_t v[10] = {(g.uniform ? 1 : 0) | (walk_tab ? 1 << 8 : 0) | (walk_tab ? g.top_levels << 16 : 0), g.px, g.py, g.tiles_x, g.tiles_y, g.swz_log2, g.swz_q, g.ss_row, p->f_rw, p->f_rh};
+    const bool tile_gate = dh_tile_gate_(g, p->ws.cap_frames, p->absorb_ok, p->n_trees, p->debug, p->knobs);
+    const int32_t v[10] = {(g.uniform ? 1 : 0) | (walk_tab ? 1 << 8 : 0) | (tile_gate ? 1 << 9 : 0) | (walk_tab ? g.top_levels << 16 : 0), g.px, g.py, g.tiles_x, g.tiles_y, g.swz_log2, g.swz_q, g.ss_row, p->f_rw, p->f_rh};
     memcpy(out, v, sizeof v);
     return DH_OK;
 }
@@ -2358,6 +2385,7 @@
 DH_API(debug_grids, (dh_predictor *p, uint32_t *pos_grid, uint32_t *rot_grid), (p, pos_grid, rot_grid))
 DH_API(debug_hit_counts, (dh_predictor *p, uint32_t *out), (p, out))
 DH_API(debug_geometry, (dh_predictor *p, int32_t out[10]), (p, out))
+DH_API(debug_window_totals, (dh_predictor *p, uint32_t *out), (p, out))
 DH_API(debug_tile_shifts, (dh_predictor *p, int32_t *shifts, uint32_t counts[8]), (p, shifts, counts))
 DH_API(debug_guesses, (dh_predictor *p, int32_t *out), (p, out))
 DH_API(debug_meanshift, (dh_predictor *p, int which, int32_t *trace, uint32_t *steps), (p, which, trace, steps))
diff --git a/depthhead_amd/csrc/dh_host.cpp b/depthhead_amd/csrc/dh_host.cpp
--- a/depthhead_amd/csrc/dh_host.cpp
+++ b/depthhead_amd/csrc/dh_host.cpp
@@ -184,6 +184,7 @@
     k.region_min_hits = std::max(0, geti("DH_REGION_MIN_HITS", 0));
     k.no_general_int = getenv("DH_NO_GENERAL_INT") != nullptr;
     k.no_absorb = getenv("DH_NO_ABSORB") != nullptr;
+    k.no_tile_gate = getenv("DH_NO_TILE_GATE") != nullptr;
     k.vote_exact = getenv("DH_VOTE_EXACT") != nullptr;
     k.no_tile_list = getenv("DH_NO_TILE_LIST") != nullptr;
     k.no_zero_fold = getenv("DH_NO_ZERO_FOLD") != nullptr;
@@ -339,6 +340,12 @@
     t.on = fits;
     *out = t;
     return DH_OK;
+}
+
+bool dh_tile_gate_(const Geom &g, int cap_frames, bool absorb_ok, uint32_t n_trees, bool taps, const Knobs &k) {
+    if (!g.uniform || !absorb_ok || g.npatch <= 0 || cap_frames <= 1 || taps || k.no_tile_gate) return false;
+    const size_t items = (size_t)g.px * g.py * n_trees;
+    return items <= 4096 && items * 8 <= (size_t)4 * g.ss_max;
 }
 
 CounterLayout dh_counter_layout_(size_t cap, size_t flag_words, size_t tiles, size_t leaf_hist_leaves) {
diff --git a/depthhead_amd/csrc/dh_host.h b/depthhead_amd/csrc/dh_host.h
--- a/depthhead_amd/csrc/dh_host.h
+++ b/depthhead_amd/csrc/dh_host.h
@@ -72,6 +72,7 @@
     int tile_shift_x = 0, tile_shift_y = 0;
     bool vote_exact = false;
     bool no_absorb = false;
+    bool no_tile_gate = false;
     bool no_general_int = false;
     int stage_chunk = 64;
     int host_threads = 8;
@@ -119,6 +120,8 @@
 static const int kBoxSpan = 256, kBoxMaxRect = 96;
 int dh_box_bands_(int n, int parts, int rows, int blk, int rh, int wg_slots, int *oh);
 
+bool dh_tile_gate_(const Geom &g, int cap_frames, bool absorb_ok, uint32_t n_trees, bool taps, const Knobs &k);
+
 #define DH_GRID3 8000
 #define DH_POSGRID 400
 struct CounterLayout {
diff --git a/depthhead_amd/csrc/dh_internal.h b/depthhead_amd/csrc/dh_internal.h
--- a/depthhead_amd/csrc/dh_internal.h
+++ b/depthhead_amd/csrc/dh_internal.h
@@ -115,6 +115,8 @@
     void     *win_leaf;
     int       leaf_ls;
     int       win_cap;
+    uint32_t *win_total;
+    int       tile_gate;
     int32_t  *dbg_leaf;
     uint8_t  *dbg_flags;
 };
@@ -132,6 +134,8 @@
     const void     *win_leaf;
     int       leaf_ls;
     int       win_cap;
+    const uint32_t *win_total;
+    int       pre_gated;
     HitRec   *hits;
     HitBox   *hit_box;
     HitRot   *hit_rot;
@@ -448,6 +452,7 @@
 hipError_t dh_launch_tile_list(const uint8_t *flags, const uint32_t *gen, int n_frames, int tiles, uint2 *list, uint32_t *count, uint32_t stride, hipStream_t s);
 hipError_t dh_launch_tile_shift(const TileShiftArgs &a, hipStream_t s);
 hipError_t dh_launch_emit(const EmitArgs &a, hipStream_t s);
+hipError_t dh_launch_window_totals(const EmitArgs &a, uint32_t *out, hipStream_t s);
 hipError_t dh_launch_vote(const VoteArgs &a, hipStream_t s);
 hipError_t dh_launch_cluster(const ClusterArgs &a, hipStream_t s);
 hipError_t dh_launch_region(const ClusterArgs &a, hipStream_t s);
diff --git a/depthhead_amd/csrc/k_emit.hip b/depthhead_amd/csrc/k_emit.hip
--- a/depthhead_amd/csrc/k_emit.hip
+++ b/depthhead_amd/csrc/k_emit.hip
@@ -1,7 +1,7 @@
 #include "dh_device.h"
 
 #define EMIT_THREADS 256
-template <int EB, int LS, bool CAM, bool SUP>
+template <int EB, int LS, bool CAM, bool SUP, bool PG>
 __global__ void __launch_bounds__(EMIT_THREADS) k_emit(EmitArgs a) {
     const int frame = blockIdx.y, lane = threadIdx.x & (WAVE - 1);
     if (CAM) cam_kinv(a.kinv, a.cams + frame);
@@ -11,6 +11,9 @@
     const uint32_t idx = (uint32_t)blockIdx.x * EMIT_THREADS + threadIdx.x;
     uint32_t before = 0;
     int tile = -1, slot = 0;
+    if (PG) {
+        if (idx < min(a.win_total[frame], (uint32_t)a.win_cap)) { tile = 0; slot = (int)idx; }
+    } else
     for (int t0 = 0; t0 < a.tiles; t0 += WAVE) {
         const uint32_t c = t0 + lane < a.tiles ? counts[t0 + lane] : 0u;
         const uint32_t inc = wave_incl_scan(c);
@@ -60,15 +63,15 @@
 #pragma unroll
             for (int k = 0; k < EB; ++k)
                 if (t0 + k < T) {
-                    prob = __dadd_rn(prob, pr[k]);
+                    if (!PG) prob = __dadd_rn(prob, pr[k]);
                     if ((lf[k] & LF_PROB) && (lf[k] & (LF_ROT | LF_OFF))) {
                         cnt++; voting |= 1ull << ((t0 + k) & 63);
                         if (lf[k] & LF_ROT) rotv |= 1u << k;
                     }
                 }
         }
-        prob = __ddiv_rn(prob, (double)T);
-        gated = prob > DH_PROB_GATE;
+        if (!PG) prob = __ddiv_rn(prob, (double)T);
+        gated = PG ? true : prob > DH_PROB_GATE;
         if (!gated) { cnt = 0; voting = 0; rotv = 0; }
         if (gated && a.dbg_flags) a.dbg_flags[(size_t)frame * a.npatch + gp] = 3;
     }
@@ -162,20 +165,46 @@
     }
 }
 
+__global__ void __launch_bounds__(EMIT_THREADS) k_window_totals(EmitArgs a, uint32_t *out) {
+    const int frame = blockIdx.x, T = (int)a.f.n_trees, pp = a.px * a.py;
+    const char *wl = (const char *)a.win_leaf + (((size_t)frame * a.win_cap * T) << a.leaf_ls);
+    uint32_t n = 0;
+    for (int tile = 0; tile < a.tiles; ++tile) {
+        const uint32_t c = min(a.win_count[(size_t)frame * a.tiles + tile], (uint32_t)pp);
+        for (uint32_t slot = threadIdx.x; slot < c; slot += EMIT_THREADS) {
+            const size_t w = (size_t)tile * pp + slot;
+            double prob = 0.0;
+            for (int t = 0; t < T; ++t) prob = __dadd_rn(prob, a.f.leaf_prob[load_leaf(wl, a.leaf_ls, (size_t)t * a.win_cap + w)]);
+            if (__ddiv_rn(prob, (double)T) > DH_PROB_GATE) ++n;
+        }
+    }
+    if (n) atomicAdd(&out[frame], n);
+}
+hipError_t dh_launch_window_totals(const EmitArgs &a, uint32_t *out, hipStream_t s) {
+    if (a.n_frames == 0 || a.tiles == 0) return hipSuccess;
+    hipLaunchKernelGGL(k_window_totals, dim3(a.n_frames), dim3(EMIT_THREADS), 0, s, a, out);
+    return hipGetLastError();
+}
+
 hipError_t dh_launch_emit(const EmitArgs &a, hipStream_t s) {
     if (a.n_frames == 0 || a.tiles == 0 || a.npatch == 0) return hipSuccess;
-    if (a.n_frames > 65535) return hipErrorInvalidConfiguration;
+    if (a.n_frames > 65535 || (a.pre_gated && !a.win_total)) return hipErrorInvalidConfiguration;
     const dim3 grid((a.npatch + EMIT_THREADS - 1) / EMIT_THREADS, a.n_frames), block(EMIT_THREADS);
     const uint32_t T = a.f.n_trees;
-#define EMIT_LAUNCH_S(EB_, SUP_)                                                                      \
-    do {                                                                                              \
-        if (a.cams) {                                                                                 \
-            if (a.leaf_ls == 1) hipLaunchKernelGGL((k_emit<EB_, 1, true, SUP_>), grid, block, 0, s, a);   \
-            else hipLaunchKernelGGL((k_emit<EB_, 2, true, SUP_>), grid, block, 0, s, a);                  \
-        } else {                                                                                      \
-            if (a.leaf_ls == 1) hipLaunchKernelGGL((k_emit<EB_, 1, false, SUP_>), grid, block, 0, s, a);  \
-            else hipLaunchKernelGGL((k_emit<EB_, 2, false, SUP_>), grid, block, 0, s, a);                 \
-        }                                                                                             \
+#define EMIT_LAUNCH_P(EB_, SUP_, PG_)                                                                      \
+    do {                                                                                                   \
+        if (a.cams) {                                                                                      \
+            if (a.leaf_ls == 1) hipLaunchKernelGGL((k_emit<EB_, 1, true, SUP_, PG_>), grid, block, 0, s, a);   \
+            else hipLaunchKernelGGL((k_emit<EB_, 2, true, SUP_, PG_>), grid, block, 0, s, a);                  \
+        } else {                                                                                           \
+            if (a.leaf_ls == 1) hipLaunchKernelGGL((k_emit<EB_, 1, false, SUP_, PG_>), grid, block, 0, s, a);  \
+            else hipLaunchKernelGGL((k_emit<EB_, 2, false, SUP_, PG_>), grid, block, 0, s, a);                 \
+        }                                                                                                  \
+    } while (0)
+#define EMIT_LAUNCH_S(EB_, SUP_)                        \
+    do {                                                \
+        if (a.pre_gated) EMIT_LAUNCH_P(EB_, SUP_, true); \
+        else EMIT_LAUNCH_P(EB_, SUP_, false);           \
     } while (0)
 #define EMIT_LAUNCH(EB_)                                \
     do {                                                \
@@ -189,5 +218,6 @@
     else EMIT_LAUNCH(16);
 #undef EMIT_LAUNCH
 #undef EMIT_LAUNCH_S
+#undef EMIT_LAUNCH_P
     return hipGetLastError();
 }
diff --git a/depthhead_amd/csrc/k_traverse.hip b/depthhead_amd/csrc/k_traverse.hip
--- a/depthhead_amd/csrc/k_traverse.hip
+++ b/depthhead_amd/csrc/k_traverse.hip
@@ -277,9 +277,10 @@
     }
 }
 
-template <int W>
+template <int W, bool GATE>
 __device__ __forceinline__ void walk_absorb(const TraverseArgs &a, const uint32_t *sat, const uint32_t *top, char *wleaf, int32_t *dleaf,
-                                            const uint32_t *active, const uint32_t *agp, int n_active, int total, int cx, int ss, int T) {
+                                            const uint32_t *active, const uint32_t *agp, int n_active, int total, int cx, int ss, int T,
+                                            uint32_t (&gl)[TRAV_WMAX], double (&gpr)[TRAV_WMAX]) {
     const int tid = threadIdx.x;
     const char *tab = (const char *)a.nodes_a;
     const uint32_t lb = a.walk_lb;
@@ -359,13 +360,20 @@
                 }
             if (__ballot(again) == 0ull) break;
         }
-#pragma unroll
-        for (int i = 0; i < W; ++i)
-            if (k0 + i * TRAV_THREADS < total) {
-                const int32_t leaf = (int32_t)((cur[i] - lb) >> 4);
-                store_leaf(wleaf, a.leaf_ls, dst[i], leaf);
-                if (dleaf) dleaf[ddst[i]] = leaf;
-            }
+        if (GATE) {
+#pragma unroll
+            for (int i = 0; i < W; ++i) gl[i] = (cur[i] - lb) >> 4;
+#pragma unroll
+            for (int i = 0; i < W; ++i) gpr[i] = a.f.leaf_prob[gl[i]];
+        } else {
+#pragma unroll
+            for (int i = 0; i < W; ++i)
+                if (k0 + i * TRAV_THREADS < total) {
+                    const int32_t leaf = (int32_t)((cur[i] - lb) >> 4);
+                    store_leaf(wleaf, a.leaf_ls, dst[i], leaf);
+                    if (dleaf) dleaf[ddst[i]] = leaf;
+                }
+        }
     }
 }
 
@@ -449,7 +457,7 @@
 #define STAMP(k)
 #endif
 
-template <bool UNI, bool GI>
+template <bool UNI, bool GI, bool GATE = false>
 __global__ void __launch_bounds__(TRAV_THREADS, TRAV_THREADS / 128) k_traverse(TraverseArgs a) {
     extern __shared__ __attribute__((aligned(16))) uint32_t lds[];
     const int tid = threadIdx.x, lane = tid & (WAVE - 1);
@@ -589,29 +597,33 @@
     if (KNOB_STOP(a.stop_phase == 3)) return;
     STAMP(1)
     const int n_active = (int)misc[0];
-    if (tid == 0) a.win_count[(size_t)frame * (a.tiles_x * a.tiles_y) + tile] = (uint32_t)n_active;
+    if (!GATE && tid == 0) a.win_count[(size_t)frame * (a.tiles_x * a.tiles_y) + tile] = (uint32_t)n_active;
     if (n_active == 0) return;
-    if (tid < n_active) wpatch[tid] = agp[tid];
+    if (!GATE && tid < n_active) wpatch[tid] = agp[tid];
 
     const int total = n_active * T;
     char *wleaf = (char *)a.win_leaf + (((size_t)frame * a.win_cap * T + wbase) << a.leaf_ls);
     int32_t *dleaf = a.dbg_leaf ? a.dbg_leaf + (size_t)frame * a.nx * a.ny * T : nullptr;
+    uint32_t gl[TRAV_WMAX];
+    double gpr[TRAV_WMAX];
+#pragma unroll
+    for (int i = 0; i < TRAV_WMAX; ++i) { gl[i] = 0; gpr[i] = 0.0; }
     if (UNI) {
         const int wave_first = __builtin_amdgcn_readfirstlane(tid & ~(WAVE - 1));
         const int all_passes = (total - wave_first + TRAV_THREADS - 1) / TRAV_THREADS;
         const int per_lane = all_passes > TRAV_WMAX ? (total + TRAV_THREADS - 1) / TRAV_THREADS : all_passes;
         if (GI) {
-            if (per_lane <= 1) walk_absorb<1>(a, sat, top, wleaf, dleaf, active, agp, n_active, total, cx, ss, T);
-            else if (per_lane == 2) walk_absorb<2>(a, sat, top, wleaf, dleaf, active, agp, n_active, total, cx, ss, T);
-            else if (per_lane == 3) walk_absorb<3>(a, sat, top, wleaf, dleaf, active, agp, n_active, total, cx, ss, T);
+            if (per_lane <= 1) walk_absorb<1, GATE>(a, sat, top, wleaf, dleaf, active, agp, n_active, total, cx, ss, T, gl, gpr);
+            else if (per_lane == 2) walk_absorb<2, GATE>(a, sat, top, wleaf, dleaf, active, agp, n_active, total, cx, ss, T, gl, gpr);
+            else if (per_lane == 3) walk_absorb<3, GATE>(a, sat, top, wleaf, dleaf, active, agp, n_active, total, cx, ss, T, gl, gpr);
 #if TRAV_WMAX >= 8
-            else if (per_lane == 4) walk_absorb<4>(a, sat, top, wleaf, dleaf, active, agp, n_active, total, cx, ss, T);
-            else if (per_lane == 5) walk_absorb<5>(a, sat, top, wleaf, dleaf, active, agp, n_active, total, cx, ss, T);
-            else if (per_lane == 6) walk_absorb<6>(a, sat, top, wleaf, dleaf, active, agp, n_active, total, cx, ss, T);
-            else if (per_lane == 7) walk_absorb<7>(a, sat, top, wleaf, dleaf, active, agp, n_active, total, cx, ss, T);
-            else walk_absorb<8>(a, sat, top, wleaf, dleaf, active, agp, n_active, total, cx, ss, T);
+            else if (per_lane == 4) walk_absorb<4, GATE>(a, sat, top, wleaf, dleaf, active, agp, n_active, total, cx, ss, T, gl, gpr);
+            else if (per_lane == 5) walk_absorb<5, GATE>(a, sat, top, wleaf, dleaf, active, agp, n_active, total, cx, ss, T, gl, gpr);
+            else if (per_lane == 6) walk_absorb<6, GATE>(a, sat, top, wleaf, dleaf, active, agp, n_active, total, cx, ss, T, gl, gpr);
+            else if (per_lane == 7) walk_absorb<7, GATE>(a, sat, top, wleaf, dleaf, active, agp, n_active, total, cx, ss, T, gl, gpr);
+            else walk_absorb<8, GATE>(a, sat, top, wleaf, dleaf, active, agp, n_active, total, cx, ss, T, gl, gpr);
 #else
-            else walk_absorb<4>(a, sat, top, wleaf, dleaf, active, agp, n_active, total, cx, ss, T);
+            else walk_absorb<4, GATE>(a, sat, top, wleaf, dleaf, active, agp, n_active, total, cx, ss, T, gl, gpr);
 #endif
         } else
         if (per_lane <= 1) walk_uniform<1>(a, sat, wleaf, dleaf, active, agp, n_active, total, cx, ss, T);
@@ -648,6 +660,50 @@
     }
 
     STAMP(2)
+
+    if (GATE) {
+        if (KNOB_STOP(a.stop_phase == 4)) return;
+        __syncthreads();
+        double *pprob = (double *)sat;
+#pragma unroll
+        for (int i = 0; i < TRAV_WMAX; ++i) {
+            const int k = tid + i * TRAV_THREADS;
+            if (k < total) pprob[k] = gpr[i];
+        }
+        __syncthreads();
+        if (__builtin_amdgcn_readfirstlane(tid & ~(WAVE - 1)) < n_active) {
+            bool gated = false;
+            if (tid < n_active) {
+                double prob = 0.0;
+                for (int t = 0; t < T; ++t) prob = __dadd_rn(prob, pprob[t * n_active + tid]);
+                prob = __ddiv_rn(prob, (double)T);
+                gated = prob > DH_PROB_GATE;
+            }
+            const unsigned long long bal = __ballot(gated);
+            uint32_t lslot = 0xffffffffu;
+            if (bal) {
+                uint32_t wave_base = 0;
+                if (lane == 0) wave_base = atomicAdd(&a.win_total[frame], (uint32_t)__popcll(bal));
+                wave_base = __shfl(wave_base, 0);
+                if (gated) lslot = wave_base + (uint32_t)__popcll(bal & ((1ull << lane) - 1ull));
+                if (lslot < (uint32_t)a.win_cap) a.win_patch[(size_t)frame * a.win_cap + lslot] = agp[tid];
+            }
+            if (tid < n_active) active[tid] = lslot;
+        }
+        __syncthreads();
+        char *fl = (char *)a.win_leaf + (((size_t)frame * a.win_cap * T) << a.leaf_ls);
+        const float r_act = 1.0f / (float)n_active;
+#pragma unroll
+        for (int i = 0; i < TRAV_WMAX; ++i) {
+            const int k = tid + i * TRAV_THREADS;
+            if (k < total) {
+                const int t = div_small(k, n_active, r_act);
+                const uint32_t lslot = active[k - t * n_active];
+                if (lslot < (uint32_t)a.win_cap) store_leaf(fl, a.leaf_ls, t * a.win_cap + (int)lslot, (int32_t)gl[i]);
+            }
+        }
+        STAMP(3)
+    }
 }
 
 #include <algorithm>
@@ -658,6 +714,7 @@
     if (tracked && (done[device >> 6].load(std::memory_order_acquire) >> (device & 63)) & 1ull) return hipSuccess;
     hipError_t e = hipFuncSetAttribute((const void *)k_traverse<true, false>, hipFuncAttributeMaxDynamicSharedMemorySize, 160 * 1024);
     if (e == hipSuccess) e = hipFuncSetAttribute((const void *)k_traverse<true, true>, hipFuncAttributeMaxDynamicSharedMemorySize, 160 * 1024);
+    if (e == hipSuccess) e = hipFuncSetAttribute((const void *)k_traverse<true, true, true>, hipFuncAttributeMaxDynamicSharedMemorySize, 160 * 1024);
     if (e == hipSuccess) e = hipFuncSetAttribute((const void *)k_traverse<false, false>, hipFuncAttributeMaxDynamicSharedMemorySize, 160 * 1024);
     if (e == hipSuccess) e = hipFuncSetAttribute((const void *)k_traverse<false, true>, hipFuncAttributeMaxDynamicSharedMemorySize, 160 * 1024);
     if (e == hipSuccess) e = dh_region_init();
@@ -671,7 +728,9 @@
     if (tiles == 0 || fb == 0) return hipSuccess;
     if (tiles > 65535 || fb > 65535) return hipErrorInvalidConfiguration;
     const dim3 grid((unsigned)std::min(8, a.n_frames), tiles, fb);
-    if (a.uniform && a.nodes_a) hipLaunchKernelGGL((k_traverse<true, true>), grid, dim3(TRAV_THREADS), lds_bytes, s, a);
+    if (a.tile_gate && !(a.uniform && a.nodes_a && a.win_total)) return hipErrorInvalidValue;
+    if (a.tile_gate) hipLaunchKernelGGL((k_traverse<true, true, true>), grid, dim3(TRAV_THREADS), lds_bytes, s, a);
+    else if (a.uniform && a.nodes_a) hipLaunchKernelGGL((k_traverse<true, true>), grid, dim3(TRAV_THREADS), lds_bytes, s, a);
     else if (a.uniform) hipLaunchKernelGGL((k_traverse<true, false>), grid, dim3(TRAV_THREADS), lds_bytes, s, a);
     else if (a.nodes_g) hipLaunchKernelGGL((k_traverse<false, true>), grid, dim3(TRAV_THREADS), lds_bytes, s, a);
     else hipLaunchKernelGGL((k_traverse<false, false>), grid, dim3(TRAV_THREADS), lds_bytes, s, a);
diff --git a/depthhead_amd/prediction.py b/depthhead_amd/prediction.py
--- a/depthhead_amd/prediction.py
+++ b/depthhead_amd/prediction.py
@@ -354,7 +354,7 @@
         keys = ("uniform", "px", "py", "tiles_x", "tiles_y", "swz_log2", "swz_q", "ss_row", "rw", "rh")
         geo = dict(zip(keys, (int(x) for x in out)))
         path = geo["uniform"]
-        geo.update(uniform=path & 1, walk_table=(path >> 8) & 1, top_levels=path >> 16)
+        geo.update(uniform=path & 1, walk_table=(path >> 8) & 1, tile_gate=bool((path >> 9) & 1), top_levels=path >> 16)
         return geo
 
     def debug_tile_shifts(self, n: int) -> tuple[np.ndarray, np.ndarray]:
@@ -365,6 +365,11 @@
     def debug_hit_counts(self, n: int) -> np.ndarray:
         out = np.zeros(n, dtype=np.uint32)
         check(self._lib.dh_debug_hit_counts(self._ph, vp(out)))
+        return out
+
+    def debug_window_totals(self, n: int) -> np.ndarray:
+        out = np.zeros(n, dtype=np.uint32)
+        check(self._lib.dh_debug_window_totals(self._ph, vp(out)))
         return out
 
     def debug_votes(self, frame: int, which: int, cap: int = 1 << 22) -> np.ndarray:
diff --git a/include/depthhead_hip.h b/include/depthhead_hip.h
--- a/include/depthhead_hip.h
+++ b/include/depthhead_hip.h
@@ -773,6 +773,7 @@
 int dh_debug_hit_counts(dh_predictor *p, uint32_t *out);
 int dh_debug_geometry(dh_predictor *p, int32_t out[10]);
 int dh_debug_tile_shifts(dh_predictor *p, int32_t *shifts, uint32_t counts[8]);
+int dh_debug_window_totals(dh_predictor *p, uint32_t *out);
 
 #ifdef __cplusplus
 }
```

New measurement: 757,100, median of 6. 5.9% higher.
